# zhangkao/IIP_UAVSal_Saliency

Hardware: AMD Instinct MI355X
Metric: saliency frames/sec at 360x640 (higher is better)
Workload: dtype f32; 1 GPU; 360x640 batch=1 clip(s)/GPU seq=8, UAVSal.forward_clips, prec=f32, launch loop; requests_in_flight=1, clips_per_gpu=1, seq_len=8, height=360, width=640, precision=f32, persistent_state=False, parallelism=single GPU, fused_dw=10

## Files before the change

iip_uavsal_saliency_amd/_lib.py:

```python
from __future__ import annotations

import collections
import ctypes as C
import os

PKG = os.path.dirname(os.path.abspath(__file__))
LIB_PATH = os.environ.get("UAVSAL_HIP_LIB") or os.path.join(PKG, "libuavsal_hip.so")

PREC = {"f32": 0, "bf16x3": 1, "bf16": 2, "f16x3": 3}
ACT_NONE, ACT_RELU6, ACT_SIGMOID = 0, 1, 2
EPI_AFFINE, EPI_TWA, EPI_LSTM = 0, 1, 2
SK_TICKET_BASE = 4096

_ERR = {-1: "UAVSAL_EINVAL (null pointer / non-positive size)",
        -2: "UAVSAL_EALIGN (channel count / ld / pointer not 16-byte aligned)",
        -3: "UAVSAL_ESHAPE (shape not supported by the kernel)",
        -4: "UAVSAL_ESTATE (plan used in the wrong state)",
        -5: "UAVSAL_EDEVICE (a kernel reported a device-side error; the run's outputs are invalid)"}
ERR_STREAMK = 1
DW_KERNEL = {1: "dw3x3_kernel<1, 4, 4>", 2: "dw3x3_kernel<1, 2, 2>", 3: "dw3x3_kernel<2, 2, 2>", 4: "dw3x3_dilated_kernel",
             16: "dw3x3_map_lds_kernel<16, 256>", 32: "dw3x3_map_lds_kernel<32, 256>",
             528: "dw3x3_map_lds_kernel<16, 512>", 544: "dw3x3_map_lds_kernel<32, 512>",
             2048: "dw3x3_rowclass_kernel<256>"}

_f = C.c_void_p


class ConvDesc(C.Structure):
    _fields_ = [("a", _f), ("lda", C.c_int32), ("a_img_stride", C.c_int64),
                ("w", _f), ("scale", _f), ("bias", _f),
                ("out", _f), ("ldc", C.c_int32), ("o_img_stride", C.c_int64),
                ("res", _f), ("ldr", C.c_int32), ("r_img_stride", C.c_int64),
                ("aux", _f), ("ldx", C.c_int32), ("x_img_stride", C.c_int64),
                ("n_img", C.c_int32), ("H", C.c_int32), ("W", C.c_int32),
                ("Cin", C.c_int32), ("Cout", C.c_int32), ("taps", C.c_int32),
                ("prec", C.c_int32), ("act", C.c_int32), ("epi", C.c_int32), ("tile", C.c_int32),
                ("out2", _f), ("ld2", C.c_int32),
                ("dw_w9c", _f), ("dw_scale", _f), ("dw_bias", _f),
                ("dw_stride", C.c_int32), ("dw_Hin", C.c_int32), ("dw_Win", C.c_int32),
                ("sk_ws", _f), ("sk_ws_bytes", C.c_int64),
                ("a_split", _f), ("ldas", C.c_int32),
                ("out_split", _f), ("ldos", C.c_int32),
                ("err", _f), ("sk_spin_limit", C.c_int32), ("sk_debug_drop", C.c_int32),
                ("w_group_stride", C.c_int64), ("n_group", C.c_int32), ("a_group_off", C.c_int32)]


ROUTE_PRESPLIT, ROUTE_DWPROJ, ROUTE_STREAMK, ROUTE_K32, ROUTE_F32_DMA, ROUTE_STAGED = 1, 2, 3, 4, 5, 6
REDUCE_NONE, REDUCE_LAUNCH, REDUCE_IN_LAUNCH = 0, 1, 2


class ConvRoute(C.Structure):
    _fields_ = [("family", C.c_int32), ("tile", C.c_int32), ("dwproj", C.c_int32), ("streamk", C.c_int32),
                ("ksplit", C.c_int32), ("reduce", C.c_int32)]


Route = collections.namedtuple("Route", [f for f, _ in ConvRoute._fields_])


def conv_route(lib, d: ConvDesc) -> Route:
    r = ConvRoute()
    check(lib.uavsal_conv_route_of(C.byref(d), C.byref(r)), "uavsal_conv_route_of")
    return Route(*(int(getattr(r, f)) for f in Route._fields))


class DwDesc(C.Structure):
    _fields_ = [("inp", _f), ("ldi", C.c_int32), ("w9c", _f), ("scale", _f), ("bias", _f),
                ("out", _f), ("ldo", C.c_int32),
                ("n_img", C.c_int32), ("H", C.c_int32), ("W", C.c_int32), ("C", C.c_int32),
                ("stride", C.c_int32), ("dilation", C.c_int32), ("act", C.c_int32),
                ("out_split", _f), ("ldos", C.c_int32), ("dil_group_c", C.c_int32), ("dil_groups", C.c_int32 * 4)]


class DwDotDesc(C.Structure):
    _fields_ = [("inp", _f), ("ldi", C.c_int32), ("w9c", _f), ("scale", _f), ("bias", _f),
                ("w2", _f), ("scale2", _f), ("bias2", _f), ("out", _f), ("ldo", C.c_int32),
                ("n_img", C.c_int32), ("H", C.c_int32), ("W", C.c_int32), ("C", C.c_int32), ("act", C.c_int32)]


class StemDesc(C.Structure):
    _fields_ = [("inp", _f), ("in_u8", _f), ("w", _f), ("scale", _f), ("bias", _f),
                ("out", _f), ("ldo", C.c_int32),
                ("n_img", C.c_int32), ("H", C.c_int32), ("W", C.c_int32),
                ("mean", C.c_float * 3), ("stdv", C.c_float * 3)]


class BilinearDesc(C.Structure):
    _fields_ = [("inp", _f), ("ldi", C.c_int32), ("Hi", C.c_int32), ("Wi", C.c_int32),
                ("out", _f), ("ldo", C.c_int32), ("Ho", C.c_int32), ("Wo", C.c_int32),
                ("n_out", C.c_int32), ("C", C.c_int32), ("src_mod", C.c_int32), ("src_div", C.c_int32),
                ("out_split", _f), ("ldos", C.c_int32)]


class TdiffDesc(C.Structure):
    _fields_ = [("inp", _f), ("ldi", C.c_int32), ("out", _f), ("ldo", C.c_int32),
                ("n_img", C.c_int32), ("HW", C.c_int32), ("C", C.c_int32), ("seq_len", C.c_int32)]


class TsumDesc(C.Structure):
    _fields_ = [("inp", _f), ("ldi", C.c_int32), ("out", _f), ("ldo", C.c_int32),
                ("n_groups", C.c_int32), ("T", C.c_int32), ("HW", C.c_int32), ("C", C.c_int32)]


class LayoutDesc(C.Structure):
    _fields_ = [("inp", _f), ("out", _f), ("n_img", C.c_int32), ("C", C.c_int32), ("HW", C.c_int32),
                ("ld", C.c_int32), ("to_nhwc", C.c_int32), ("Cpad", C.c_int32)]


class PostDesc(C.Structure):
    _fields_ = [("inp", _f), ("out", _f), ("scratch", _f), ("n_img", C.c_int32), ("h", C.c_int32),
                ("w", C.c_int32), ("H", C.c_int32), ("W", C.c_int32)]


class GuardDesc(C.Structure):
    _fields_ = [("err", _f), ("host_err", _f), ("buf", _f * 3), ("n", C.c_int64 * 3)]


class CopyDesc(C.Structure):
    _fields_ = [("inp", _f), ("out", _f), ("in_pitch", C.c_int64), ("out_pitch", C.c_int64),
                ("row_floats", C.c_int64), ("rows", C.c_int32)]


class FillDesc(C.Structure):
    _fields_ = [("out", _f), ("n", C.c_int64), ("bits", C.c_uint32)]


class FusedIrDesc(C.Structure):
    _fields_ = [("inp", _f), ("ldi", C.c_int32), ("w1", _f), ("scale1", _f), ("bias1", _f),
                ("wd", _f), ("scale_d", _f), ("bias_d", _f), ("w2", _f), ("scale2", _f), ("bias2", _f),
                ("res", _f), ("ldr", C.c_int32), ("out", _f), ("ldo", C.c_int32),
                ("n_img", C.c_int32), ("H", C.c_int32), ("W", C.c_int32), ("Cin", C.c_int32),
                ("hidden", C.c_int32), ("Cout", C.c_int32), ("stride", C.c_int32), ("tile", C.c_int32)]


class WinoDesc(C.Structure):
    _fields_ = [("inp", _f), ("ldi", C.c_int32), ("in_img_stride", C.c_int64),
                ("out", _f), ("ldo", C.c_int32), ("out_img_stride", C.c_int64),
                ("n_img", C.c_int32), ("H", C.c_int32), ("W", C.c_int32), ("C", C.c_int32),
                ("Mp", C.c_int64), ("R", C.c_int32),
                ("scale", _f), ("bias", _f), ("act", C.c_int32), ("epi", C.c_int32),
                ("res", _f), ("ldr", C.c_int32), ("res_img_stride", C.c_int64),
                ("aux", _f), ("ldx", C.c_int32), ("aux_img_stride", C.c_int64),
                ("hprev", _f), ("ldh", C.c_int32), ("h_img_stride", C.c_int64),
                ("n_seg", C.c_int32), ("seg_in", _f * 3), ("seg_ld", C.c_int32 * 3), ("seg_c", C.c_int32 * 3),
                ("seg_H", C.c_int32 * 3), ("seg_W", C.c_int32 * 3)]


SCORE_NSTAT, SCORE_REPS, SCORE_RUN, SCORE_NKEY = 16, 100, 4096, 7


class ScoreDesc(C.Structure):
    _fields_ = [("sal", _f), ("fix_loc", _f), ("fix_map", _f), ("jitter", _f),
                ("sal_u8", C.c_int32), ("loc_u8", C.c_int32), ("n_frames", C.c_int32), ("n_pix", C.c_int32),
                ("stats", _f), ("fix_off", _f), ("run_off", _f), ("total_fix", C.c_int64), ("total_runs", C.c_int32),
                ("nan_rows", C.c_int32), ("samp", _f * 2), ("samp_off", _f * 2), ("n_samp", C.c_int64 * 2),
                ("ws", _f), ("ws_bytes", C.c_int64),
                ("out", _f), ("n_keys", C.c_int32), ("keys", C.c_int32 * SCORE_NKEY)]


LETTERBOX_HWC, LETTERBOX_CHW = 0, 1


class LetterboxDesc(C.Structure):
    _fields_ = [("src", _f), ("dst", _f), ("row_pitch", C.c_int64), ("plane_pitch", C.c_int64), ("img_pitch", C.c_int64),
                ("n_img", C.c_int32), ("h0", C.c_int32), ("w0", C.c_int32), ("R", C.c_int32), ("C", C.c_int32),
                ("layout", C.c_int32), ("swap_rb", C.c_int32)]


class OverlayDesc(C.Structure):
    _fields_ = [("frames", _f), ("row_pitch", C.c_int64), ("plane_pitch", C.c_int64), ("img_pitch", C.c_int64),
                ("map", _f), ("map_img_pitch", C.c_int64), ("fix", _f), ("lut", _f),
                ("out", _f), ("ws", _f), ("ws_bytes", C.c_int64),
                ("n_img", C.c_int32), ("layout", C.c_int32), ("h0", C.c_int32), ("w0", C.c_int32),
                ("map_h", C.c_int32), ("map_w", C.c_int32), ("fix_h", C.c_int32), ("fix_w", C.c_int32),
                ("mid_h", C.c_int32), ("mid_w", C.c_int32), ("out_h", C.c_int32), ("out_w", C.c_int32)]


class GazeDesc(C.Structure):
    _fields_ = [("fix_map", _f), ("map_row_pitch", C.c_int64), ("map_col_pitch", C.c_int64), ("map_img_pitch", C.c_int64),
                ("fix_loc", _f), ("loc_row_pitch", C.c_int64), ("loc_col_pitch", C.c_int64), ("loc_img_pitch", C.c_int64),
                ("out", _f), ("flags", _f),
                ("n_img", C.c_int32), ("h0", C.c_int32), ("w0", C.c_int32), ("h", C.c_int32), ("w", C.c_int32)]


LOSS_NSTAT = 16
LOSS_FU_WEIGHTS, LOSS_KL_WEIGHTS = (10.0, -2.0, -1.0), (10.0, 0.0, 0.0)


class LossDesc(C.Structure):
    _fields_ = [("pred", _f), ("truth", _f), ("stats", _f), ("out", _f), ("grad_out", _f), ("grad", _f),
                ("n_img", C.c_int32), ("n_pix", C.c_int32),
                ("w_kl", C.c_double), ("w_cc", C.c_double), ("w_nss", C.c_double)]


PRIOR_MIN_SLAB = 32
PRIOR_MAX_FRAMES = (2 ** 31 - 1) // 255


class PriorAccDesc(C.Structure):
    _fields_ = [("frames", _f), ("row_pitch", C.c_int64), ("col_pitch", C.c_int64), ("img_pitch", C.c_int64),
                ("acc", _f), ("acc_row_pitch", C.c_int64), ("acc_col_pitch", C.c_int64),
                ("n_img", C.c_int32), ("h0", C.c_int32), ("w0", C.c_int32)]


class PriorFinishDesc(C.Structure):
    _fields_ = [("acc", _f), ("acc_row_pitch", C.c_int64), ("acc_col_pitch", C.c_int64),
                ("ws", _f), ("out", _f), ("image", _f),
                ("n_frames", C.c_int32), ("h0", C.c_int32), ("w0", C.c_int32), ("h", C.c_int32), ("w", C.c_int32)]


PRIOR_DESC_TYPES = [PriorAccDesc, PriorFinishDesc]

WGRAD_CHAIN = 1024


class TwaGateDesc(C.Structure):
    _fields_ = [("g", _f), ("ldg", C.c_int32), ("carry", _f), ("z", _f), ("x", _f), ("ldx", C.c_int32),
                ("hprev", _f), ("ldh", C.c_int32), ("dz", _f), ("carry_out", _f), ("dx", _f),
                ("n_pix", C.c_int64), ("C", C.c_int32)]


class TwaWgradDesc(C.Structure):
    _fields_ = [("dz", _f), ("x", _f), ("ldx", C.c_int32), ("h", _f), ("ldh", C.c_int32), ("h0", _f), ("ldh0", C.c_int32),
                ("ws", _f), ("ws_bytes", C.c_int64), ("out", _f),
                ("T", C.c_int32), ("H", C.c_int32), ("W", C.c_int32), ("C", C.c_int32), ("accumulate", C.c_int32)]


class DecBwdDesc(C.Structure):
    _fields_ = [("gy", _f), ("gy_img_pitch", C.c_int64), ("gy_row_pitch", C.c_int64), ("gy_col_pitch", C.c_int64),
                ("y", _f), ("e", _f), ("d", _f), ("s1", _f), ("wd9", _f), ("s2", _f), ("w3", _f), ("s3", _f), ("ge", _f),
                ("n_img", C.c_int32), ("H", C.c_int32), ("W", C.c_int32), ("C", C.c_int32)]


TRAIN_DESC_TYPES = [TwaGateDesc, TwaWgradDesc, DecBwdDesc]

class PixGemmDesc(C.Structure):
    _fields_ = [("a", _f), ("lda", C.c_int32), ("b", _f), ("ldb", C.c_int32), ("row_scale", _f),
                ("w", _f), ("ldw", C.c_int32), ("rowdot", C.c_void_p), ("ws", _f), ("ws_bytes", C.c_int64),
                ("out", _f), ("ldo", C.c_int32), ("K", C.c_int64), ("M", C.c_int32), ("N", C.c_int32), ("accumulate", C.c_int32)]


class DecSumsDesc(C.Structure):
    _fields_ = [("gy", _f), ("gy_img_pitch", C.c_int64), ("gy_row_pitch", C.c_int64), ("gy_col_pitch", C.c_int64),
                ("y", _f), ("e", _f), ("d", _f), ("ga", _f), ("w3", _f), ("s3", _f),
                ("ws", C.c_void_p), ("ws_bytes", C.c_int64),
                ("n_img", C.c_int32), ("H", C.c_int32), ("W", C.c_int32), ("C", C.c_int32)]


class DecFinishDesc(C.Structure):
    _fields_ = [("ws", C.c_void_p), ("ws_bytes", C.c_int64), ("rowdot", C.c_void_p)] + [(n, _f) for n in (
        "wd", "w3", "s2", "s3", "r1", "mu1", "r2", "mu2", "r3", "mu3",
        "g_gamma1", "g_beta1", "g_wd", "g_gamma2", "g_beta2", "g_w3", "g_gamma3", "g_beta3")] + [
        ("C", C.c_int32), ("slabs", C.c_int32), ("accumulate", C.c_int32)]


DEC_NSUM = 12
TRAIN_DECODER_DESC_TYPES = [PixGemmDesc, DecSumsDesc, DecFinishDesc]


class IrBwdDesc(C.Structure):
    _fields_ = [("gd", _f), ("d", _f), ("e", _f), ("wd9", _f), ("s2", _f), ("ga", _f),
                ("n_img", C.c_int32), ("H", C.c_int32), ("W", C.c_int32), ("C", C.c_int32)]


class IrSumsDesc(C.Structure):
    _fields_ = [("gd", _f), ("d", _f), ("e", _f), ("ga", _f), ("go", _f), ("ldgo", C.c_int32),
                ("ws", C.c_void_p), ("ws_bytes", C.c_int64),
                ("n_img", C.c_int32), ("H", C.c_int32), ("W", C.c_int32), ("Ch", C.c_int32), ("Co", C.c_int32)]


class IrFinishDesc(C.Structure):
    _fields_ = [("ws", C.c_void_p), ("ws_bytes", C.c_int64), ("rowdot1", C.c_void_p), ("rowdot3", C.c_void_p)] + [(n, _f) for n in (
        "wd", "s2", "r1", "mu1", "r2", "mu2", "r3", "mu3",
        "g_gamma1", "g_beta1", "g_wd", "g_gamma2", "g_beta2", "g_gamma3", "g_beta3")] + [
        ("Ch", C.c_int32), ("Co", C.c_int32), ("slabs", C.c_int32), ("accumulate", C.c_int32)]


IR_NSUM = 11
BLOCK_DESC_TYPES = [IrBwdDesc, IrSumsDesc, IrFinishDesc]


class IrBwdS2Desc(C.Structure):
    _fields_ = [("gd", _f), ("d", _f), ("e", _f), ("wd9", _f), ("s2", _f), ("ga", _f),
                ("n_img", C.c_int32), ("H", C.c_int32), ("W", C.c_int32), ("C", C.c_int32)]


class BilinearBwdDesc(C.Structure):
    _fields_ = [("gout", _f), ("ldo", C.c_int32), ("Ho", C.c_int32), ("Wo", C.c_int32),
                ("gin", _f), ("Hi", C.c_int32), ("Wi", C.c_int32),
                ("n_out", C.c_int32), ("n_src", C.c_int32), ("C", C.c_int32), ("src_mod", C.c_int32), ("src_div", C.c_int32)]


class TsumBwdDesc(C.Structure):
    _fields_ = [("a", _f), ("lda", C.c_int32), ("g", _f), ("ldg", C.c_int32), ("out", _f), ("ldo", C.c_int32),
                ("n_groups", C.c_int32), ("T", C.c_int32), ("HW", C.c_int32), ("C", C.c_int32)]


CTX_DESC_TYPES = [IrBwdS2Desc, BilinearBwdDesc, TsumBwdDesc]


class IrSumsS2Desc(C.Structure):
    _fields_ = IrSumsDesc._fields_


MP_DESC_TYPES = [IrSumsS2Desc]


class IrNarrowDesc(C.Structure):
    _fields_ = [("x", _f), ("e", _f), ("d", _f), ("gd", _f), ("ga", _f), ("go", _f), ("ldgo", C.c_int32),
                ("ws", C.c_void_p), ("ws_bytes", C.c_int64),
                ("n_img", C.c_int32), ("H", C.c_int32), ("W", C.c_int32), ("Cin", C.c_int32), ("Ch", C.c_int32), ("Co", C.c_int32)]


class IrNarrowFinishDesc(C.Structure):
    _fields_ = [("ws", C.c_void_p), ("ws_bytes", C.c_int64)] + [(n, _f) for n in (
        "w1", "wd", "w3", "s1", "s2", "s3", "r1", "mu1", "r2", "mu2", "r3", "mu3",
        "g_w1", "g_gamma1", "g_beta1", "g_wd", "g_gamma2", "g_beta2", "g_w3", "g_gamma3", "g_beta3")] + [
        ("Cin", C.c_int32), ("Ch", C.c_int32), ("Co", C.c_int32), ("slabs", C.c_int32), ("accumulate", C.c_int32)]


class FrameSumDesc(C.Structure):
    _fields_ = [("a", _f), ("lda", C.c_int32), ("out", _f), ("ldo", C.c_int32),
                ("N", C.c_int32), ("HW", C.c_int32), ("C", C.c_int32)]


NARROW_CHUNK = 32
NETS_DESC_TYPES = [IrNarrowDesc, IrNarrowFinishDesc, FrameSumDesc]

REPACK_MAX_SRC = 4
REPACK_CONV, REPACK_WINO, REPACK_FOLD, REPACK_DW, REPACK_COPY = range(5)
REPACK_LAYOUT = {"f32": 0, "f32k32": 0, "f16x3": 1, "f16x3i": 2, "f16x3j": 3, "bf16": 4, "bf16x3": 5}
REPACK_SCALE, REPACK_BIAS, REPACK_RSTD, REPACK_MEAN = range(4)


class RepackEntry(C.Structure):
    _fields_ = [("kind", C.c_int32), ("layout", C.c_int32), ("dst", _f), ("units", C.c_int64),
                ("src", _f * REPACK_MAX_SRC), ("beta", _f * REPACK_MAX_SRC), ("mean", _f * REPACK_MAX_SRC),
                ("var", _f * REPACK_MAX_SRC), ("eps", C.c_double * REPACK_MAX_SRC), ("rows", C.c_int32 * REPACK_MAX_SRC),
                ("n_src", C.c_int32), ("N", C.c_int32), ("C", C.c_int32), ("taps", C.c_int32), ("Npad", C.c_int32),
                ("Kpad", C.c_int32), ("kt", C.c_int32), ("flip", C.c_int32), ("gi", C.c_int32), ("P", C.c_int32),
                ("sN", C.c_int64), ("sC", C.c_int64), ("off", C.c_int64),
                ("sg", _f), ("sv", _f), ("seps", C.c_double), ("pad", C.c_float), ("reserved", C.c_int32),
                ("G", C.c_double * 18)]


DESC_TYPES = [ConvDesc, DwDesc, StemDesc, BilinearDesc, TdiffDesc, TsumDesc, LayoutDesc, PostDesc, GuardDesc, CopyDesc,
              FusedIrDesc, WinoDesc, DwDotDesc, FillDesc, ScoreDesc, LetterboxDesc, OverlayDesc, GazeDesc, LossDesc, ConvRoute]

SYMBOLS = [
    ("uavsal_conv_gemm", C.c_int, [C.POINTER(ConvDesc), C.c_void_p]),
    ("uavsal_conv_route_of", C.c_int, [C.POINTER(ConvDesc), C.POINTER(ConvRoute)]),
    ("uavsal_conv_tile", C.c_int, [C.POINTER(ConvDesc)]),
    ("uavsal_conv_uses_split", C.c_int, [C.POINTER(ConvDesc)]),
    ("uavsal_conv_dwproj", C.c_int, [C.POINTER(ConvDesc)]),
    ("uavsal_streamk_workspace_bytes", C.c_longlong, []),
    ("uavsal_conv_streamk_grid", C.c_int, [C.POINTER(ConvDesc)]),
    ("uavsal_dw3x3", C.c_int, [C.POINTER(DwDesc), C.c_void_p]),
    ("uavsal_dw3x3_dot", C.c_int, [C.POINTER(DwDotDesc), C.c_void_p]),
    ("uavsal_dw_variant", C.c_int, [C.POINTER(DwDesc)]),
    ("uavsal_stem_conv", C.c_int, [C.POINTER(StemDesc), C.c_void_p]),
    ("uavsal_bilinear_ac", C.c_int, [C.POINTER(BilinearDesc), C.c_void_p]),
    ("uavsal_tdiff", C.c_int, [C.POINTER(TdiffDesc), C.c_void_p]),
    ("uavsal_tsum", C.c_int, [C.POINTER(TsumDesc), C.c_void_p]),
    ("uavsal_layout", C.c_int, [C.POINTER(LayoutDesc), C.c_void_p]),
    ("uavsal_postprocess", C.c_int, [C.POINTER(PostDesc), C.c_void_p]),
    ("uavsal_letterbox_u8", C.c_int, [C.POINTER(LetterboxDesc), C.c_void_p]),
    ("uavsal_overlay_workspace_bytes", C.c_int64, [C.POINTER(OverlayDesc)]),
    ("uavsal_overlay_u8", C.c_int, [C.POINTER(OverlayDesc), C.c_void_p]),
    ("uavsal_gaze_prepare", C.c_int, [C.POINTER(GazeDesc), C.c_void_p]),
    ("uavsal_loss_fu", C.c_int, [C.POINTER(LossDesc), C.c_void_p]),
    ("uavsal_loss_fu_grad", C.c_int, [C.POINTER(LossDesc), C.c_void_p]),
    ("uavsal_prior_accumulate", C.c_int, [C.POINTER(PriorAccDesc), C.c_void_p]),
    ("uavsal_prior_finish", C.c_int, [C.POINTER(PriorFinishDesc), C.c_void_p]),
    ("uavsal_prior_slab_frames", C.c_int, [C.c_int64, C.c_int32]),
    ("uavsal_prior_sizeof_desc", C.c_int, [C.c_int]),
    ("uavsal_twa_gate_bwd", C.c_int, [C.POINTER(TwaGateDesc), C.c_void_p]),
    ("uavsal_twa_wgrad_workspace_bytes", C.c_int64, [C.POINTER(TwaWgradDesc)]),
    ("uavsal_twa_wgrad_shares", C.c_int, [C.POINTER(TwaWgradDesc)]),
    ("uavsal_twa_wgrad", C.c_int, [C.POINTER(TwaWgradDesc), C.c_void_p]),
    ("uavsal_dec_bwd", C.c_int, [C.POINTER(DecBwdDesc), C.c_void_p]),
    ("uavsal_train_sizeof_desc", C.c_int, [C.c_int]),
    ("uavsal_pix_gemm_workspace_bytes", C.c_int64, [C.POINTER(PixGemmDesc)]),
    ("uavsal_pix_gemm_shares", C.c_int, [C.POINTER(PixGemmDesc)]),
    ("uavsal_pix_gemm", C.c_int, [C.POINTER(PixGemmDesc), C.c_void_p]),
    ("uavsal_dec_sums_workspace_bytes", C.c_int64, [C.POINTER(DecSumsDesc)]),
    ("uavsal_dec_sums_slabs", C.c_int, [C.POINTER(DecSumsDesc)]),
    ("uavsal_dec_sums_slab_rows", C.c_int, [C.POINTER(DecSumsDesc)]),
    ("uavsal_dec_sums", C.c_int, [C.POINTER(DecSumsDesc), C.c_void_p]),
    ("uavsal_dec_finish", C.c_int, [C.POINTER(DecFinishDesc), C.c_void_p]),
    ("uavsal_train_decoder_sizeof_desc", C.c_int, [C.c_int]),
    ("uavsal_ir_bwd", C.c_int, [C.POINTER(IrBwdDesc), C.c_void_p]),
    ("uavsal_ir_sums_workspace_bytes", C.c_int64, [C.POINTER(IrSumsDesc)]),
    ("uavsal_ir_sums_slabs", C.c_int, [C.POINTER(IrSumsDesc)]),
    ("uavsal_ir_sums_slab_rows", C.c_int, [C.POINTER(IrSumsDesc)]),
    ("uavsal_ir_sums", C.c_int, [C.POINTER(IrSumsDesc), C.c_void_p]),
    ("uavsal_ir_finish", C.c_int, [C.POINTER(IrFinishDesc), C.c_void_p]),
    ("uavsal_block_sizeof_desc", C.c_int, [C.c_int]),
    ("uavsal_ir_bwd_s2", C.c_int, [C.POINTER(IrBwdS2Desc), C.c_void_p]),
    ("uavsal_bilinear_ac_bwd", C.c_int, [C.POINTER(BilinearBwdDesc), C.c_void_p]),
    ("uavsal_tsum_bwd", C.c_int, [C.POINTER(TsumBwdDesc), C.c_void_p]),
    ("uavsal_ctx_sizeof_desc", C.c_int, [C.c_int]),
    ("uavsal_ir_sums_s2_workspace_bytes", C.c_int64, [C.POINTER(IrSumsS2Desc)]),
    ("uavsal_ir_sums_s2_slabs", C.c_int, [C.POINTER(IrSumsS2Desc)]),
    ("uavsal_ir_sums_s2_slab_rows", C.c_int, [C.POINTER(IrSumsS2Desc)]),
    ("uavsal_ir_sums_s2", C.c_int, [C.POINTER(IrSumsS2Desc), C.c_void_p]),
    ("uavsal_mp_sizeof_desc", C.c_int, [C.c_int]),
    ("uavsal_ir_narrow_workspace_bytes", C.c_int64, [C.POINTER(IrNarrowDesc)]),
    ("uavsal_ir_narrow_slabs", C.c_int, [C.POINTER(IrNarrowDesc)]),
    ("uavsal_ir_narrow_slab_rows", C.c_int, [C.POINTER(IrNarrowDesc)]),
    ("uavsal_ir_narrow_grads", C.c_int, [C.POINTER(IrNarrowDesc), C.c_void_p]),
    ("uavsal_ir_narrow_finish", C.c_int, [C.POINTER(IrNarrowFinishDesc), C.c_void_p]),
    ("uavsal_frame_sum", C.c_int, [C.POINTER(FrameSumDesc), C.c_void_p]),
    ("uavsal_nets_sizeof_desc", C.c_int, [C.c_int]),
    ("uavsal_repack", C.c_int, [C.c_void_p, C.c_int, C.c_int, C.c_void_p]),
    ("uavsal_repack_sizeof_desc", C.c_int, []),
    ("uavsal_guard", C.c_int, [C.POINTER(GuardDesc), C.c_void_p]),
    ("uavsal_copy_rows", C.c_int, [C.POINTER(CopyDesc), C.c_void_p]),
    ("uavsal_fill", C.c_int, [C.POINTER(FillDesc), C.c_void_p]),
    ("uavsal_plan_add_fill", C.c_int, [C.c_void_p, C.POINTER(FillDesc)]),
    ("uavsal_fused_ir", C.c_int, [C.POINTER(FusedIrDesc), C.c_void_p]),
    ("uavsal_fused_ir_supported", C.c_int, [C.POINTER(FusedIrDesc)]),
    ("uavsal_plan_add_fused_ir", C.c_int, [C.c_void_p, C.POINTER(FusedIrDesc)]),
    ("uavsal_wino_input", C.c_int, [C.POINTER(WinoDesc), C.c_void_p]),
    ("uavsal_wino_output", C.c_int, [C.POINTER(WinoDesc), C.c_void_p]),
    ("uavsal_plan_add_wino_input", C.c_int, [C.c_void_p, C.POINTER(WinoDesc)]),
    ("uavsal_plan_add_wino_output", C.c_int, [C.c_void_p, C.POINTER(WinoDesc)]),
    ("uavsal_plan_add_copy", C.c_int, [C.c_void_p, C.POINTER(CopyDesc)]),
    ("uavsal_plan_create", C.c_void_p, []),
    ("uavsal_plan_destroy", None, [C.c_void_p]),
    ("uavsal_plan_add_conv", C.c_int, [C.c_void_p, C.POINTER(ConvDesc)]),
    ("uavsal_plan_add_dw", C.c_int, [C.c_void_p, C.POINTER(DwDesc)]),
    ("uavsal_plan_add_dw_dot", C.c_int, [C.c_void_p, C.POINTER(DwDotDesc)]),
    ("uavsal_plan_add_stem", C.c_int, [C.c_void_p, C.POINTER(StemDesc)]),
    ("uavsal_plan_add_bilinear", C.c_int, [C.c_void_p, C.POINTER(BilinearDesc)]),
    ("uavsal_plan_add_tdiff", C.c_int, [C.c_void_p, C.POINTER(TdiffDesc)]),
    ("uavsal_plan_add_tsum", C.c_int, [C.c_void_p, C.POINTER(TsumDesc)]),
    ("uavsal_plan_add_layout", C.c_int, [C.c_void_p, C.POINTER(LayoutDesc)]),
    ("uavsal_plan_error_word", C.c_void_p, [C.c_void_p]),
    ("uavsal_plan_add_guard", C.c_int, [C.c_void_p, _f, C.c_int64, _f, C.c_int64, _f, C.c_int64]),
    ("uavsal_plan_status", C.c_int, [C.c_void_p, C.c_int]),
    ("uavsal_plan_patch_ptr", C.c_int, [C.c_void_p, C.c_int, C.c_int, C.c_void_p]),
    ("uavsal_plan_set_lane", C.c_int, [C.c_void_p, C.c_int]),
    ("uavsal_plan_add_fork", C.c_int, [C.c_void_p, C.c_int]),
    ("uavsal_plan_add_join", C.c_int, [C.c_void_p, C.c_int]),
    ("uavsal_plan_enable_lanes", C.c_int, [C.c_void_p, C.c_int]),
    ("uavsal_plan_size", C.c_int, [C.c_void_p]),
    ("uavsal_plan_run", C.c_int, [C.c_void_p, C.c_int, C.c_int, C.c_void_p]),
    ("uavsal_plan_group_mark", C.c_int, [C.c_void_p, C.c_int, C.c_int, C.c_int]),
    ("uavsal_plan_group_enable", C.c_int, [C.c_void_p, C.c_int, C.c_int]),
    ("uavsal_plan_group_launches", C.c_int, [C.c_void_p, C.c_int]),
    ("uavsal_plan_last_launches", C.c_int, [C.c_void_p]),
    ("uavsal_plan_frame_repeat", C.c_int, [C.c_void_p, C.c_int, C.c_int, C.c_int, C.c_int, C.c_int]),
    ("uavsal_plan_frame_repeat_workgroups", C.c_int, [C.c_void_p, C.c_int]),
    ("uavsal_plan_graph_build", C.c_int, [C.c_void_p, C.c_void_p]),
    ("uavsal_plan_graph_launch", C.c_int, [C.c_void_p, C.c_void_p]),
    ("uavsal_plan_time", C.c_int, [C.c_void_p, C.c_int, C.c_int, C.c_int, C.c_void_p, C.POINTER(C.c_float)]),
    ("uavsal_score_workspace_bytes", C.c_int64, [C.POINTER(ScoreDesc)]),
    ("uavsal_score_stats", C.c_int, [C.POINTER(ScoreDesc), C.c_void_p]),
    ("uavsal_score_run", C.c_int, [C.POINTER(ScoreDesc), C.c_void_p]),
    ("uavsal_abi_version", C.c_int, []),
    ("uavsal_sizeof_desc", C.c_int, [C.c_int]),
    ("uavsal_build_info", C.c_char_p, []),
]

_lib = None


def load():
    global _lib
    if _lib is not None:
        return _lib
    if not os.path.exists(LIB_PATH):
        raise RuntimeError(
            "libuavsal_hip.so is not built (%s). Run `python -m iip_uavsal_saliency_amd.build` "
            "(needs hipcc). There is no CPU fallback for the UAVSal HIP path." % LIB_PATH)
    lib = C.CDLL(LIB_PATH)
    for name, res, args in SYMBOLS:
        fn = getattr(lib, name)
        fn.restype = res
        fn.argtypes = args
    if lib.uavsal_abi_version() != 20:
        raise RuntimeError("libuavsal_hip.so ABI version mismatch")
    for i, t in enumerate(DESC_TYPES):
        if lib.uavsal_sizeof_desc(i) != C.sizeof(t):
            raise RuntimeError("descriptor %s: ctypes size %d != C size %d" % (
                t.__name__, C.sizeof(t), lib.uavsal_sizeof_desc(i)))
    for sizeof, types in ((lib.uavsal_prior_sizeof_desc, PRIOR_DESC_TYPES), (lib.uavsal_train_sizeof_desc, TRAIN_DESC_TYPES),
                          (lib.uavsal_train_decoder_sizeof_desc, TRAIN_DECODER_DESC_TYPES),
                          (lib.uavsal_block_sizeof_desc, BLOCK_DESC_TYPES), (lib.uavsal_ctx_sizeof_desc, CTX_DESC_TYPES),
                          (lib.uavsal_mp_sizeof_desc, MP_DESC_TYPES), (lib.uavsal_nets_sizeof_desc, NETS_DESC_TYPES)):
        for i, t in enumerate(types):
            if sizeof(i) != C.sizeof(t):
                raise RuntimeError("descriptor %s: ctypes size %d != C size %d" % (t.__name__, C.sizeof(t), sizeof(i)))
    if lib.uavsal_repack_sizeof_desc() != C.sizeof(RepackEntry):
        raise RuntimeError("descriptor RepackEntry: ctypes size %d != C size %d" % (C.sizeof(RepackEntry), lib.uavsal_repack_sizeof_desc()))
    _lib = lib
    return lib


def check(code: int, what: str = "uavsal call"):
    if code == 0:
        return
    if code == -5:
        raise RuntimeError("%s: %s" % (what, _ERR[-5]))
    if code < 0:
        raise RuntimeError("%s rejected its arguments: %s" % (what, _ERR.get(code, str(code))))
    raise RuntimeError("%s failed with hipError_t %d" % (what, code))
```

iip_uavsal_saliency_amd/csrc/plan.hip:

```cpp
#include <vector>
#include <new>
#include "common.h"

namespace {
enum OpKind { OP_CONV = 0, OP_DW, OP_STEM, OP_BILINEAR, OP_TDIFF, OP_TSUM, OP_LAYOUT, OP_GUARD, OP_COPY, OP_FUSED_IR, OP_FORK, OP_JOIN,
              OP_WINO_IN, OP_WINO_OUT, OP_DW_DOT, OP_FILL };
constexpr int MAX_LANES = 8;
constexpr int MAX_GROUPS = 32;

struct Op {
    int kind;
    int lane;
    int group;
    union {
        uavsal_conv_desc conv;
        uavsal_dw_desc dw;
        uavsal_stem_desc stem;
        uavsal_bilinear_desc bil;
        uavsal_tdiff_desc td;
        uavsal_tsum_desc ts;
        uavsal_layout_desc lay;
        uavsal_guard_desc guard;
        uavsal_copy_desc copy;
        uavsal_fused_ir_desc fir;
        uavsal_wino_desc wino;
        uavsal_dw_dot_desc dwdot;
        uavsal_fill_desc fill;
    } u;
};

int run_op(const Op& op, uavsal_stream_t s) {
    switch (op.kind) {
        case OP_CONV: return uavsal_conv_gemm(&op.u.conv, s);
        case OP_DW: return uavsal_dw3x3(&op.u.dw, s);
        case OP_STEM: return uavsal_stem_conv(&op.u.stem, s);
        case OP_BILINEAR: return uavsal_bilinear_ac(&op.u.bil, s);
        case OP_TDIFF: return uavsal_tdiff(&op.u.td, s);
        case OP_TSUM: return uavsal_tsum(&op.u.ts, s);
        case OP_LAYOUT: return uavsal_layout(&op.u.lay, s);
        case OP_GUARD: return uavsal_guard(&op.u.guard, s);
        case OP_COPY: return uavsal_copy_rows(&op.u.copy, s);
        case OP_FUSED_IR: return uavsal_fused_ir(&op.u.fir, s);
        case OP_WINO_IN: return uavsal_wino_input(&op.u.wino, s);
        case OP_WINO_OUT: return uavsal_wino_output(&op.u.wino, s);
        case OP_DW_DOT: return uavsal_dw3x3_dot(&op.u.dwdot, s);
        case OP_FILL: return uavsal_fill(&op.u.fill, s);
    }
    return UAVSAL_EINVAL;
}
}

struct uavsal_plan {
    std::vector<Op> ops;
    hipGraph_t graph = nullptr;
    hipGraphExec_t exec = nullptr;
    int cur_lane = 0;
    bool lanes_on = true;
    hipStream_t side[MAX_LANES] = {};
    std::vector<hipEvent_t> events;
    int32_t* err_dev = nullptr;
    int32_t* err_host = nullptr;
    int32_t* err_host_dev = nullptr;
    hipEvent_t done = nullptr;
    bool ran = false;
    uint32_t groups_off = 0;
    int last_launches = 0;
    int graph_launches = 0;
    int fr_pw = -1, fr_dw = -1, fr_mod = 0, fr_div = 0;
    bool fr_on = false;
    int fr_wg[2] = {0, 0};
};

extern "C" uavsal_plan* uavsal_plan_create(void) { return new (std::nothrow) uavsal_plan(); }

static bool ensure_error_words(uavsal_plan* p) {
    if (p->err_dev && p->err_host && p->done) return true;
    bool ok = hipMalloc((void**)&p->err_dev, 64) == hipSuccess && hipMemset(p->err_dev, 0, 64) == hipSuccess &&
              hipHostMalloc((void**)&p->err_host, 64, hipHostMallocMapped) == hipSuccess;
    if (ok) {
        p->err_host[0] = 0;
        ok = hipHostGetDevicePointer((void**)&p->err_host_dev, p->err_host, 0) == hipSuccess &&
             hipEventCreateWithFlags(&p->done, hipEventDisableTiming) == hipSuccess;
    }
    if (!ok) (void)hipGetLastError();
    return ok;
}

extern "C" int32_t* uavsal_plan_error_word(uavsal_plan* p) { return (p && ensure_error_words(p)) ? p->err_dev : nullptr; }

extern "C" int uavsal_plan_add_guard(uavsal_plan* p, float* b0, int64_t n0, float* b1, int64_t n1, float* b2, int64_t n2) {
    if (!p) return UAVSAL_EINVAL;
    if (p->exec) return UAVSAL_ESTATE;
    if (!ensure_error_words(p)) return UAVSAL_ESTATE;
    Op op; op.kind = OP_GUARD; op.lane = 0; op.group = -1;
    op.u.guard.err = p->err_dev; op.u.guard.host_err = p->err_host_dev;
    op.u.guard.buf[0] = b0; op.u.guard.n[0] = n0;
    op.u.guard.buf[1] = b1; op.u.guard.n[1] = n1;
    op.u.guard.buf[2] = b2; op.u.guard.n[2] = n2;
    for (int b = 0; b < 3; ++b)
        if ((op.u.guard.buf[b] == nullptr) != (op.u.guard.n[b] == 0) || op.u.guard.n[b] < 0) return UAVSAL_EINVAL;
    p->ops.push_back(op);
    return (int)p->ops.size() - 1;
}

extern "C" int uavsal_plan_status(uavsal_plan* p, int wait) {
    if (!p) return UAVSAL_EINVAL;
    if (!p->ran) return 0;
    if (wait) {
        const hipError_t e = hipEventSynchronize(p->done);
        if (e != hipSuccess) return (int)e;
    } else {
        const hipError_t e = hipEventQuery(p->done);
        if (e == hipErrorNotReady) { (void)hipGetLastError(); return 0; }
        if (e != hipSuccess) return (int)e;
    }
    const int32_t code = *(volatile int32_t*)p->err_host;
    if (code == 0) return 0;
    p->err_host[0] = 0;
    const hipError_t e = hipMemset(p->err_dev, 0, 64);
    if (e != hipSuccess) return (int)e;
    return UAVSAL_EDEVICE;
}

extern "C" void uavsal_plan_destroy(uavsal_plan* p) {
    if (!p) return;
    if (p->exec) hipGraphExecDestroy(p->exec);
    if (p->graph) hipGraphDestroy(p->graph);
    for (hipEvent_t e : p->events) if (e) hipEventDestroy(e);
    for (int i = 1; i < MAX_LANES; ++i) if (p->side[i]) hipStreamDestroy(p->side[i]);
    if (p->done) hipEventDestroy(p->done);
    if (p->err_host) hipHostFree(p->err_host);
    if (p->err_dev) hipFree(p->err_dev);
    delete p;
}

extern "C" int uavsal_plan_set_lane(uavsal_plan* p, int lane) {
    if (!p || lane < 0 || lane >= MAX_LANES) return UAVSAL_EINVAL;
    p->cur_lane = lane;
    return 0;
}

extern "C" int uavsal_plan_enable_lanes(uavsal_plan* p, int on) {
    if (!p) return UAVSAL_EINVAL;
    if (p->exec) return UAVSAL_ESTATE;
    p->lanes_on = on != 0;
    return 0;
}

static int add_sync(uavsal_plan* p, int kind, int lane) {
    if (!p || lane < 1 || lane >= MAX_LANES) return UAVSAL_EINVAL;
    if (p->exec) return UAVSAL_ESTATE;
    Op op; op.kind = kind; op.lane = lane; op.group = -1;
    p->ops.push_back(op);
    return (int)p->ops.size() - 1;
}
extern "C" int uavsal_plan_add_fork(uavsal_plan* p, int lane) { return add_sync(p, OP_FORK, lane); }
extern "C" int uavsal_plan_add_join(uavsal_plan* p, int lane) { return add_sync(p, OP_JOIN, lane); }

#define UAVSAL_ADD(fn, KIND, field, T)                                   \
    extern "C" int fn(uavsal_plan* p, const T* d) {                      \
        if (!p || !d) return UAVSAL_EINVAL;                              \
        if (p->exec) return UAVSAL_ESTATE;                               \
        Op op; op.kind = KIND; op.lane = p->cur_lane; op.group = -1; op.u.field = *d; \
        p->ops.push_back(op);                                            \
        return (int)p->ops.size() - 1;                                   \
    }
UAVSAL_ADD(uavsal_plan_add_conv, OP_CONV, conv, uavsal_conv_desc)
UAVSAL_ADD(uavsal_plan_add_dw, OP_DW, dw, uavsal_dw_desc)
UAVSAL_ADD(uavsal_plan_add_stem, OP_STEM, stem, uavsal_stem_desc)
UAVSAL_ADD(uavsal_plan_add_bilinear, OP_BILINEAR, bil, uavsal_bilinear_desc)
UAVSAL_ADD(uavsal_plan_add_tdiff, OP_TDIFF, td, uavsal_tdiff_desc)
UAVSAL_ADD(uavsal_plan_add_tsum, OP_TSUM, ts, uavsal_tsum_desc)
UAVSAL_ADD(uavsal_plan_add_layout, OP_LAYOUT, lay, uavsal_layout_desc)
UAVSAL_ADD(uavsal_plan_add_copy, OP_COPY, copy, uavsal_copy_desc)
UAVSAL_ADD(uavsal_plan_add_fused_ir, OP_FUSED_IR, fir, uavsal_fused_ir_desc)
UAVSAL_ADD(uavsal_plan_add_wino_input, OP_WINO_IN, wino, uavsal_wino_desc)
UAVSAL_ADD(uavsal_plan_add_wino_output, OP_WINO_OUT, wino, uavsal_wino_desc)
UAVSAL_ADD(uavsal_plan_add_dw_dot, OP_DW_DOT, dwdot, uavsal_dw_dot_desc)
UAVSAL_ADD(uavsal_plan_add_fill, OP_FILL, fill, uavsal_fill_desc)

extern "C" int uavsal_plan_patch_ptr(uavsal_plan* p, int op, int slot, void* ptr) {
    if (!p || op < 0 || op >= (int)p->ops.size() || !ptr) return UAVSAL_EINVAL;
    if (p->exec) return UAVSAL_ESTATE;
    Op& o = p->ops[op];
    switch (o.kind) {
        case OP_CONV:
            if (!uavsal_aligned16(ptr)) return UAVSAL_EALIGN;
            if (slot == 0) o.u.conv.a = (const float*)ptr;
            else if (slot == 1) o.u.conv.out = (float*)ptr;
            else return UAVSAL_EINVAL;
            return 0;
        case OP_DW_DOT:
            if (slot == 0) { if (!uavsal_aligned16(ptr)) return UAVSAL_EALIGN; o.u.dwdot.in = (const float*)ptr; }
            else if (slot == 1) o.u.dwdot.out = (float*)ptr;
            else return UAVSAL_EINVAL;
            return 0;
        case OP_STEM:
            if (slot == 0) { o.u.stem.in = (const float*)ptr; o.u.stem.in_u8 = nullptr; }
            else if (slot == 1) { o.u.stem.in_u8 = (const uint8_t*)ptr; o.u.stem.in = nullptr; }
            else return UAVSAL_EINVAL;
            return 0;
        case OP_LAYOUT:
            if (slot == 0) o.u.lay.in = (const float*)ptr;
            else if (slot == 1) o.u.lay.out = (float*)ptr;
            else return UAVSAL_EINVAL;
            return 0;
        case OP_GUARD:
            if (slot < 0 || slot > 2 || !o.u.guard.buf[slot]) return UAVSAL_EINVAL;
            o.u.guard.buf[slot] = (float*)ptr;
            return 0;
    }
    return UAVSAL_ESHAPE;
}

extern "C" int uavsal_plan_size(const uavsal_plan* p) { return p ? (int)p->ops.size() : UAVSAL_EINVAL; }

extern "C" int uavsal_plan_group_mark(uavsal_plan* p, int group, int first, int last) {
    if (!p || group < 0 || group >= MAX_GROUPS || first < 0 || last > (int)p->ops.size() || first >= last) return UAVSAL_EINVAL;
    if (p->exec) return UAVSAL_ESTATE;
    for (int i = first; i < last; ++i)
        if (p->ops[i].group >= 0 && p->ops[i].group != group) return UAVSAL_EINVAL;
    for (int i = first; i < last; ++i) p->ops[i].group = group;
    return 0;
}

extern "C" int uavsal_plan_group_enable(uavsal_plan* p, int group, int on) {
    if (!p || group < 0 || group >= MAX_GROUPS) return UAVSAL_EINVAL;
    const uint32_t bit = 1u << group;
    if (((p->groups_off & bit) == 0) == (on != 0)) return 0;
    if (p->exec) return UAVSAL_ESTATE;
    if (on) p->groups_off &= ~bit; else p->groups_off |= bit;
    return 0;
}

extern "C" int uavsal_plan_group_launches(const uavsal_plan* p, int group) {
    if (!p || group < 0 || group >= MAX_GROUPS) return UAVSAL_EINVAL;
    int n = 0;
    for (const Op& op : p->ops) n += op.group == group && op.kind != OP_FORK && op.kind != OP_JOIN;
    return n;
}

extern "C" int uavsal_plan_last_launches(const uavsal_plan* p) { return p ? p->last_launches : UAVSAL_EINVAL; }

static int run_range(uavsal_plan* p, int first, int last, uavsal_stream_t stream, bool masked, int* launched, bool repeat = false) {
    const int n = (int)p->ops.size();
    if (last < 0 || last > n) last = n;
    if (first < 0 || first > last) return UAVSAL_EINVAL;
    bool fr = repeat && p->fr_on && p->fr_pw >= 0 && first == 0 && last > p->fr_dw;
    if (fr) {
        const Op& a = p->ops[p->fr_pw];
        const Op& b = p->ops[p->fr_dw];
        const uint32_t goff = masked ? p->groups_off : 0u;
        hipStreamCaptureStatus cs = hipStreamCaptureStatusNone;
        if (hipStreamIsCapturing((hipStream_t)stream, &cs) != hipSuccess) { (void)hipGetLastError(); cs = hipStreamCaptureStatusActive; }
        fr = cs == hipStreamCaptureStatusNone && !(a.group >= 0 && ((goff >> a.group) & 1u)) && !(b.group >= 0 && ((goff >> b.group) & 1u)) &&
             uavsal_conv_repeat_pair(&a.u.conv, &b.u.conv, p->fr_mod, p->fr_div) == 1;
    }
    const bool lanes = p->lanes_on && first == 0 && last == n;
    const uint32_t off = masked ? p->groups_off : 0u;
    hipStream_t main_s = (hipStream_t)stream;
    if (p->events.size() < p->ops.size()) p->events.resize(p->ops.size(), nullptr);
    for (int i = first; i < last; ++i) {
        const Op& op = p->ops[i];
        if (op.group >= 0 && ((off >> op.group) & 1u)) continue;
        if (op.kind == OP_FORK || op.kind == OP_JOIN) {
            if (!lanes) continue;
            if (!p->side[op.lane] &&
                hipStreamCreateWithFlags(&p->side[op.lane], hipStreamNonBlocking) != hipSuccess) return (int)hipGetLastError();
            if (!p->events[i] &&
                hipEventCreateWithFlags(&p->events[i], hipEventDisableTiming) != hipSuccess) return (int)hipGetLastError();
            hipStream_t from = op.kind == OP_FORK ? main_s : p->side[op.lane];
            hipStream_t to = op.kind == OP_FORK ? p->side[op.lane] : main_s;
            hipError_t e = hipEventRecord(p->events[i], from);
            if (e == hipSuccess) e = hipStreamWaitEvent(to, p->events[i], 0);
            if (e != hipSuccess) return (int)e;
            continue;
        }
        uavsal_stream_t s = (lanes && op.lane > 0) ? (uavsal_stream_t)p->side[op.lane] : stream;
        if (lanes && op.lane > 0 && !p->side[op.lane]) return UAVSAL_ESTATE;
        int e;
        if (repeat && (i == p->fr_pw || i == p->fr_dw))
            e = uavsal_conv_gemm_mapped(&op.u.conv, s, fr ? p->fr_mod : 0, fr ? p->fr_div : 0, &p->fr_wg[i == p->fr_dw]);
        else
            e = run_op(op, s);
        if (e) return e;
        ++*launched;
    }
    if (last == n) {
        hipStreamCaptureStatus cs = hipStreamCaptureStatusNone;
        if (hipStreamIsCapturing(main_s, &cs) != hipSuccess) { (void)hipGetLastError(); cs = hipStreamCaptureStatusNone; }
        if (cs == hipStreamCaptureStatusNone && p->done) {
            const hipError_t e = hipEventRecord(p->done, main_s);
            if (e != hipSuccess) return (int)e;
            p->ran = true;
        }
    }
    return 0;
}

extern "C" int uavsal_plan_run(uavsal_plan* p, int first, int last, uavsal_stream_t stream) {
    if (!p) return UAVSAL_EINVAL;
    if (first == 0) p->last_launches = 0;
    return run_range(p, first, last, stream, true, &p->last_launches, true);
}

extern "C" int uavsal_plan_frame_repeat(uavsal_plan* p, int op_pw, int op_dwpl, int src_mod, int src_div, int on) {
    const int n = p ? (int)p->ops.size() : 0;
    if (!p || op_pw < 0 || op_dwpl <= op_pw || op_dwpl >= n || src_mod <= 0 || src_div <= 0) return UAVSAL_EINVAL;
    if (p->ops[op_pw].kind != OP_CONV || p->ops[op_dwpl].kind != OP_CONV) return UAVSAL_EINVAL;
    p->fr_pw = op_pw; p->fr_dw = op_dwpl; p->fr_mod = src_mod; p->fr_div = src_div;
    p->fr_on = on != 0 && !p->exec &&
               uavsal_conv_repeat_pair(&p->ops[op_pw].u.conv, &p->ops[op_dwpl].u.conv, src_mod, src_div) == 1;
    return p->fr_on ? 1 : 0;
}

extern "C" int uavsal_plan_frame_repeat_workgroups(const uavsal_plan* p, int which) {
    return p && (which == 0 || which == 1) ? p->fr_wg[which] : UAVSAL_EINVAL;
}

extern "C" int uavsal_plan_graph_build(uavsal_plan* p, uavsal_stream_t stream) {
    if (!p) return UAVSAL_EINVAL;
    if (p->exec) return 0;
    p->fr_on = false;
    hipStream_t s = (hipStream_t)stream;
    hipError_t e = hipStreamBeginCapture(s, hipStreamCaptureModeThreadLocal);
    if (e != hipSuccess) return (int)e;
    const int r = uavsal_plan_run(p, 0, -1, stream);
    hipGraph_t g = nullptr;
    e = hipStreamEndCapture(s, &g);
    if (r) { if (g) hipGraphDestroy(g); return r; }
    if (e != hipSuccess) return (int)e;
    hipGraphExec_t ex = nullptr;
    e = hipGraphInstantiate(&ex, g, nullptr, nullptr, 0);
    if (e != hipSuccess) { hipGraphDestroy(g); return (int)e; }
    p->graph = g; p->exec = ex;
    p->graph_launches = p->last_launches;
    return 0;
}

extern "C" int uavsal_plan_graph_launch(uavsal_plan* p, uavsal_stream_t stream) {
    if (!p) return UAVSAL_EINVAL;
    if (!p->exec) return UAVSAL_ESTATE;
    hipError_t e = hipGraphLaunch(p->exec, (hipStream_t)stream);
    if (e == hipSuccess && p->done) {
        e = hipEventRecord(p->done, (hipStream_t)stream);
        if (e == hipSuccess) p->ran = true;
    }
    if (e == hipSuccess) p->last_launches = p->graph_launches;
    return e == hipSuccess ? 0 : (int)e;
}

extern "C" int uavsal_plan_time(uavsal_plan* p, int first, int last, int iters, uavsal_stream_t stream, float* ms) {
    if (!p || !ms || iters <= 0) return UAVSAL_EINVAL;
    hipStream_t s = (hipStream_t)stream;
    hipEvent_t e0, e1;
    if (hipEventCreate(&e0) != hipSuccess) return (int)hipGetLastError();
    if (hipEventCreate(&e1) != hipSuccess) { hipEventDestroy(e0); return (int)hipGetLastError(); }
    int r = 0, launched = 0;
    hipEventRecord(e0, s);
    for (int i = 0; i < iters && !r; ++i) r = run_range(p, first, last, stream, false, &launched);
    hipEventRecord(e1, s);
    hipError_t e = hipEventSynchronize(e1);
    float t = 0.f;
    if (e == hipSuccess) e = hipEventElapsedTime(&t, e0, e1);
    hipEventDestroy(e0); hipEventDestroy(e1);
    if (r) return r;
    if (e != hipSuccess) return (int)e;
    *ms = t / iters;
    return 0;
}

extern "C" int uavsal_abi_version(void) { return UAVSAL_ABI_VERSION; }

extern "C" int uavsal_sizeof_desc(int which) {
    switch (which) {
        case 0: return (int)sizeof(uavsal_conv_desc);
        case 1: return (int)sizeof(uavsal_dw_desc);
        case 2: return (int)sizeof(uavsal_stem_desc);
        case 3: return (int)sizeof(uavsal_bilinear_desc);
        case 4: return (int)sizeof(uavsal_tdiff_desc);
        case 5: return (int)sizeof(uavsal_tsum_desc);
        case 6: return (int)sizeof(uavsal_layout_desc);
        case 7: return (int)sizeof(uavsal_post_desc);
        case 8: return (int)sizeof(uavsal_guard_desc);
        case 9: return (int)sizeof(uavsal_copy_desc);
        case 10: return (int)sizeof(uavsal_fused_ir_desc);
        case 11: return (int)sizeof(uavsal_wino_desc);
        case 12: return (int)sizeof(uavsal_dw_dot_desc);
        case 13: return (int)sizeof(uavsal_fill_desc);
        case 14: return (int)sizeof(uavsal_score_desc);
        case 15: return (int)sizeof(uavsal_letterbox_desc);
        case 16: return (int)sizeof(uavsal_overlay_desc);
        case 17: return (int)sizeof(uavsal_gaze_desc);
        case 18: return (int)sizeof(uavsal_loss_desc);
        case 19: return (int)sizeof(uavsal_conv_route);
    }
    return UAVSAL_EINVAL;
}

extern "C" const char* uavsal_build_info(void) {
#define UAVSAL_STR2(x) #x
#define UAVSAL_STR(x) UAVSAL_STR2(x)
    return "libuavsal_hip gfx950 abi " UAVSAL_STR(UAVSAL_ABI_VERSION) " (" __DATE__ " " __TIME__ ")";
}
```

iip_uavsal_saliency_amd/csrc/winograd.hip:

```cpp
#include "common.h"

namespace {

struct WinoK {
    const float* in; float* out;
    const float* scale; const float* bias; const float* res; const float* aux; const float* hprev;
    long long in_is, out_is, res_is, aux_is, h_is;
    long long Mp;
    int ldi, ldo, ldr, ldx, ldh;
    int n_img, H, W, C4, ty, tx, act, epi;
    long long total;
    int nseg;
    const float* sin[3];
    int sld[3], sq1[3], sH[3], sW[3];
    float ssy[3], ssx[3];
};

template <int R> struct WinoT;
template <> struct WinoT<2> {
    static constexpr int P = 4;
    __device__ static __forceinline__ void bt(const f32x4 (&d)[4], f32x4 (&t)[4]) {
        t[0] = d[0] - d[2]; t[1] = d[1] + d[2]; t[2] = d[2] - d[1]; t[3] = d[1] - d[3];
    }
    __device__ static __forceinline__ void at(const f32x4 (&m)[4], f32x4 (&y)[2]) {
        y[0] = m[0] + m[1] + m[2]; y[1] = m[1] - m[2] - m[3];
    }
};
template <> struct WinoT<4> {
    static constexpr int P = 6;
    __device__ static __forceinline__ void bt(const f32x4 (&d)[6], f32x4 (&t)[6]) {
        t[0] = 4.f * d[0] - 5.f * d[2] + d[4];
        t[1] = (d[3] + d[4]) - 4.f * (d[1] + d[2]);
        t[2] = 4.f * (d[1] - d[2]) + (d[4] - d[3]);
        t[3] = 2.f * (d[3] - d[1]) + (d[4] - d[2]);
        t[4] = 2.f * (d[1] - d[3]) + (d[4] - d[2]);
        t[5] = 4.f * d[1] - 5.f * d[3] + d[5];
    }
    __device__ static __forceinline__ void at(const f32x4 (&m)[6], f32x4 (&y)[4]) {
        const f32x4 s12 = m[1] + m[2], d12 = m[1] - m[2], s34 = m[3] + m[4], d34 = m[3] - m[4];
        y[0] = m[0] + s12 + s34;
        y[1] = d12 + 2.f * d34;
        y[2] = s12 + 4.f * s34;
        y[3] = d12 + 8.f * d34 + m[5];
    }
};

template <int R, bool SEG>
__global__ __launch_bounds__(256) void wino_input_kernel(const WinoK p) {
    constexpr int P = WinoT<R>::P;
    const long long idx = (long long)blockIdx.x * 256 + threadIdx.x;
    if (idx >= p.total) return;
    const int c4 = (int)(idx % p.C4);
    const long long tile = idx / p.C4;
    const int tpi = p.ty * p.tx;
    const int n = (int)(tile / tpi);
    const int r = (int)(tile - (long long)n * tpi);
    const int tyi = r / p.tx, txi = r - tyi * p.tx;
    const int y0 = R * tyi - 1, x0 = R * txi - 1;
    const float* base = p.in + (size_t)n * p.in_is * p.ldi + c4 * 4;
    int ldi = p.ldi, sW = p.W, sH = p.H;
    bool resize = false;
    float sy = 0.f, sx = 0.f;
    if (SEG) {
        const int s = c4 < p.sq1[0] ? 0 : (c4 < p.sq1[1] ? 1 : 2);
        const int q0 = s == 0 ? 0 : (s == 1 ? p.sq1[0] : p.sq1[1]);
        ldi = s == 0 ? p.sld[0] : (s == 1 ? p.sld[1] : p.sld[2]);
        sH = s == 0 ? p.sH[0] : (s == 1 ? p.sH[1] : p.sH[2]);
        sW = s == 0 ? p.sW[0] : (s == 1 ? p.sW[1] : p.sW[2]);
        sy = s == 0 ? p.ssy[0] : (s == 1 ? p.ssy[1] : p.ssy[2]);
        sx = s == 0 ? p.ssx[0] : (s == 1 ? p.ssx[1] : p.ssx[2]);
        const float* b0 = s == 0 ? p.sin[0] : (s == 1 ? p.sin[1] : p.sin[2]);
        base = b0 + (size_t)n * sH * sW * ldi + (c4 - q0) * 4;
        resize = sH != p.H || sW != p.W;
    }
    int ry0[P], ry1[P];
    float rly[P];
    if (SEG && resize) {
#pragma unroll
        for (int i = 0; i < P; ++i) {
            const int y = y0 + i;
            const float fy = sy * (float)y;
            const int a = (int)fy;
            ry0[i] = a; ry1[i] = a + (a < sH - 1 ? 1 : 0); rly[i] = fy - (float)a;
        }
    }
    f32x4 t[P][P];
#pragma unroll
    for (int j = 0; j < P; ++j) {
        const int x = x0 + j;
        f32x4 col[P], tc[P];
        int cx0 = 0, cx1 = 0;
        float lx = 0.f;
        if (SEG && resize) {
            const float fx = sx * (float)x;
            cx0 = (int)fx; cx1 = cx0 + (cx0 < sW - 1 ? 1 : 0); lx = fx - (float)cx0;
        }
#pragma unroll
        for (int i = 0; i < P; ++i) {
            const int y = y0 + i;
            const bool ok = y >= 0 && y < p.H && x >= 0 && x < p.W;
            if (SEG && resize) {
                col[i] = (f32x4){0.f, 0.f, 0.f, 0.f};
                if (ok) {
                    const float ly = rly[i], hy = 1.f - ly, hx = 1.f - lx;
                    const f32x4 v00 = *reinterpret_cast<const f32x4*>(base + ((size_t)ry0[i] * sW + cx0) * ldi);
                    const f32x4 v01 = *reinterpret_cast<const f32x4*>(base + ((size_t)ry0[i] * sW + cx1) * ldi);
                    const f32x4 v10 = *reinterpret_cast<const f32x4*>(base + ((size_t)ry1[i] * sW + cx0) * ldi);
                    const f32x4 v11 = *reinterpret_cast<const f32x4*>(base + ((size_t)ry1[i] * sW + cx1) * ldi);
                    col[i] = hy * (hx * v00 + lx * v01) + ly * (hx * v10 + lx * v11);
                }
            } else {
                col[i] = ok ? *reinterpret_cast<const f32x4*>(base + ((size_t)y * p.W + x) * ldi) : (f32x4){0.f, 0.f, 0.f, 0.f};
            }
        }
        WinoT<R>::bt(col, tc);
#pragma unroll
        for (int i = 0; i < P; ++i) t[i][j] = tc[i];
    }
    float* o = p.out + (size_t)tile * p.ldo + c4 * 4;
    const size_t plane = (size_t)p.Mp * p.ldo;
#pragma unroll
    for (int i = 0; i < P; ++i) {
        f32x4 v[P];
        WinoT<R>::bt(t[i], v);
#pragma unroll
        for (int j = 0; j < P; ++j) *reinterpret_cast<f32x4*>(o + (size_t)(P * i + j) * plane) = v[j];
    }
}

__device__ __forceinline__ f32x4 sigmoid4(f32x4 z) {
    f32x4 g;
    g.x = 1.f / (1.f + expf(-z.x)); g.y = 1.f / (1.f + expf(-z.y));
    g.z = 1.f / (1.f + expf(-z.z)); g.w = 1.f / (1.f + expf(-z.w));
    return g;
}

template <int R>
__global__ __launch_bounds__(256) void wino_output_kernel(const WinoK p) {
    constexpr int P = WinoT<R>::P;
    const long long idx = (long long)blockIdx.x * 256 + threadIdx.x;
    if (idx >= p.total) return;
    const int c4 = (int)(idx % p.C4);
    const long long tile = idx / p.C4;
    const int tpi = p.ty * p.tx;
    const int n = (int)(tile / tpi);
    const int r = (int)(tile - (long long)n * tpi);
    const int tyi = r / p.tx, txi = r - tyi * p.tx;
    const float* mi = p.in + (size_t)tile * p.ldi + c4 * 4;
    const size_t plane = (size_t)p.Mp * p.ldi;
    f32x4 s[R][P];
#pragma unroll
    for (int j = 0; j < P; ++j) {
        f32x4 col[P], sc_[R];
#pragma unroll
        for (int i = 0; i < P; ++i) col[i] = *reinterpret_cast<const f32x4*>(mi + (size_t)(P * i + j) * plane);
        WinoT<R>::at(col, sc_);
#pragma unroll
        for (int a = 0; a < R; ++a) s[a][j] = sc_[a];
    }
    f32x4 y[R][R];
#pragma unroll
    for (int a = 0; a < R; ++a) WinoT<R>::at(s[a], y[a]);
    f32x4 sc = {1.f, 1.f, 1.f, 1.f}, bi = {0.f, 0.f, 0.f, 0.f};
    if (p.scale) {
        sc = *reinterpret_cast<const f32x4*>(p.scale + c4 * 4);
        bi = *reinterpret_cast<const f32x4*>(p.bias + c4 * 4);
    }
    const float lo = p.act == UAVSAL_ACT_RELU6 ? 0.f : -3.0e38f, hi = p.act == UAVSAL_ACT_RELU6 ? 6.f : 3.0e38f;
#pragma unroll
    for (int a = 0; a < R; ++a)
#pragma unroll
        for (int b = 0; b < R; ++b) {
            const int yy = R * tyi + a, xx = R * txi + b;
            if (yy >= p.H || xx >= p.W) continue;
            const size_t pix = (size_t)yy * p.W + xx;
            f32x4 v = y[a][b];
            if (p.epi == UAVSAL_EPI_TWA) {
                const f32x4 z = v + *reinterpret_cast<const f32x4*>(p.aux + ((size_t)n * p.aux_is + pix) * p.ldx + c4 * 4);
                const f32x4 xt = *reinterpret_cast<const f32x4*>(p.res + ((size_t)n * p.res_is + pix) * p.ldr + c4 * 4);
                const f32x4 hp = *reinterpret_cast<const f32x4*>(p.hprev + ((size_t)n * p.h_is + pix) * p.ldh + c4 * 4);
                const f32x4 g = sigmoid4(z);
                v = g * xt + (1.f - g) * hp;
            } else {
                v.x = __builtin_amdgcn_fmed3f(fmaf(v.x, sc.x, bi.x), lo, hi); v.y = __builtin_amdgcn_fmed3f(fmaf(v.y, sc.y, bi.y), lo, hi);
                v.z = __builtin_amdgcn_fmed3f(fmaf(v.z, sc.z, bi.z), lo, hi); v.w = __builtin_amdgcn_fmed3f(fmaf(v.w, sc.w, bi.w), lo, hi);
                if (p.res) v += *reinterpret_cast<const f32x4*>(p.res + ((size_t)n * p.res_is + pix) * p.ldr + c4 * 4);
            }
            *reinterpret_cast<f32x4*>(p.out + ((size_t)n * p.out_is + pix) * p.ldo + c4 * 4) = v;
        }
}

int fill(const uavsal_wino_desc* d, WinoK& k, bool input) {
    if (!d || !d->out) return UAVSAL_EINVAL;
    const bool seg = input && d->n_seg > 0;
    if (!seg && !d->in) return UAVSAL_EINVAL;
    if (d->n_seg < 0 || d->n_seg > 3 || (!input && d->n_seg)) return UAVSAL_EINVAL;
    if (d->n_img <= 0 || d->H <= 0 || d->W <= 0 || d->C <= 0) return UAVSAL_EINVAL;
    if ((d->C & 3) || (d->ldo & 3) || d->ldo < d->C) return UAVSAL_EALIGN;
    if (!seg && ((d->ldi & 3) || d->ldi < d->C || !uavsal_aligned16(d->in))) return UAVSAL_EALIGN;
    if (!uavsal_aligned16(d->out)) return UAVSAL_EALIGN;
    k.nseg = 0;
    for (int s = 0; s < 3; ++s) { k.sin[s] = nullptr; k.sld[s] = 0; k.sq1[s] = 0x7fffffff; k.sH[s] = d->H; k.sW[s] = d->W; k.ssy[s] = k.ssx[s] = 0.f; }
    if (seg) {
        int c = 0;
        for (int s = 0; s < d->n_seg; ++s) {
            if (!d->seg_in[s] || d->seg_c[s] <= 0 || d->seg_H[s] <= 0 || d->seg_W[s] <= 0) return UAVSAL_EINVAL;
            if ((d->seg_c[s] & 3) || (d->seg_ld[s] & 3) || d->seg_ld[s] < d->seg_c[s] || !uavsal_aligned16(d->seg_in[s])) return UAVSAL_EALIGN;
            c += d->seg_c[s];
            k.sin[s] = d->seg_in[s]; k.sld[s] = d->seg_ld[s]; k.sq1[s] = c / 4; k.sH[s] = d->seg_H[s]; k.sW[s] = d->seg_W[s];
            k.ssy[s] = d->H > 1 ? (float)(d->seg_H[s] - 1) / (float)(d->H - 1) : 0.f;
            k.ssx[s] = d->W > 1 ? (float)(d->seg_W[s] - 1) / (float)(d->W - 1) : 0.f;
        }
        if (c != d->C) return UAVSAL_ESHAPE;
        k.sq1[d->n_seg - 1] = 0x7fffffff;
        k.nseg = d->n_seg;
    }
    if (d->R != 2 && d->R != 4) return UAVSAL_ESHAPE;
    k.ty = (d->H + d->R - 1) / d->R; k.tx = (d->W + d->R - 1) / d->R;
    const long long tiles = (long long)d->n_img * k.ty * k.tx;
    if ((d->Mp & 127) || d->Mp < tiles) return UAVSAL_ESHAPE;
    k.in = d->in; k.out = d->out; k.ldi = d->ldi; k.ldo = d->ldo; k.Mp = d->Mp;
    k.n_img = d->n_img; k.H = d->H; k.W = d->W; k.C4 = d->C / 4;
    const long long hw = (long long)d->H * d->W;
    k.in_is = d->in_img_stride > 0 ? d->in_img_stride : hw;
    k.out_is = d->out_img_stride > 0 ? d->out_img_stride : hw;
    k.scale = k.bias = k.res = k.aux = k.hprev = nullptr;
    k.res_is = k.aux_is = k.h_is = hw; k.ldr = k.ldx = k.ldh = 0; k.act = UAVSAL_ACT_NONE; k.epi = UAVSAL_EPI_AFFINE;
    if (!input) {
        if ((d->scale == nullptr) != (d->bias == nullptr)) return UAVSAL_EINVAL;
        if (d->act != UAVSAL_ACT_NONE && d->act != UAVSAL_ACT_RELU6) return UAVSAL_ESHAPE;
        if (d->epi != UAVSAL_EPI_AFFINE && d->epi != UAVSAL_EPI_TWA) return UAVSAL_ESHAPE;
        k.scale = d->scale; k.bias = d->bias; k.act = d->act; k.epi = d->epi;
        if (d->res) {
            if ((d->ldr & 3) || d->ldr < d->C || !uavsal_aligned16(d->res)) return UAVSAL_EALIGN;
            k.res = d->res; k.ldr = d->ldr; k.res_is = d->res_img_stride > 0 ? d->res_img_stride : hw;
        }
        if (d->epi == UAVSAL_EPI_TWA) {
            if (!d->res || !d->aux || !d->hprev) return UAVSAL_EINVAL;
            if ((d->ldx & 3) || (d->ldh & 3) || d->ldx < d->C || d->ldh < d->C || !uavsal_aligned16(d->aux) || !uavsal_aligned16(d->hprev))
                return UAVSAL_EALIGN;
            k.aux = d->aux; k.ldx = d->ldx; k.aux_is = d->aux_img_stride > 0 ? d->aux_img_stride : hw;
            k.hprev = d->hprev; k.ldh = d->ldh; k.h_is = d->h_img_stride > 0 ? d->h_img_stride : hw;
        }
        if (d->scale && (!uavsal_aligned16(d->scale) || !uavsal_aligned16(d->bias))) return UAVSAL_EALIGN;
    }
    k.total = tiles * k.C4;
    if ((k.total + 255) / 256 > 0x7fffffffLL) return UAVSAL_ESHAPE;
    return 0;
}

}

extern "C" int uavsal_wino_input(const uavsal_wino_desc* d, uavsal_stream_t stream) {
    WinoK k;
    const int e = fill(d, k, true);
    if (e) return e;
    const dim3 grid((unsigned)((k.total + 255) / 256));
    if (k.nseg) {
        if (d->R == 4) hipLaunchKernelGGL((wino_input_kernel<4, true>), grid, dim3(256), 0, (hipStream_t)stream, k);
        else hipLaunchKernelGGL((wino_input_kernel<2, true>), grid, dim3(256), 0, (hipStream_t)stream, k);
    } else if (d->R == 4) hipLaunchKernelGGL((wino_input_kernel<4, false>), grid, dim3(256), 0, (hipStream_t)stream, k);
    else hipLaunchKernelGGL((wino_input_kernel<2, false>), grid, dim3(256), 0, (hipStream_t)stream, k);
    return uavsal_launch_status();
}

extern "C" int uavsal_wino_output(const uavsal_wino_desc* d, uavsal_stream_t stream) {
    WinoK k;
    const int e = fill(d, k, false);
    if (e) return e;
    if (d->R == 4) hipLaunchKernelGGL(wino_output_kernel<4>, dim3((unsigned)((k.total + 255) / 256)), dim3(256), 0, (hipStream_t)stream, k);
    else hipLaunchKernelGGL(wino_output_kernel<2>, dim3((unsigned)((k.total + 255) / 256)), dim3(256), 0, (hipStream_t)stream, k);
    return uavsal_launch_status();
}
```

iip_uavsal_saliency_amd/engine.py:

```python
from __future__ import annotations

import contextlib
import ctypes as C
from typing import Dict, Optional

import torch

from . import _lib as L
from .arena import ARENA_ALIGN, Arena, _ArenaRef, arena_conflict, plan_arena
from .views import OpView, V, _down, read_view
from .recorder import PRIOR_GROUP, Recorder
from .topology import record_forward
from .weights import WeightCache


class PriorCache:

    def __init__(self, lib, plan, ops):
        self.lib, self.plan, self.ops = lib, plan, sorted(ops)
        self.marked = self.off = False
        self.rec = self.new = None
        self.group_launches = 0

    def mark(self):
        if self.marked:
            return
        self.marked = True
        ops = self.ops
        i = 0
        while i < len(ops):
            j = i
            while j + 1 < len(ops) and ops[j + 1] == ops[j] + 1:
                j += 1
            L.check(self.lib.uavsal_plan_group_mark(self.plan, PRIOR_GROUP, ops[i], ops[j] + 1), "plan_group_mark")
            i = j + 1
        self.group_launches = int(self.lib.uavsal_plan_group_launches(self.plan, PRIOR_GROUP)) if ops else 0

    def gate(self, sig, check) -> bool:
        self.mark()
        self.new = None
        if not self.ops:
            return False
        skip = False
        rec = self.rec
        if sig is not None and rec is not None and len(rec["sig"]) == len(sig) and all(
                a[0] is b[0] and a[1:] == b[1:] for a, b in zip(rec["sig"], sig)):
            if not rec["confirmed"]:
                check()
            skip = self.rec is not None
        if not skip:
            self.rec = None
            self.new = None if sig is None else dict(sig=sig, bound={})
        if skip != self.off:
            L.check(self.lib.uavsal_plan_group_enable(self.plan, PRIOR_GROUP, 0 if skip else 1), "plan_group_enable")
            self.off = skip
        return skip

    def note(self, bound):
        if self.new is not None:
            self.new["bound"].update(bound)

    def compare_frames(self, src_idx):
        if self.new is None:
            return
        ts = [t for t in self.new["bound"].values() if t.shape[0] > 1]
        if not ts:
            self.new["same"] = True
            return
        ok = None
        for t in ts:
            e = (t == t.index_select(0, src_idx)).all()
            ok = e if ok is None else ok & e
        word = torch.zeros(1, dtype=torch.bool).pin_memory()
        word.copy_(ok.reshape(1), non_blocking=True)
        ev = torch.cuda.Event()
        ev.record()
        self.new["same"] = (ev, word)

    def frames_repeat(self) -> bool:
        s = self.rec.get("same") if self.rec is not None else None
        if isinstance(s, tuple):
            ev, word = s
            if not ev.query():
                return False
            s = self.rec["same"] = bool(word[0])
        return s is True

    def bound(self):
        return self.rec["bound"]

    @contextlib.contextmanager
    def launches(self):
        try:
            yield
        except Exception:
            self.rec = self.new = None
            raise
        if self.new is not None:
            self.rec = dict(self.new, confirmed=False)
            self.new = None

    def confirm(self):
        if self.rec is not None:
            self.rec["confirmed"] = True

    def drop(self):
        self.rec = None


class Engine:
    def __init__(self, model, device, n_seq, seq_len, H, W, ctx_T, ctx_mode="tile",
                 precision="f32", taps=False, in_dtype=torch.float32, use_graph=False, fuse_dw=None,
                 use_lanes=True, stream_k=True, sync_errors=True, persistent=False,
                 wcache=None, static_priors=False, plan_only=False):
        if precision not in L.PREC:
            raise ValueError("precision must be one of %s" % list(L.PREC))
        self.lib = L.load()
        self.device = torch.device(device)
        self.plan_only = bool(plan_only)
        if self.device.type != "cuda" and not self.plan_only:
            raise RuntimeError("Engine needs a cuda (ROCm) device; there is no CPU fallback")
        self.model, self.n_seq, self.seq_len = model, n_seq, seq_len
        self.N = n_seq * seq_len
        self.H, self.W = H, W
        self.ctx_T, self.ctx_mode = ctx_T, ctx_mode
        self.prec_name, self.prec = precision, L.PREC[precision]
        self.keep_taps = taps
        self.in_dtype = in_dtype
        self.static_priors = bool(static_priors)
        self.use_graph = use_graph
        self.stream_k = bool(stream_k)
        self.sync_errors = bool(sync_errors)
        self._first_run_verified = False
        self._sk_debug = tuple(getattr(model, "_sk_debug", (0, 0)))
        self.fuse_dw = fuse_dw if fuse_dw is None else bool(fuse_dw)
        if self.N % ctx_T:
            raise RuntimeError("frame count %d is not a multiple of time_dims %d" % (self.N, ctx_T))
        self.h = _down(_down(_down(H)))
        self.w = _down(_down(_down(W)))
        self.weights = WeightCache(self.device, wcache if wcache is not None else {})
        self.lstm = getattr(model, "rnn_type", "twa") == "lstm"
        self.persistent = bool(persistent)
        presplit = getattr(model, "presplit", None)
        self.prec_overrides = dict(getattr(model, "prec_overrides", None) or {})
        for v in self.prec_overrides.values():
            if v not in L.PREC:
                raise ValueError("prec_overrides: unknown precision %r" % (v,))
        self.split_mode = (precision == "f16x3" and not self.prec_overrides
                           and (bool(presplit) if presplit is not None else n_seq >= 4))
        self.winograd = (precision == "f32" or bool(getattr(model, "prec_overrides", None))) and bool(getattr(model, "winograd", True))
        self.winograd_r = int(getattr(model, "winograd_r", None) or 4)
        self.winograd_step_r = int(getattr(model, "winograd_step_r", None)
                                   or (2 if getattr(model, "winograd_r", None) == 2 else 0))
        self.fuse_blocks = bool(getattr(model, "fuse_blocks", True))
        self.use_priors = tuple(bool(getattr(model, a, 1)) for a in ("use_gauss_prior", "use_ob_prior", "use_context_prior"))
        self.inplace = not use_graph
        self._bound_t: Dict[str, torch.Tensor] = {}
        self.priors = None
        self.use_arena = bool(getattr(model, "arena", True))
        self.arena_debug = bool(getattr(model, "arena_debug", False))
        self.rec = Recorder(torch, self.lib, self.device, self.weights, precision, self.prec_overrides, self.split_mode, self.stream_k,
                            self._sk_debug, self.fuse_dw, self.fuse_blocks, self.use_arena, self.arena_debug)
        if self.plan_only:
            self._size()
            return
        with torch.cuda.device(self.device):
            self._init_on_device(use_lanes)

    plan = property(lambda self: self.rec.plan)
    ops_meta = property(lambda self: self.rec.ops_meta)
    op_args = property(lambda self: self.rec.op_args)
    _op_idx = property(lambda self: self.rec.op_idx)
    named = property(lambda self: self.rec.named)
    stage_ranges = property(lambda self: self.rec.stage_ranges)
    arena = property(lambda self: self.rec.arena)
    _scratch = property(lambda self: self.rec.scratch)
    _sk_ws = property(lambda self: self.rec.sk_ws)
    x_in = property(lambda self: self.rec.callers["x"])
    cb0_in = property(lambda self: self.rec.callers["cb0"])
    cb1_in = property(lambda self: self.rec.callers["cb1"])
    state_in = property(lambda self: self.rec.callers["state_in"])
    state_out = property(lambda self: self.rec.callers["state_out"])
    cstate_in = property(lambda self: self.rec.callers["cstate_in"])
    cstate_out = property(lambda self: self.rec.callers["cstate_out"])
    zero_state = property(lambda self: self.rec.callers["zero_state"])
    out = property(lambda self: self.rec.callers["out"])
    logits = property(lambda self: self.rec.callers.get("logits"))
    _prior_rec = property(lambda self: self.priors.rec)
    prior_group_launches = property(lambda self: self.priors.group_launches if self.priors else 0)
    _arena = property(lambda self: self.arena.buf)
    arena_stats = property(lambda self: self.arena.stats)
    TAP_NAMES = ("c3", "c4", "c5", "sfnet", "st0", "st1", "fust_in_cb", "prefuse", "rnn")
    TAPS_ON_REQUEST = ("fu320", "cb192")

    def _size(self):
        self.rec.begin(dry=True)
        record_forward(self.rec, self)
        self.rec.place(self.TAP_NAMES + self.TAPS_ON_REQUEST if self.keep_taps else ())

    def arena_layout(self):
        return self.arena.layout()

    def _init_on_device(self, use_lanes, resume=False):
        if not resume:
            self._size()
        N, h, w = self.N, self.h, self.w
        f32, state = torch.float32, (self.n_seq, 256, h, w)
        stage = "shape" if self.inplace else "empty"
        np_ = 1 if self.static_priors else N
        callers = {"x": ((N, 3, self.H, self.W), self.in_dtype, stage), "cb0": ((np_, 8, h, w), f32, stage),
                   "cb1": ((np_, 20, h, w), f32, stage), "state_in": (state, f32, "zeros"),
                   "zero_state": (state, f32, "zeros"),
                   "state_out": (state, f32, "empty"), "cstate_in": (state, f32, "zeros"), "cstate_out": (state, f32, "empty"),
                   "out": ((N, h * w), f32, "empty")}
        if self.keep_taps:
            callers["logits"] = ((N, h * w), f32, "empty")
        rec = self.rec
        rec.allocate(callers)
        rec.begin(dry=False)
        record_forward(rec, self)
        rec.end()
        if self.persistent:
            self.h_view, self.c_view = (rec.named[k].t.view(self.n_seq, h, w, 256).permute(0, 3, 1, 2) if k in rec.named else None
                                        for k in ("h0", "c0"))
        self.priors = PriorCache(self.lib, rec.plan, rec.prior_ops)
        pw, dwpl = rec.op_idx.get("fucb.pw"), rec.op_idx.get("fucb.dwpl")
        self._fr = None
        if pw is not None and dwpl is not None and rec.ops_meta[pw]["kind"] == "conv1" and rec.ops_meta[dwpl]["kind"] == "conv1":
            self._fr = (pw, dwpl) + ((N // self.ctx_T, 1) if self.ctx_mode == "tile" else (N, self.ctx_T))
        self._fr_idx = None
        self.repeat_armed = False
        self.use_lanes = bool(use_lanes)
        L.check(self.lib.uavsal_plan_enable_lanes(self.plan, 1 if self.use_lanes else 0), "plan_enable_lanes")
        self._graph_ready = False

    def __del__(self):
        try:
            if getattr(self, "plan", None) and not getattr(self, "plan_only", False):
                self.lib.uavsal_plan_destroy(self.plan)
                self.rec.plan = None
        except Exception:
            pass

    def bound(self, name) -> torch.Tensor:
        return self._bound_t[name] if self.inplace else self.rec.callers[name]

    def _stream(self):
        return C.c_void_p(torch.cuda.current_stream(self.device).cuda_stream)

    def _prior_sig(self, srcs):
        sig = []
        for t, on in zip(srcs, self.use_priors[:2]):
            if not on:
                continue
            try:
                base = t._base if t._base is not None else t
                sig.append((base, t.data_ptr(), tuple(t.shape), tuple(t.stride()), t._version))
            except RuntimeError:
                return None
        return sig

    def drop_prior_record(self):
        self.priors.drop()

    def _prior_gate(self, srcs) -> bool:
        sig = self._prior_sig(srcs) if (self.inplace and bool(getattr(self.model, "cache_priors", True))) else None
        return self.priors.gate(sig, lambda: self.check(wait=True))

    def _arm_repeat(self, skip):
        self.repeat_armed = False
        if self._fr is None or not self.inplace:
            return
        pw, dwpl, mod, div = self._fr
        if not skip:
            if self._fr_idx is None:
                self._fr_idx = torch.tensor([(f // div * div) % mod for f in range(self.N)], dtype=torch.int64, device=self.device)
            self.priors.compare_frames(self._fr_idx)
        on = (skip and bool(getattr(self.model, "dedupe_priors", True)) and bool(getattr(self.model, "cache_priors", True))
              and self.priors.frames_repeat())
        r = self.lib.uavsal_plan_frame_repeat(self.plan, pw, dwpl, mod, div, 1 if on else 0)
        if r < 0:
            L.check(r, "plan_frame_repeat")
        self.repeat_armed = r == 1

    def _disarm_repeat(self):
        if self.repeat_armed:
            pw, dwpl, mod, div = self._fr
            self.lib.uavsal_plan_frame_repeat(self.plan, pw, dwpl, mod, div, 0)

    def repeat_workgroups(self):
        return tuple(int(self.lib.uavsal_plan_frame_repeat_workgroups(self.plan, i)) for i in (0, 1))

    def last_launches(self) -> int:
        return int(self.lib.uavsal_plan_last_launches(self.plan))

    def launch(self):
        self.priors.mark()
        if self.use_graph:
            cur = torch.cuda.current_stream(self.device)
            if not self._graph_ready:
                self._gstream = torch.cuda.Stream(self.device)
                self._gstream.wait_stream(cur)
                gs = C.c_void_p(self._gstream.cuda_stream)
                L.check(self.lib.uavsal_plan_run(self.plan, 0, -1, gs), "plan_run (warm-up)")
                self._gstream.synchronize()
                L.check(self.lib.uavsal_plan_graph_build(self.plan, gs), "plan_graph_build")
                self._graph_ready = True
            self._gstream.wait_stream(cur)
            L.check(self.lib.uavsal_plan_graph_launch(self.plan, C.c_void_p(self._gstream.cuda_stream)),
                    "plan_graph_launch")
            cur.wait_stream(self._gstream)
        else:
            if self.inplace and not self._bound_t:
                raise RuntimeError("launch-loop plan was never bound to the caller's tensors (Engine.run does that)")
            L.check(self.lib.uavsal_plan_run(self.plan, 0, -1, self._stream()), "plan_run")

    def _is_resident(self, t, view) -> bool:
        return (t is not None and view is not None and t.data_ptr() == view.data_ptr()
                and t.numel() == view.numel() and t.reshape(view.shape).stride() == view.stride())

    def _stage_state_persistent(self, state, cstate):
        pairs = [(state, self.h_view, self.state_in, "h0")]
        if self.c_view is not None:
            pairs.append((cstate, self.c_view, self.cstate_in, "c0"))
        for t, view, stage, name in pairs:
            if self._is_resident(t, view):
                continue
            buf = self.named[name]
            if t is None:
                buf.t.zero_()
                continue
            stage.copy_(t.reshape(stage.shape))
            d = L.LayoutDesc()
            d.inp, d.out, d.n_img, d.C, d.HW, d.ld, d.to_nhwc, d.Cpad = (
                stage.data_ptr(), buf.ptr, self.n_seq, 256, self.h * self.w, 256, 1, 0)
            L.check(self.lib.uavsal_layout(C.byref(d), self._stream()), "uavsal_layout(state)")

    def _bind_in_place(self, x, cb0, cb1, state, cstate, lstm, skip_priors=False):
        dev, callers = self.device, self.rec.callers
        bound = {"x": x.reshape(callers["x"].shape).contiguous()}
        if not skip_priors:
            for name, t, on in (("cb0", cb0, self.use_priors[0]), ("cb1", cb1, self.use_priors[1])):
                if not on:
                    continue
                if self.static_priors:
                    t = t[:1]
                bound[name] = t.reshape(callers[name].shape).contiguous()
            self.priors.note({k: bound[k] for k in ("cb0", "cb1") if k in bound})
        out = bound["out"] = torch.empty((self.N, self.h * self.w), dtype=torch.float32, device=dev)
        st = None
        if self.persistent:
            self._stage_state_persistent(state, cstate)
        else:
            shape = callers["state_in"].shape
            for nm, t in [("state", state)] + ([("cstate", cstate)] if lstm else []):
                bound[nm + "_in"] = callers["zero_state"] if t is None else t.reshape(shape).contiguous()
                bound[nm + "_out"] = torch.empty(shape, dtype=torch.float32, device=dev)
            st = (bound["state_out"], bound["cstate_out"]) if lstm else bound["state_out"]
        for name, op, slot, off in self.rec.binds:
            if name in bound:
                L.check(self.lib.uavsal_plan_patch_ptr(self.plan, op, slot, bound[name].data_ptr() + off), "plan_patch_ptr(%s)" % name)
        if skip_priors:
            bound.update(self.priors.bound())
        self._bound_t = bound
        return out, st

    def stage_inputs(self, x, cb0, cb1, state, cstate=None):
        self.x_in.copy_(x.reshape(self.x_in.shape))
        for t, stage, on in ((cb0, self.cb0_in, self.use_priors[0]), (cb1, self.cb1_in, self.use_priors[1])):
            if on:
                stage.copy_((t[:1] if self.static_priors else t).reshape(stage.shape))
        if self.persistent:
            return self._stage_state_persistent(state, cstate)
        if state is None:
            self.state_in.zero_()
        else:
            self.state_in.copy_(state.reshape(self.state_in.shape))
        if cstate is None:
            self.cstate_in.zero_()
        else:
            self.cstate_in.copy_(cstate.reshape(self.cstate_in.shape))

    def run(self, x, cb0, cb1, state=None, taps: Optional[dict] = None, cstate=None, prior_src=None):
        if x.dtype != self.in_dtype:
            raise RuntimeError("engine built for %s frames, got %s" % (self.in_dtype, x.dtype))
        lstm = self.lstm
        with torch.cuda.device(self.device):
            self.check(wait=False)
            skip = self._prior_gate(prior_src if prior_src is not None else (cb0, cb1))
            if self.inplace:
                out, st = self._bind_in_place(x, cb0, cb1, state, cstate, lstm, skip)
            else:
                self.stage_inputs(x, cb0, cb1, state, cstate)
            self._arm_repeat(skip)
            with self.priors.launches():
                try:
                    self.launch()
                finally:
                    self._disarm_repeat()
            if self.sync_errors:
                self.check(wait=True)
            if not self._first_run_verified and self.split_mode:
                self._first_run_verified = True
                self.check(wait=True)
                res = out if self.inplace else self.out
                if bool(torch.isnan(res).any().item()) and not bool(torch.isnan(x.float()).any().item()):
                    raise RuntimeError("the first run of this plan produced NaN maps from finite frames: a split shadow "
                                       "was read that no producer wrote (Recorder.no_shadow is missing a buffer)")
            if not self.inplace:
                out = self.out.clone()
                if self.persistent:
                    st = None
                else:
                    st = self.state_out.clone()
                    if lstm:
                        st = (st, self.cstate_out.clone())
            if self.persistent:
                st = (self.h_view, self.c_view) if lstm else self.h_view
            if taps is not None:
                if not self.keep_taps:
                    raise RuntimeError("engine was built without taps")
                for k in self.TAPS_ON_REQUEST:
                    if k in taps:
                        if k not in self.named:
                            raise RuntimeError("this plan has no buffer %r to tap (a model without priors)" % k)
                        taps[k] = self.tap(k, channels_last=True)
                for k in self.TAP_NAMES:
                    if k in self.named:
                        taps[k] = self.tap(k)
                taps["logits"] = self.logits.clone().view(self.N, 1, self.h, self.w)
        return out, st

    def state_split(self) -> int:
        for i, m in enumerate(self.ops_meta):
            if m.get("name", "").startswith(("twa.step0", "lstm.step0")):
                return i
        raise RuntimeError("plan has no recurrence step")

    def run_streamed(self, x, cb0, cb1, prev: Optional["Engine"] = None, prev_done: Optional[torch.cuda.Event] = None, reset=False):
        if not (self.persistent and self.inplace):
            raise RuntimeError("run_streamed needs the resident-state launch-loop plan (model.persistent_state = True, no graph)")
        lstm = self.lstm
        with torch.cuda.device(self.device):
            self.check(wait=False)
            skip = self._prior_gate((cb0, cb1))
            out, _ = self._bind_in_place(x, cb0, cb1, self.h_view, self.c_view, lstm, skip)
            split = self.state_split()
            self._arm_repeat(skip)
            with self.priors.launches():
                try:
                    L.check(self.lib.uavsal_plan_run(self.plan, 0, split, self._stream()), "plan_run(head)")
                finally:
                    self._disarm_repeat()
                cur = torch.cuda.current_stream(self.device)
                if prev_done is not None:
                    cur.wait_event(prev_done)
                for name in ("h0", "c0") if lstm else ("h0",):
                    mine = self.named[name].t
                    if reset:
                        mine.zero_()
                    elif prev is not None and prev is not self:
                        mine.copy_(prev.named[name].t)
                L.check(self.lib.uavsal_plan_run(self.plan, split, -1, self._stream()), "plan_run(tail)")
        return out

    def check(self, wait=True):
        code = self.lib.uavsal_plan_status(self.plan, 1 if wait else 0)
        if code == 0:
            if wait:
                self.priors.confirm()
            return
        self.priors.drop()
        if code == -5:
            torch.cuda.synchronize(self.device)
            for ws in self._sk_ws.values():
                ws[:65536].zero_()
            raise RuntimeError("UAVSal HIP path: a stream-K hand-off timed out on the device "
                               "(UAVSAL_ERR_STREAMK); the maps and state of that call are invalid (NaN-filled)")
        L.check(code, "uavsal_plan_status")

    def streamk_clean(self) -> bool:
        torch.cuda.synchronize(self.device)
        return all(int(ws[:65536].view(torch.int32).abs().sum().item()) == 0 for ws in self._sk_ws.values())

    def tap(self, name, channels_last=False) -> torch.Tensor:
        v = self.named[name]
        base = v.t.tensor() if isinstance(v.t, _ArenaRef) else v.t
        t = base.view(v.n, v.h, v.w, v.ld) if base.numel() == v.n * v.h * v.w * v.ld else None
        if t is None:
            raise RuntimeError("tap %s is not a dense buffer" % name)
        t = t[..., v.coff:v.coff + v.c]
        return t.contiguous().permute(0, 3, 1, 2) if channels_last else t.permute(0, 3, 1, 2).contiguous()

    def run_ops(self, first, last):
        if last > first:
            L.check(self.lib.uavsal_plan_run(self.plan, first, last, self._stream()), "plan_run")

    def time_ops(self, first, last, iters=10) -> float:
        ms = C.c_float(0.0)
        L.check(self.lib.uavsal_plan_time(self.plan, first, last, iters, self._stream(), C.byref(ms)), "plan_time")
        return float(ms.value)
```

iip_uavsal_saliency_amd/model.py:

```python
from __future__ import annotations

import os
from collections import OrderedDict
from typing import Dict, List, Optional, Sequence, Tuple

import numpy as np
import torch
import torch.nn as nn

from .model_convlstm import ConvLSTM, ConvTWA
from .model_feature import ReMobileNetV2, _no_eager

feature_inplanes = {"mobilenet_v2": [24, 32, 96, 320]}


def init_weights(model, funcname="kaiming_normal", **kwargs):
    fn = {"kaiming_normal": nn.init.kaiming_normal_, "kaiming_uniform": nn.init.kaiming_uniform_,
          "xavier_uniform": nn.init.xavier_uniform_, "xavier_normal": nn.init.xavier_normal_,
          "normal": nn.init.normal_, "uniform": nn.init.uniform_}[funcname]
    for m in model.modules():
        if isinstance(m, nn.Conv2d):
            fn(m.weight, **kwargs)
            if m.bias is not None:
                nn.init.zeros_(m.bias)
        elif isinstance(m, nn.BatchNorm2d):
            nn.init.ones_(m.weight)
            nn.init.zeros_(m.bias)


class BasicConv2d(nn.Sequential):

    def __init__(self, in_planes, out_planes, kernel_size=3, stride=1, dilation=1, groups=1):
        padding = dilation * (kernel_size - 1) // 2
        super().__init__(
            nn.Conv2d(in_planes, out_planes, kernel_size, stride, padding, dilation=dilation, groups=groups, bias=False),
            nn.BatchNorm2d(out_planes), nn.ReLU6(inplace=True))

    def forward(self, x):
        _no_eager("BasicConv2d")


class dwBlock(nn.Module):

    def __init__(self, inp, oup, kernel_size=3, stride=1, expand_ratio=6, dilation=1, res_connect=None):
        super().__init__()
        assert stride in (1, 2) and kernel_size == 3
        hidden = int(round(inp * expand_ratio))
        self.stride, self.dilation, self.expand_ratio = stride, dilation, expand_ratio
        self.cin, self.cout, self.hidden = inp, oup, hidden
        self.use_res_connect = stride == 1 and inp == oup
        if res_connect is not None:
            self.use_res_connect = bool(res_connect) and self.use_res_connect
        layers = []
        if expand_ratio != 1:
            layers.append(BasicConv2d(inp, hidden, kernel_size=1))
        layers += [BasicConv2d(hidden, hidden, kernel_size, stride=stride, dilation=dilation, groups=hidden),
                   nn.Conv2d(hidden, oup, 1, 1, 0, bias=False), nn.BatchNorm2d(oup)]
        self.conv = nn.Sequential(*layers)

    def forward(self, x):
        _no_eager("dwBlock")


class uavsal_srfnet_aspp(nn.Module):

    def __init__(self, cnn_type="mobilenet_v2", planes=(64, 64, 128, 256), last_channel=256):
        super().__init__()
        if cnn_type.lower() != "mobilenet_v2":
            raise NotImplementedError("the HIP path covers the mobilenet_v2 backbone (Demo_Test.py:33)")
        planes = list(planes)
        if last_channel == 128:
            planes = [32, 32, 64, 128]
        inpl = feature_inplanes["mobilenet_v2"]
        self.conv_lv3 = BasicConv2d(inpl[1], planes[1], 1)
        self.conv_lv4 = BasicConv2d(inpl[2], planes[2], 1)
        self.lv5_aspp1 = BasicConv2d(inpl[3], planes[3], 1)
        self.lv5_aspp2 = dwBlock(inpl[3], planes[3], 3, dilation=6)
        self.lv5_aspp3 = dwBlock(inpl[3], planes[3], 3, dilation=12)
        self.lv5_aspp4 = dwBlock(inpl[3], planes[3], 3, dilation=18)
        self.conv_lv5 = BasicConv2d(planes[3] * 4, planes[3], 1)
        self.conv_last = BasicConv2d(planes[1] + planes[2] + planes[3], last_channel, 3)
        init_weights(self, "kaiming_normal", mode="fan_out")
        self.features = ReMobileNetV2(name="mobilenet_v2")

    def forward(self, x):
        _no_eager("uavsal_srfnet_aspp")


class spConv(nn.Module):
    def __init__(self, inplanes, planes=256, kernel_size=3, stride=1, expand_ratio=6, dilation=1, res_connect=False):
        super().__init__()
        self.spconv = dwBlock(inplanes, planes, kernel_size, stride, expand_ratio, dilation, res_connect)
        init_weights(self, "kaiming_normal", mode="fan_out")

    def forward(self, x):
        _no_eager("spConv")


class teConv_sub(nn.Module):
    def __init__(self, inplanes, planes=256, time_dims=8, reduction=8, res_connect=False):
        super().__init__()
        self.time_dims = time_dims
        self.res_connect = res_connect and inplanes == planes
        width = planes // reduction
        self.reduce_conv = BasicConv2d(inplanes, width, 1)
        self.sub_conv = dwBlock(2 * width, width, 3, res_connect=False)
        self.last_conv = BasicConv2d(width, planes, 1)
        init_weights(self, "kaiming_normal", mode="fan_out")

    def forward(self, x):
        _no_eager("teConv_sub")


class STBlock(nn.Module):
    def __init__(self, inplanes, planes=256, time_dims=8, fu_type="sum", res_connect=True, **kwargs):
        super().__init__()
        if fu_type.lower() != "sum":
            raise NotImplementedError("UAVSal builds STBlock with fu_type='sum' (model.py:274)")
        self.res_connect = res_connect and inplanes == planes
        self.time_dims, self.fu_type, self.inplanes, self.planes = time_dims, "sum", inplanes, planes
        self.stconv_sp = spConv(inplanes, planes, res_connect=False)
        self.stconv_te = teConv_sub(inplanes, planes, time_dims, res_connect=False, **kwargs)
        self.stconv_last = BasicConv2d(planes, planes, 1)
        init_weights(self, "kaiming_normal", mode="fan_out")

    def forward(self, x):
        _no_eager("STBlock")


class UAVSal(nn.Module):
    rnn_type = "twa"

    def __init__(self, cnn_type="mobilenet_v2", time_dims=5, num_stblock=2, bias_type=[1, 1, 1],
                 iosize=[360, 640, 45, 80], planes=256, pre_model_path="", precision="f32"):
        super().__init__()
        bias_type = [int(b) for b in bias_type]
        if len(bias_type) != 3 or any(b not in (0, 1) for b in bias_type):
            raise ValueError("bias_type must be three 0/1 flags [gauss, observed, context] (reference model.py:281-284)")
        if planes != 256:
            raise NotImplementedError("planes=256 is the only configuration on the Demo_Test path")
        self.time_dims = time_dims
        self.precision = precision
        self.use_graph = False
        self.fuse_dw = None
        self.use_lanes = True
        self.stream_k = True
        self.presplit = None
        self.fuse_blocks = True
        self.winograd = True
        self.prec_overrides = None
        self.winograd_r = None
        self.sync_errors = None
        self.persistent_state = False
        self.dedupe_priors = True
        self.cache_priors = True
        self.arena = True
        self.arena_debug = False
        self.max_engines = 4
        self.check_weight_versions = True
        self.sfnet = uavsal_srfnet_aspp(cnn_type, last_channel=planes)
        self.num_stblock = num_stblock
        self.st_layer = nn.Sequential(*[
            STBlock(planes, planes, time_dims=time_dims, reduction=planes // 32, res_connect=True)
            for _ in range(num_stblock)])
        self.fust_layer = nn.Sequential(dwBlock(planes, planes, kernel_size=3))
        self.use_gauss_prior, self.use_ob_prior, self.use_context_prior = bias_type
        self.num_cb = int(np.sum(np.array(bias_type) > 0))
        if self.use_gauss_prior:
            self.gauss_cb_layer = nn.Sequential(dwBlock(8, 64, kernel_size=3), dwBlock(64, 64, kernel_size=3))
            init_weights(self.gauss_cb_layer)
        if self.use_ob_prior:
            self.ob_cb_layer = nn.Sequential(dwBlock(20, 64, kernel_size=3), dwBlock(64, 64, kernel_size=3))
            init_weights(self.ob_cb_layer)
        if self.use_context_prior:
            self.cxt_cb_prior = nn.Sequential(dwBlock(planes, 64, kernel_size=3, stride=2),
                                              dwBlock(64, 64, kernel_size=3, stride=2))
            init_weights(self.cxt_cb_prior)
        if self.num_cb:
            self.fucb_layer = nn.Sequential(dwBlock(64 * self.num_cb, planes // 4, kernel_size=3))
            self.fucbst_layer = nn.Sequential(dwBlock(planes + planes // 4, planes, kernel_size=3))
        _, _, shape_r_out, shape_c_out = iosize
        rnn_cls = ConvLSTM if self.rnn_type == "lstm" else ConvTWA
        self.rnn = rnn_cls((shape_r_out, shape_c_out), planes, planes, kernel_size=(3, 3), num_layers=1,
                           batch_first=True, bias=False, return_all_layers=False)
        self.conv_out_st = dwBlock(planes, 1, kernel_size=3)
        init_weights(self.st_layer, "kaiming_normal", mode="fan_out")
        init_weights(self.fust_layer, "kaiming_normal", mode="fan_out")
        init_weights(self.conv_out_st, "kaiming_normal", mode="fan_out")
        self._engines: "OrderedDict[tuple, object]" = OrderedDict()
        self._wshared: Dict[str, dict] = {}
        self._wversion = None
        if pre_model_path and os.path.exists(pre_model_path):
            from .checkpoint import load_reference_state_dict
            self.load_state_dict(load_reference_state_dict(pre_model_path), strict=False)

    def replica(self):
        import copy
        r = copy.copy(self)
        r._wshared, r._wversion = self._wshared, self._wversion
        for k in ("_wtensors", "_wvers"):
            if k in self.__dict__:
                setattr(r, k, self.__dict__[k])
        return r

    _RUNTIME_STATE = ("_engines", "_wshared", "_wversion", "_wtensors", "_wvers", "_stream_replicas", "_stream_streams")

    def __getstate__(self):
        return {k: v for k, v in self.__dict__.items() if k not in self._RUNTIME_STATE}

    def __setstate__(self, state):
        super().__setstate__(state)
        self._engines = OrderedDict()
        self._wshared = {}
        self._wversion = None

    def _drop_engines(self):
        self._engines = OrderedDict()
        self._wshared = {}
        self._wversion = None

    invalidate_engines = _drop_engines

    def refresh_weights(self, *modules, device=False):
        from .weights import WeightCache
        if self._wversion is None or "_wtensors" not in self.__dict__:
            return 0
        mods = {id(s): s for m in modules for s in m.modules()}
        mine = {id(t) for m in modules for t in list(m.parameters()) + list(m.buffers())}
        then = self.__dict__.get("_wvers")
        if then is None or any(t._version != v for t, v in zip(self._wtensors, then) if id(t) not in mine):
            self._drop_engines()
            return 0
        caches = [WeightCache(dev, store) for dev, store in self._wshared.items()]
        if device and any(c.device.type == "cpu" for c in caches):
            raise ValueError("refresh_weights(device=True) needs packed weights on a GPU: this model holds a CPU store")
        for c in caches:
            (c.refresh_device if device else c.refresh)(mods, dry=True)
        n = sum(c.refresh_device(mods) if device else c.refresh(mods) for c in caches)
        for m in [self] + list(self.__dict__.get("_stream_replicas") or []):
            if m._wversion is not None and "_wtensors" in m.__dict__:
                m._wversion = m._weights_version()
                m._wvers = [t._version for t in m._wtensors]
        nets = [getattr(self, a, None) for a in ("gauss_cb_layer", "ob_cb_layer")]
        if any(id(s) in mods for net in nets if net is not None for s in net.modules()):
            self.invalidate_priors()
        return n

    def invalidate_priors(self):
        for m in [self] + list(self.__dict__.get("_stream_replicas") or []):
            for eng in list(m._engines.values()):
                eng.drop_prior_record()

    def _weights_version(self):
        return sum(t._version for t in self._wtensors)

    def check_errors(self):
        for eng in list(self._engines.values()):
            eng.check(wait=True)

    def load_state_dict(self, *args, **kwargs):
        out = super().load_state_dict(*args, **kwargs)
        self._drop_engines()
        return out

    def _apply(self, fn, *args, **kwargs):
        out = super()._apply(fn, *args, **kwargs)
        self._drop_engines()
        return out

    def train(self, mode: bool = True):
        if mode:
            self._drop_engines()
        return super().train(mode)

    @staticmethod
    def frame_invariant(cb, frame_dims=1):
        return all(all(t.shape[d] == 1 or t.stride(d) == 0 for d in range(frame_dims)) for t in cb)

    def _check_weights(self):
        if not self.check_weight_versions:
            return
        if self._wversion is not None and self._weights_version() != self._wversion:
            self._drop_engines()
        if self._wversion is None:
            self._wtensors = [t for k, t in self.state_dict(keep_vars=True).items()
                              if not k.endswith("num_batches_tracked")]
            self._wversion = self._weights_version()
            self._wvers = [t._version for t in self._wtensors]

    def _engine(self, device, n_seq, seq_len, H, W, ctx_mode, taps=False, in_dtype=torch.float32, sync_default=True, static_priors=False):
        from .engine import Engine
        self._check_weights()
        key = (str(device), n_seq, seq_len, H, W, self.time_dims if ctx_mode == "tile" else seq_len,
               ctx_mode, self.precision, bool(taps), in_dtype, bool(self.use_graph), self.rnn_type, self.fuse_dw, bool(self.use_lanes),
               bool(self.stream_k), bool(self.persistent_state), tuple(getattr(self, "_sk_debug", (0, 0))),
               self.presplit, bool(self.fuse_blocks), bool(getattr(self, "winograd", True)), getattr(self, "winograd_r", None),
               tuple(sorted((getattr(self, "prec_overrides", None) or {}).items())), bool(static_priors),
               bool(getattr(self, "arena", True)), bool(getattr(self, "arena_debug", False)))
        eng = self._engines.get(key)
        if eng is None:
            while len(self._engines) >= max(1, int(self.max_engines)):
                _, old = self._engines.popitem(last=False)
                old.check(wait=True)
            eng = Engine(self, device, n_seq=n_seq, seq_len=seq_len, H=H, W=W,
                         ctx_T=key[5], ctx_mode=ctx_mode, precision=self.precision, taps=taps,
                         in_dtype=in_dtype, use_graph=self.use_graph, fuse_dw=self.fuse_dw,
                         use_lanes=self.use_lanes, stream_k=self.stream_k, persistent=self.persistent_state,
                         wcache=self._wshared.setdefault(str(torch.device(device)), {}), static_priors=static_priors)
            self._engines[key] = eng
        else:
            self._engines.move_to_end(key)
        eng.sync_errors = sync_default if self.sync_errors is None else bool(self.sync_errors)
        return eng

    def _check_common(self, x):
        if self.training:
            raise RuntimeError("UAVSal HIP path is inference-only: call model.eval() (Demo_Test.py:55)")
        if not x.is_cuda:
            raise RuntimeError("UAVSal.forward needs tensors on the MI355X (cuda) device; "
                               "there is no CPU fallback in this package")
        if x.dtype != torch.float32 and x.dtype != torch.uint8:
            raise RuntimeError("frames must be float32 (ImageNet-normalised) or uint8 RGB")

    @torch.no_grad()
    def forward(self, x, cb, in_state=None, taps: Optional[dict] = None):
        self._check_common(x)
        if x.dim() != 4 or x.shape[1] != 3:
            raise RuntimeError("x must be [B*T, 3, H, W]")
        n, _, H, W = x.shape
        if n < 2:
            raise RuntimeError("UAVSal.forward needs at least 2 frames per call (reference teConv_sub, model.py:194)")
        if n % self.time_dims:
            raise RuntimeError("shape '[%d, %d, ...]' is invalid for input of %d frames (model.py:357)" % (
                n // self.time_dims, self.time_dims, n))
        cb0, cb1 = self._used_cb(cb)
        static = self.dedupe_priors and n > 1 and self._static(cb0, cb1, 1)
        eng = self._engine(x.device, 1, n, H, W, "tile", taps is not None, x.dtype, static_priors=static)
        h, w = eng.h, eng.w
        self._check_cb(cb0, cb1, n, h, w)
        st, cst = None, None
        if in_state is not None:
            st = in_state[0]
            if self.rnn_type == "lstm":
                st, cst = st
            if tuple(st.shape) != (1, 256, h, w) or (cst is not None and tuple(cst.shape) != (1, 256, h, w)):
                raise RuntimeError("in_state tensors must be [1, 256, %d, %d]" % (h, w))
            if st.dtype != torch.float32 or st.device != x.device:
                raise RuntimeError("in_state must be float32 on the frames' device")
        out, state = eng.run(x, cb0, cb1, st, taps, cstate=cst)
        if self.rnn_type == "lstm":
            return out.view(n, 1, h, w), [state[0].view(1, 256, h, w), state[1].view(1, 256, h, w)]
        return out.view(n, 1, h, w), [state.view(1, 256, h, w)]

    @torch.no_grad()
    def forward_clips(self, x, cb, states=None, taps: Optional[dict] = None):
        self._check_common(x)
        if x.dim() != 5 or x.shape[2] != 3:
            raise RuntimeError("x must be [C, T, 3, H, W]")
        C, T, _, H, W = x.shape
        if T < 2:
            raise RuntimeError("each clip needs at least 2 frames (reference teConv_sub, model.py:194)")
        cb0, cb1 = self._used_cb(cb)
        for t in (cb0, cb1):
            if t is not None and (t.dim() != 5 or tuple(t.shape[:2]) != (C, T)):
                raise RuntimeError("cb tensors must be [C, T, channels, h, w]")
        static = self.dedupe_priors and self._static(cb0, cb1, 2)
        eng = self._engine(x.device, C, T, H, W, "clip", taps is not None, x.dtype, sync_default=False, static_priors=static)
        h, w = eng.h, eng.w
        src = (cb0, cb1)
        cb0 = None if cb0 is None else cb0.reshape(C * T, *cb0.shape[2:])
        cb1 = None if cb1 is None else cb1.reshape(C * T, *cb1.shape[2:])
        self._check_cb(cb0, cb1, C * T, h, w)
        cst = None
        if self.rnn_type == "lstm" and states is not None:
            states, cst = states
        if states is not None and tuple(states.shape) != (C, 256, h, w):
            raise RuntimeError("states must be [C, 256, h, w]")
        out, state = eng.run(x.reshape(C * T, 3, H, W), cb0, cb1, states, taps, cstate=cst, prior_src=src)
        if self.rnn_type == "lstm":
            return out.view(C, T, 1, h, w), (state[0].view(C, 256, h, w), state[1].view(C, 256, h, w))
        return out.view(C, T, 1, h, w), state.view(C, 256, h, w)

    def _used_cb(self, cb):
        need = 2 if self.use_ob_prior else (1 if self.use_gauss_prior else 0)
        if need and (cb is None or len(cb) < need):
            raise RuntimeError("cb must be [gauss priors, observed priors] (Demo_Test.py:14-27)")
        return (cb[0] if self.use_gauss_prior else None), (cb[1] if self.use_ob_prior else None)

    def _static(self, cb0, cb1, frame_dims):
        used = [t for t in (cb0, cb1) if t is not None]
        return bool(used) and all(t.dim() > frame_dims for t in used) and self.frame_invariant(used, frame_dims)

    @staticmethod
    def _check_cb(cb0, cb1, n, h, w):
        for t, c, what in ((cb0, 8, "gauss"), (cb1, 20, "observed")):
            if t is None:
                continue
            if tuple(t.shape) != (n, c, h, w):
                raise RuntimeError("%s priors must be [%d,%d,%d,%d], got %s" % (what, n, c, h, w, tuple(t.shape)))
            if t.dtype != torch.float32:
                raise RuntimeError("cb tensors must be float32")


class UAVSAL_LSTM(UAVSal):
    rnn_type = "lstm"
```

iip_uavsal_saliency_amd/recorder.py:

```python
import ctypes as C
from typing import Dict, List, Optional

import torch

from . import _lib as L
from . import synth
from .arena import Arena, _ArenaRef
from .packing import conv_weight_layout, roundup
from .views import Caller, OpView, V, _Fake

FUSE_DW_MIN_WORK = 1 << 20
FUSE_DW_MAX_WASTE = 1.15


MID_MIN_WGS = 1
MID_MAX_WGS = 288


def _dwproj_patch_waste(h, w):
    return ((h + 7) // 8 * 8) * ((w + 15) // 16 * 16) / float(h * w)


BLOCK_CHUNK_BYTES = 6 << 30

PRIOR_LANE = 1
PRIOR_GROUP = 0


SLOT_CONV_A, SLOT_CONV_OUT = 0, 1
SLOT_STEM_F32, SLOT_STEM_U8 = 0, 1
SLOT_LAYOUT_IN, SLOT_LAYOUT_OUT = 0, 1


class Recorder:
    def __init__(self, alloc, lib, device, weights, precision, prec_overrides, split_mode, stream_k, sk_debug, fuse_dw, fuse_blocks,
                 use_arena, arena_debug):
        self.torch = alloc
        self.lib, self.device, self.weights = lib, device, weights
        self.prec_name, self.prec, self.prec_overrides = precision, L.PREC[precision], prec_overrides
        self.split_mode, self.stream_k, self.sk_debug = split_mode, stream_k, sk_debug
        self.fuse_dw, self.fuse_blocks = fuse_dw, fuse_blocks
        self.use_arena, self.arena_debug = use_arena, arena_debug
        self.arena = Arena()
        self.plan, self.err = None, None
        self.split_want, self.no_shadow = set(), set()
        self.scratch_need: Dict[tuple, int] = {}
        self.arena_floats = 0
        self.scratch: Dict[tuple, torch.Tensor] = {}
        self.sk_ws: Dict[int, torch.Tensor] = {}
        self.callers: Dict[str, torch.Tensor] = {}
        self.keep: List[torch.Tensor] = []

    def begin(self, dry):
        self.dry = dry
        self.lane = 0
        self.arena.begin(dry)
        self.ops_meta: List[dict] = []
        self.op_args: List[dict] = []
        self.op_idx: Dict[str, int] = {}
        self.stage_ranges: Dict[str, tuple] = {}
        self.named: Dict[str, V] = {}
        self.prior_ops: List[int] = []
        self.binds: List[tuple] = []
        if not dry:
            self.plan = C.c_void_p(self.lib.uavsal_plan_create())
            if not self.plan:
                raise RuntimeError("uavsal_plan_create failed")
            self.err = self.lib.uavsal_plan_error_word(self.plan)

    def place(self, keep_names=()):
        self.arena.close(len(self.ops_meta))
        if self.use_arena:
            keep = [self.named[k].t for k in keep_names if k in self.named]
            self.arena_floats = self.arena.place(len(self.ops_meta), [t for t in keep if isinstance(t, _ArenaRef)])

    def allocate(self, callers):
        self.split_want -= self.no_shadow
        if self.use_arena:
            self.arena.buf = self.torch.empty(max(self.arena_floats, 4), dtype=torch.float32, device=self.device)
            if self.arena_debug:
                self.arena.buf.fill_(float("nan"))
        for k, need in self.scratch_need.items():
            alloc = self.torch.zeros if k[0] == "WV" else self.torch.empty
            self.scratch[k] = alloc(max(need, 4), dtype=torch.float16 if k[0] == "Ds" else torch.float32,
                                    device=self.device)
        for name, (shape, dtype, how) in callers.items():
            if how == "shape":
                t = self.torch.zeros(1024, dtype=dtype, device=self.device)[:1].expand(shape)
            else:
                t = (self.torch.zeros if how == "zeros" else self.torch.empty)(shape, dtype=dtype, device=self.device)
            self.callers[name] = t

    def end(self):
        self._flush_poison(final=True)
        self.arena.recording = False

    def caller(self, name, n, h, w, c) -> V:
        return V(Caller(name, self.callers.get(name), named=name != "logits"), n, h, w, c)

    def _bind(self, v, slot):
        if v is not None and isinstance(v.t, Caller):
            self.binds.append((v.t.name, len(self.ops_meta) - 1, slot, 4 * v.coff))

    def pin(self, *vs):
        if self.use_arena and self.dry:
            for t in {id(v.t): v.t for v in vs}.values():
                self.arena.pin(t)

    def buf(self, name, n, h, w, c, pinned=False) -> V:
        sp = None
        numel = n * h * w * c
        if self.use_arena and not pinned:
            t = self.arena.ref(name, numel)
        elif self.dry:
            t = _Fake()
        else:
            t = self.torch.empty(numel, dtype=torch.float32, device=self.device)
            self.keep.append(t)
        if not self.dry and name in self.split_want and c % 32 == 0:
            sp = self.torch.full((2 * numel,), float("nan"), dtype=torch.float16, device=self.device)
            self.keep.append(sp)
        v = V(t, n, h, w, c, sp=sp, key=name)
        if name:
            self.named[name] = v
        return v

    def _flush_poison(self, final=False):
        if not (self.arena_debug and self.use_arena) or self.dry:
            return
        cur = self.lane
        for r, lane in self.arena.due(final):
            if lane != cur:
                L.check(self.lib.uavsal_plan_set_lane(self.plan, lane), "plan_set_lane")
                cur = lane
            self.op_idx["poison:%s" % (r.aid,)] = len(self.ops_meta)
            if lane == PRIOR_LANE:
                self.prior_ops.append(len(self.ops_meta))
            self.ops_meta.append(dict(kind="poison", name="poison:%s" % (r.aid,), flops=0.0, bytes=4.0 * r.numel_, lane=lane))
            self.op_args.append(dict(kind="poison", name="poison:%s" % (r.aid,)))
            d = L.FillDesc()
            d.out, d.n, d.bits = self.arena.buf.data_ptr() + 4 * r.off, r.numel_, 0x7FC00000
            self._add(self.lib.uavsal_plan_add_fill, d, "plan_add_fill")
        if cur != self.lane:
            L.check(self.lib.uavsal_plan_set_lane(self.plan, self.lane), "plan_set_lane")

    def scr_split(self, n, h, w, c) -> V:
        numel = 2 * n * h * w * c
        k = ("Ds", self.lane)
        if self.dry:
            self.scratch_need[k] = max(self.scratch_need.get(k, 0), numel)
            return V(None, n, h, w, c, sp=_Fake(), key=k)
        return V(None, n, h, w, c, sp=self.scratch[k], key=k)

    def _would_split(self, n_img, h, w, cin, cout, taps, act, has_res, ldc=None, ldr=None) -> bool:
        if not self.split_mode:
            return False
        d = L.ConvDesc()
        P_ = 1 << 20
        d.a, d.lda, d.a_img_stride = P_, cin, h * w
        d.a_split, d.ldas = P_, 2 * cin
        d.w, d.out, d.ldc, d.o_img_stride = P_, P_, (cout if ldc is None else ldc), h * w
        if has_res:
            d.res, d.ldr, d.r_img_stride = P_, (cout if ldr is None else ldr), h * w
        d.n_img, d.H, d.W, d.Cin, d.Cout, d.taps = n_img, h, w, cin, cout, taps
        d.prec, d.act, d.epi, d.tile = self.prec, act, L.EPI_AFFINE, 0
        return L.conv_route(self.lib, d).family == L.ROUTE_PRESPLIT

    def scr(self, kind, n, h, w, c) -> V:
        numel = n * h * w * c
        if self.use_arena:
            return V(self.arena.scratch(kind, numel), n, h, w, c)
        key = (kind, self.lane)
        if self.dry:
            self.scratch_need[key] = max(self.scratch_need.get(key, 0), numel)
            return V(_Fake(), n, h, w, c)
        return V(self.scratch[key], n, h, w, c)

    def fork(self, lane):
        self._meta(kind="sync", name="fork%d" % lane, flops=0.0, bytes=0.0, group_lane=lane)
        self.arena.fork(lane)
        if not self.dry:
            r = self.lib.uavsal_plan_add_fork(self.plan, lane)
            if r < 0:
                L.check(r, "plan_add_fork")
            L.check(self.lib.uavsal_plan_set_lane(self.plan, lane), "plan_set_lane")
        self.lane = self.arena.lane = lane

    def main(self):
        if not self.dry:
            L.check(self.lib.uavsal_plan_set_lane(self.plan, 0), "plan_set_lane")
        self.lane = self.arena.lane = 0

    def join(self, lane):
        self._meta(kind="sync", name="join%d" % lane, flops=0.0, bytes=0.0, group_lane=lane)
        self.arena.join(lane)
        if not self.dry:
            r = self.lib.uavsal_plan_add_join(self.plan, lane)
            if r < 0:
                L.check(r, "plan_add_join")

    def prec_for(self, name) -> str:
        best, val = -1, self.prec_name
        for k, v in self.prec_overrides.items():
            if name.startswith(k) and len(k) > best:
                best, val = len(k), v
        return val

    def _tile_of(self, n_img, h, w, cout, epi) -> int:
        d = L.ConvDesc()
        d.n_img, d.H, d.W, d.Cout, d.prec, d.epi, d.tile = n_img, h, w, cout, self.prec, epi, 0
        d.out = 1 << 20
        return L.conv_route(self.lib, d).tile

    def _meta(self, **kw):
        self._flush_poison()
        self.arena.lop += 1
        if kw.pop("group_lane", self.lane) == PRIOR_LANE:
            self.prior_ops.append(len(self.ops_meta))
        self.op_idx[kw.get("name")] = len(self.ops_meta)
        self.ops_meta.append(kw)
        self.op_args.append(dict(kind=kw.get("kind"), name=kw.get("name")))

    def _ov(self, v, img=None):
        return None if v is None else OpView.of(v, img)

    def _add(self, fn, desc, what):
        r = fn(self.plan, C.byref(desc))
        if r < 0:
            L.check(r, what)

    def conv(self, name, a: V, conv, bn, out: V, act, taps=1, res: Optional[V] = None, wslice=None,
             epi=L.EPI_AFFINE, aux: Optional[V] = None, n_img=None, strides=None, cout=None,
             out2: Optional[V] = None, gate_interleave=0, dw=None, n_group=0):
        cin = a.c
        cout = out.c if cout is None else cout
        n_img = a.n if n_img is None else n_img
        hin, win = a.h, a.w
        a_in = a
        if dw is not None:
            a = V(a.t, a.n, (hin - 1) // dw[2] + 1, (win - 1) // dw[2] + 1, a.c, a.ld, a.coff)
        hw = a.h * a.w
        flops = 2.0 * n_img * hw * cin * cout * taps
        byts = 4.0 * n_img * hw * (cin + cout) + 4.0 * cin * cout * taps
        if dw is not None:
            flops += 18.0 * n_img * hw * cin
            byts = 4.0 * n_img * (hin * win * cin + hw * cout) + 4.0 * cin * (cout + 11)
        self._meta(kind="conv%d" % (3 if taps == 9 else 1), name=name, flops=flops, bytes=byts,
                   M=n_img * hw, K=cin * taps, Nc=cout)
        self.arena.touch(a, out, res, aux, out2)
        shadow_out = False
        if self.split_mode:
            aligned = cout % 4 == 0 and out.ld % 4 == 0 and (res is None or res.ld % 4 == 0)
            if epi == L.EPI_AFFINE:
                shadow_out = aligned and act != L.ACT_SIGMOID
            elif epi == L.EPI_TWA:
                shadow_out = aligned and self._tile_of(n_img, a.h, a.w, cout, epi) in (3, 4)
            if self.dry:
                if not shadow_out and out.key is not None:
                    self.no_shadow.add(out.key)
                if (a.key is not None and a.key not in self.no_shadow and dw is None and strides is None
                        and epi == L.EPI_AFFINE and a.ld % 32 == 0 and (a.coff % a.ld) % 32 == 0 and self._would_split(
                            n_img, a.h, a.w, cin, cout, taps, act, res is not None, out.ld, res.ld if res is not None else None)):
                    self.split_want.add(a.key)
        if self.dry:
            return
        d = L.ConvDesc()
        st = strides or {}
        d.a, d.lda, d.a_img_stride = a.ptr, a.ld, st.get("a", hin * win if dw is not None else hw)
        self._bind(a, SLOT_CONV_A)
        self._bind(out, SLOT_CONV_OUT)
        if a.sp is not None and dw is None and strides is None and epi == L.EPI_AFFINE:
            d.a_split, d.ldas = a.sp_ptr, 2 * a.ld
        if out.sp is not None and shadow_out:
            d.out_split, d.ldos = out.sp_ptr, 2 * out.ld
        if dw is not None:
            w9, s_, b_ = self.weights.depthwise(dw[0], dw[1])
            d.dw_w9c, d.dw_scale, d.dw_bias = w9.data_ptr(), s_.data_ptr(), b_.data_ptr()
            d.dw_stride, d.dw_Hin, d.dw_Win = dw[2], hin, win
            self.ops_meta[-1]["fused_dw"] = True
        if bn is not None:
            s, b = self.weights.affine(bn, cout)
            d.scale, d.bias = s.data_ptr(), b.data_ptr()
        else:
            d.scale, d.bias = None, None
        d.out, d.ldc, d.o_img_stride = out.ptr, out.ld, st.get("o", hw)
        if res is not None:
            d.res, d.ldr, d.r_img_stride = res.ptr, res.ld, st.get("r", hw)
        else:
            d.res, d.ldr, d.r_img_stride = None, 0, hw
        if aux is not None:
            d.aux, d.ldx, d.x_img_stride = aux.ptr, aux.ld, st.get("x", hw)
        else:
            d.aux, d.ldx, d.x_img_stride = None, 0, hw
        d.n_img, d.H, d.W = n_img, a.h, a.w
        d.Cin, d.Cout, d.taps = cin, cout, taps
        pn = self.prec_for(name)
        d.prec, d.act, d.epi, d.tile = L.PREC[pn], act, epi, 0
        d.n_group, d.a_group_off = n_group, (cin if n_group else 0)
        if self.lane != 0 and pn == "f32" and epi == L.EPI_AFFINE and dw is None and cin % 32 == 0:
            d.tile = 11
        if out2 is not None:
            d.out2, d.ld2 = out2.ptr, out2.ld
        if self.stream_k:
            ws = self.sk_ws.get(self.lane)
            if ws is None:
                ws = self.sk_ws[self.lane] = self.torch.zeros(int(self.lib.uavsal_streamk_workspace_bytes()),
                                                           dtype=torch.uint8, device=self.device)
            d.sk_ws, d.sk_ws_bytes = ws.data_ptr(), ws.numel()
        d.err = self.err
        d.sk_spin_limit, d.sk_debug_drop = self.sk_debug
        d.w = 1 << 20
        route = L.conv_route(self.lib, d)
        split, dwproj, tile = route.family == L.ROUTE_PRESPLIT, route.dwproj, route.tile
        if a.t is None and not split:
            raise RuntimeError("%s: its input only exists as a split shadow but the GEMM is not eligible" % name)
        ksize = (conv[0] if isinstance(conv, (list, tuple)) else conv).weight.shape[-1]
        d.w = self.weights.conv(conv, wslice, gate_interleave, conv_weight_layout(pn, split, dwproj != 0, tile, ksize)).data_ptr()
        self.ops_meta[-1]["prec"] = pn
        self.ops_meta[-1]["split"] = split
        self.ops_meta[-1]["tile"] = tile
        self.ops_meta[-1]["streamk"] = route.streamk
        self.ops_meta[-1]["dwproj"] = dwproj
        groups = cout // n_group if n_group else 1
        ad = self._ov(V(a_in.t, n_img, hin, win, cin + (groups - 1) * cin, a_in.ld, a_in.coff, a_in.sp, a_in.key),
                      d.a_img_stride)
        if not split:
            ad.sp = None
        od = self._ov(out, d.o_img_stride)
        if not d.out_split:
            od.sp = None
        self.op_args[-1].update(conv=conv, bn=bn, act=act, epi=epi, taps=taps, wslice=wslice, gate_interleave=gate_interleave,
                                n_group=n_group, dw=dw, prec=pn, split_in=split, cin=cin, cout=cout, a=ad, out=od,
                                res=self._ov(res, d.r_img_stride), aux=self._ov(aux, d.x_img_stride),
                                out2=self._ov(out2, d.o_img_stride))
        self._add(self.lib.uavsal_plan_add_conv, d, "plan_add_conv(%s)" % name)

    def conv3_wino(self, name, a: V, conv, bn, out: V, act, wslice=None, n_img=None, strides=None, twa=None, gemm_tile=0, r=2):
        cin, cout = a.c, out.c
        n = a.n if n_img is None else n_img
        hw = a.h * a.w
        tiles = n * ((a.h + r - 1) // r) * ((a.w + r - 1) // r)
        pp = (r + 2) * (r + 2)
        mp = roundup(tiles, 128)
        st = strides or {}
        v = self.scr("WV", pp, mp, 1, cin)
        mm = self.scr("WM", pp, mp, 1, cout)
        self._meta(kind="wino_in", name=name + ".xin", flops=0.0, bytes=4.0 * n * hw * cin + 4.0 * float(pp) * tiles * cin)
        self.op_args[-1].update(triple=name + ".xout")
        self.arena.touch(a, v)
        if not self.dry:
            wi = L.WinoDesc()
            wi.inp, wi.ldi, wi.in_img_stride = a.ptr, a.ld, st.get("a", hw)
            wi.out, wi.ldo = v.ptr, cin
            wi.n_img, wi.H, wi.W, wi.C, wi.Mp, wi.R = n, a.h, a.w, cin, mp, r
            self._add(self.lib.uavsal_plan_add_wino_input, wi, "plan_add_wino_input(%s)" % name)
        self._meta(kind="conv1", name=name, flops=2.0 * pp * tiles * cin * cout,
                   bytes=4.0 * pp * (tiles * (cin + cout) + cin * cout), M=pp * mp, K=cin, Nc=cout,
                   direct_flops=2.0 * n * hw * cin * cout * 9)
        self.arena.touch(v, mm)
        self.op_args[-1].update(triple=name + ".xout")
        if not self.dry:
            d = L.ConvDesc()
            d.a, d.lda, d.a_img_stride = v.ptr, cin, mp
            d.w, d.w_group_stride = self.weights.wino(conv, wslice, r).data_ptr(), roundup(cout, 32) * roundup(cin, 32)
            d.out, d.ldc, d.o_img_stride = mm.ptr, cout, mp
            d.n_img, d.H, d.W, d.Cin, d.Cout, d.taps = pp, mp, 1, cin, cout, 1
            d.prec, d.act, d.epi, d.tile = L.PREC["f32"], L.ACT_NONE, L.EPI_AFFINE, gemm_tile
            d.err = self.err
            m_ = self.ops_meta[-1]
            m_["split"], m_["tile"], m_["streamk"], m_["dwproj"] = False, L.conv_route(self.lib, d).tile, 0, 0
            m_["prec"] = "f32"
            self._add(self.lib.uavsal_plan_add_conv, d, "plan_add_conv(%s)" % name)
        self._meta(kind="wino_out", name=name + ".xout", flops=0.0, bytes=4.0 * (float(pp) * tiles * cout + n * hw * cout))
        self.arena.touch(mm, out, *(twa or ()), *((a,) if twa is not None else ()))
        if out.key is not None and self.dry:
            self.no_shadow.add(out.key)
        if not self.dry:
            wo = L.WinoDesc()
            wo.inp, wo.ldi = mm.ptr, cout
            wo.out, wo.ldo, wo.out_img_stride = out.ptr, out.ld, st.get("o", hw)
            wo.n_img, wo.H, wo.W, wo.C, wo.Mp, wo.R = n, a.h, a.w, cout, mp, r
            if bn is not None:
                s_, b_ = self.weights.affine(bn, cout)
                wo.scale, wo.bias = s_.data_ptr(), b_.data_ptr()
            wo.act, wo.epi = act, L.EPI_AFFINE
            if twa is not None:
                xt, pre = twa
                wo.epi = L.EPI_TWA
                wo.res, wo.ldr, wo.res_img_stride = xt.ptr, xt.ld, st.get("r", hw)
                wo.aux, wo.ldx, wo.aux_img_stride = pre.ptr, pre.ld, st.get("x", hw)
                wo.hprev, wo.ldh, wo.h_img_stride = a.ptr, a.ld, st.get("a", hw)
            ai = st.get("a", hw)
            self.op_args[-1].update(kind="wino", triple_first=name + ".xin", conv=conv, bn=bn, act=act, wslice=wslice, r=r, cin=cin,
                                    cout=cout, a=self._ov(a, ai), segs=None, out=self._ov(out, wo.out_img_stride),
                                    twa=None if twa is None else (self._ov(twa[0], wo.res_img_stride), self._ov(twa[1], wo.aux_img_stride)))
            self._add(self.lib.uavsal_plan_add_wino_output, wo, "plan_add_wino_output(%s)" % name)

    def dw(self, name, a: V, conv, bn, out: V, stride, dilation):
        c = a.c
        ho, wo = (a.h - 1) // stride + 1, (a.w - 1) // stride + 1
        byts = 4.0 * a.n * c * (a.h * a.w + ho * wo) + 4.0 * 9 * c + 4.0 * 2 * c
        self._meta(kind="dw", name=name, flops=2.0 * 9 * a.n * ho * wo * c, bytes=byts, stride=stride,
                   dil=dilation if not isinstance(dilation, (list, tuple)) else tuple(dilation), patches44=a.n * ((ho + 3) // 4) * ((wo + 3) // 4) * (c // 4))
        self.arena.touch(a, out)
        if self.dry:
            return
        grouped = isinstance(conv, (list, tuple))
        w9, s, b = self.weights.depthwise(conv, bn)
        d = L.DwDesc()
        if grouped:
            d.dil_group_c = c // len(conv)
            for gi, dl in enumerate(dilation):
                d.dil_groups[gi] = dl
            dilation = dilation[0]
        d.inp, d.ldi = a.ptr, a.ld
        d.w9c, d.scale, d.bias = w9.data_ptr(), s.data_ptr(), b.data_ptr()
        if out.t is None:
            d.out, d.ldo = None, out.ld
            d.out_split, d.ldos = out.sp_ptr, 2 * out.ld
            self.ops_meta[-1]["split_out"] = True
        else:
            d.out, d.ldo = out.ptr, out.ld
        d.n_img, d.H, d.W, d.C = a.n, a.h, a.w, c
        d.stride, d.dilation, d.act = stride, dilation, L.ACT_RELU6
        self.ops_meta[-1]["kernel"] = L.DW_KERNEL.get(int(self.lib.uavsal_dw_variant(C.byref(d))), "dw3x3")
        self.op_args[-1].update(conv=conv, bn=bn, stride=stride, dilation=(tuple(d.dil_groups[:len(conv)]) if grouped else dilation),
                                a=self._ov(a), out=self._ov(out))
        self._add(self.lib.uavsal_plan_add_dw, d, "plan_add_dw(%s)" % name)

    def dw_dot(self, name, a: V, dwc, dwbn, pl, plbn, out: V, act):
        c = a.c
        self._meta(kind="dw_dot", name=name, flops=2.0 * 10 * a.n * a.h * a.w * c, bytes=4.0 * a.n * a.h * a.w * (c + 1) + 4.0 * 12 * c,
                   stride=1, dil=1, kernel="dw3x3_dot_kernel<4, 4>")
        self.arena.touch(a, out)
        if self.dry:
            return
        w9, s, b, w2, s2, b2 = self.weights.dw_dot(dwc, dwbn, pl, plbn)
        d = L.DwDotDesc()
        d.inp, d.ldi = a.ptr, a.ld
        d.w9c, d.scale, d.bias, d.w2, d.scale2, d.bias2 = (t.data_ptr() for t in (w9, s, b, w2, s2, b2))
        d.out, d.ldo = out.ptr, out.ld
        self._bind(out, SLOT_CONV_OUT)
        d.n_img, d.H, d.W, d.C, d.act = a.n, a.h, a.w, c, act
        self.op_args[-1].update(dw=(dwc, dwbn), conv=pl, bn=plbn, act=act, a=self._ov(a), out=self._ov(out))
        self._add(self.lib.uavsal_plan_add_dw_dot, d, "plan_add_dw_dot(%s)" % name)

    def bilinear(self, name, a: V, out: V, src_mod=None, src_div=1):
        self._meta(kind="bilinear", name=name, flops=0.0, bytes=4.0 * out.n * out.h * out.w * out.c * 2)
        self.arena.touch(a, out)
        if self.dry:
            return
        d = L.BilinearDesc()
        d.inp, d.ldi, d.Hi, d.Wi = a.ptr, a.ld, a.h, a.w
        d.out, d.ldo, d.Ho, d.Wo = out.ptr, out.ld, out.h, out.w
        d.n_out, d.C = out.n, a.c
        if out.sp is not None:
            d.out_split, d.ldos = out.sp_ptr, 2 * out.ld
        d.src_mod, d.src_div = (out.n if src_mod is None else src_mod), src_div
        self.op_args[-1].update(a=self._ov(a), out=self._ov(out), src_mod=d.src_mod, src_div=src_div)
        self._add(self.lib.uavsal_plan_add_bilinear, d, "plan_add_bilinear(%s)" % name)

    def layout(self, name, src: V, dst: V, to_nhwc, cpad=0):
        nhwc, nchw = (dst, src) if to_nhwc else (src, dst)
        n, c, hw = nhwc.n, nhwc.c, nhwc.h * nhwc.w
        self._meta(kind="layout", name=name, flops=0.0, bytes=8.0 * n * c * hw)
        self.arena.touch(src, dst)
        if self.dry:
            return
        d = L.LayoutDesc()
        d.inp, d.out, d.n_img, d.C, d.HW, d.ld, d.to_nhwc, d.Cpad = src.ptr, dst.ptr, n, c, hw, nhwc.ld, to_nhwc, cpad
        self._bind(src, SLOT_LAYOUT_IN)
        self._bind(dst, SLOT_LAYOUT_OUT)
        ov = self._ov(nhwc)
        cv = OpView(nchw.t.name, nchw.coff, n, nhwc.h, nhwc.w, c, c, hw, nchw=True)
        self.op_args[-1].update(to_nhwc=to_nhwc, cpad=cpad, a=cv if to_nhwc else ov, out=ov if to_nhwc else cv)
        self._add(self.lib.uavsal_plan_add_layout, d, "plan_add_layout(%s)" % name)

    def stem(self, name, x: V, conv0, bn0, out: V, u8):
        self._meta(kind="stem", name=name, flops=2.0 * 27 * 32 * out.n * out.h * out.w,
                   bytes=(1.0 if u8 else 4.0) * x.n * 3 * x.h * x.w + 4.0 * out.n * out.h * out.w * 32)
        self.arena.touch(out)
        if self.dry:
            return
        ws, ss, bs = self.weights.stem(conv0, bn0)
        d = L.StemDesc()
        d.inp, d.in_u8 = (None, x.ptr) if u8 else (x.ptr, None)
        self._bind(x, SLOT_STEM_U8 if u8 else SLOT_STEM_F32)
        d.w, d.scale, d.bias = ws.data_ptr(), ss.data_ptr(), bs.data_ptr()
        d.out, d.ldo = out.ptr, 32
        d.n_img, d.H, d.W = x.n, x.h, x.w
        for i in range(3):
            d.mean[i], d.stdv[i] = synth.IMAGENET_MEAN[i], synth.IMAGENET_STD[i]
        self.op_args[-1].update(conv=conv0, bn=bn0, u8=u8, mean=tuple(synth.IMAGENET_MEAN), stdv=tuple(synth.IMAGENET_STD),
                                a=OpView(x.t.name, 0, x.n, x.h, x.w, 3, 3, 0, nchw=True), out=self._ov(out))
        self._add(self.lib.uavsal_plan_add_stem, d, "plan_add_stem")

    def tdiff(self, name, a: V, out: V, seq_len):
        self._meta(kind="tdiff", name=name, flops=0.0, bytes=4.0 * a.n * a.h * a.w * (a.c + out.c))
        self.arena.touch(a, out)
        if self.dry:
            return
        d = L.TdiffDesc()
        d.inp, d.ldi, d.out, d.ldo = a.ptr, a.ld, out.ptr, out.ld
        d.n_img, d.HW, d.C, d.seq_len = a.n, a.h * a.w, a.c, seq_len
        self.op_args[-1].update(a=self._ov(a), out=self._ov(out), seq_len=seq_len)
        self._add(self.lib.uavsal_plan_add_tdiff, d, "plan_add_tdiff")

    def tsum(self, name, a: V, out: V, T):
        self._meta(kind="tsum", name=name, flops=0.0, bytes=4.0 * (a.n + out.n) * a.h * a.w * out.c)
        self.arena.touch(a, out)
        if self.dry:
            return
        d = L.TsumDesc()
        d.inp, d.ldi, d.out, d.ldo = a.ptr, a.ld, out.ptr, out.ld
        d.n_groups, d.T, d.HW, d.C = out.n, T, a.h * a.w, out.c
        self.op_args[-1].update(a=self._ov(a), out=self._ov(out), T=T)
        self._add(self.lib.uavsal_plan_add_tsum, d, "plan_add_tsum")

    def copy(self, name, hist: V, keep: V, seq_len):
        hw, n = hist.h * hist.w, keep.n
        self._meta(kind="copy", name=name, flops=0.0, bytes=8.0 * n * hist.c * hw)
        self.arena.touch(hist, keep)
        if self.dry:
            return
        d = L.CopyDesc()
        d.inp, d.out = hist.frames(seq_len - 1, 1).ptr, keep.ptr
        d.in_pitch, d.out_pitch, d.row_floats, d.rows = seq_len * hw * hist.c, hw * hist.c, hw * hist.c, n
        self.op_args[-1].update(a=self._ov(hist.frames(seq_len - 1, n), seq_len * hw), out=self._ov(keep))
        self._add(self.lib.uavsal_plan_add_copy, d, "plan_add_copy")

    def guard(self, *bufs):
        self._meta(kind="guard", name="guard", flops=0.0, bytes=0.0)
        self.arena.touch(*bufs)
        if self.dry:
            return
        args = []
        for slot, v in enumerate((bufs + (None, None))[:3]):
            args += [None, 0] if v is None else [v.ptr, v.n * v.h * v.w * v.c]
            self._bind(v, slot)
        r = self.lib.uavsal_plan_add_guard(self.plan, *args)
        if r < 0:
            L.check(r, "plan_add_guard")

    def fused_block(self, name, x: V, blk, out: V) -> bool:
        if not self.fuse_blocks or getattr(blk, "dilation", 1) != 1:
            return False
        d = L.FusedIrDesc()
        d.Cin, d.hidden, d.Cout, d.stride = x.c, blk.hidden, out.c, blk.stride
        d.w1 = (1 << 20) if blk.expand_ratio != 1 else None
        kind = int(self.lib.uavsal_fused_ir_supported(C.byref(d)))
        if not kind:
            return False
        natural = kind == 2
        if natural:
            wgs = x.n * ((x.h + 3) // 4) * ((x.w + 7) // 8)
            if not (MID_MIN_WGS <= wgs <= MID_MAX_WGS):
                return False
        ho, wo = (x.h - 1) // blk.stride + 1, (x.w - 1) // blk.stride + 1
        self._meta(kind="fused_ir", name=name, kernel="%s<%d, %d, %d%s>" % ("fused_mid_kernel" if natural else "fused_ir_kernel", x.c, blk.hidden, out.c,
                                                                    "" if natural else ", %d" % blk.stride),
                   flops=2.0 * x.n * ((x.h * x.w * x.c * blk.hidden if blk.expand_ratio != 1 else 0)
                                      + ho * wo * blk.hidden * (9 + out.c)),
                   bytes=4.0 * x.n * (x.h * x.w * x.c + ho * wo * out.c * (2 if blk.use_res_connect else 1)),
                   unfused_bytes=4.0 * x.n * (x.h * x.w * (x.c + (2 * blk.hidden if blk.expand_ratio != 1 else 0))
                                              + ho * wo * (2 * blk.hidden + out.c)),
                   **({"flops_executed": 2.0 * wgs * blk.hidden * (64 * x.c + 32 * out.c)} if natural else {}))
        self.arena.touch(x, out)
        if out.key is not None:
            self.no_shadow.add(out.key)
        if self.dry:
            return True
        ws = self.weights.fused_block(blk, natural)
        d.inp, d.ldi = x.ptr, x.ld
        if "w1" in ws:
            d.w1, d.scale1, d.bias1 = ws["w1"].data_ptr(), ws["s1"].data_ptr(), ws["b1"].data_ptr()
        d.wd, d.scale_d, d.bias_d = ws["wd"].data_ptr(), ws["sd"].data_ptr(), ws["bd"].data_ptr()
        d.w2, d.scale2, d.bias2 = ws["w2"].data_ptr(), ws["s2"].data_ptr(), ws["b2"].data_ptr()
        if blk.use_res_connect:
            d.res, d.ldr = x.ptr, x.ld
        d.out, d.ldo = out.ptr, out.ld
        d.n_img, d.H, d.W = x.n, x.h, x.w
        self.op_args[-1].update(blk=blk, a=self._ov(x), out=self._ov(out), res=self._ov(x) if blk.use_res_connect else None)
        self._add(self.lib.uavsal_plan_add_fused_ir, d, "plan_add_fused_ir(%s)" % name)
        return True

    def ir_block(self, name, x: V, blk, out: V, final_act=L.ACT_NONE, expanded: Optional[V] = None):
        if expanded is None and final_act == L.ACT_NONE and self.fused_block(name, x, blk, out):
            return
        if (expanded is None and blk.expand_ratio != 1 and x.n > 1 and self.use_arena and out.c > 1
                and 4 * x.n * x.h * x.w * blk.hidden > BLOCK_CHUNK_BYTES):
            per = 4 * x.h * x.w * blk.hidden
            step = max(1, BLOCK_CHUNK_BYTES // per)
            nchunk = (x.n + step - 1) // step
            step = (x.n + nchunk - 1) // nchunk
            for ci, f0 in enumerate(range(0, x.n, step)):
                cnt = min(step, x.n - f0)
                self._ir_block_one("%s#%d" % (name, ci) if nchunk > 1 else name, x.frames(f0, cnt), blk, out.frames(f0, cnt), final_act)
            return
        self._ir_block_one(name, x, blk, out, final_act, expanded)

    def _ir_block_one(self, name, x: V, blk, out: V, final_act=L.ACT_NONE, expanded: Optional[V] = None):
        seq = blk.conv
        stride, dil = blk.stride, getattr(blk, "dilation", 1)
        if blk.expand_ratio != 1:
            if expanded is not None:
                e = expanded
            else:
                e = self.scr("E", x.n, x.h, x.w, blk.hidden)
                self.conv(name + ".pw", x, seq[0][0], seq[0][1], e, L.ACT_RELU6)
            dwc, dwbn, pl, plbn = seq[1][0], seq[1][1], seq[2], seq[3]
        else:
            e = x
            dwc, dwbn, pl, plbn = seq[0][0], seq[0][1], seq[1], seq[2]
        ho, wo = (x.h - 1) // stride + 1, (x.w - 1) // stride + 1
        if (out.c == 1 and stride == 1 and dil == 1 and blk.expand_ratio != 1 and not blk.use_res_connect
                and blk.hidden % 256 == 0 and blk.hidden <= 2048 and self.fuse_dw is not False):
            self.dw_dot(name + ".dwpl", e, dwc, dwbn, pl, plbn, out, final_act)
            return
        if dil == 1 and blk.expand_ratio != 1 and (self.fuse_dw or (
                self.fuse_dw is None and self.prec_for(name + ".dwpl") in ("f32", "f16x3") and stride == 1 and blk.hidden % 16 == 0
                and x.n * x.h * x.w * blk.hidden >= FUSE_DW_MIN_WORK and _dwproj_patch_waste(x.h, x.w) <= FUSE_DW_MAX_WASTE)):
            self.conv(name + ".dwpl", e, pl, plbn, out, final_act, res=x if blk.use_res_connect else None,
                      dw=(dwc, dwbn, stride))
            return
        res = x if blk.use_res_connect else None
        if dil == 1 and self._would_split(x.n, ho, wo, blk.hidden, out.c, 1, final_act, res is not None, out.ld,
                                          res.ld if res is not None else None):
            dd = self.scr_split(x.n, ho, wo, blk.hidden)
        else:
            dd = self.scr("D", x.n, ho, wo, blk.hidden)
        self.dw(name + ".dw", e, dwc, dwbn, dd, stride, dil)
        self.conv(name + ".pl", dd, pl, plbn, out, final_act, res=res)

    def mark(self, stage, start):
        self.stage_ranges[stage] = (start, len(self.ops_meta))
```

include/uavsal_hip.h:

```cpp
#ifndef UAVSAL_HIP_H
#define UAVSAL_HIP_H

#include <stdint.h>

#ifdef __cplusplus
extern "C" {
#endif

#define UAVSAL_ABI_VERSION 20

#define UAVSAL_EINVAL   (-1)
#define UAVSAL_EALIGN   (-2)
#define UAVSAL_ESHAPE   (-3)
#define UAVSAL_ESTATE   (-4)
#define UAVSAL_EDEVICE  (-5)

#define UAVSAL_ERR_STREAMK  1

#define UAVSAL_PREC_F32     0
#define UAVSAL_PREC_BF16X3  1
#define UAVSAL_PREC_BF16    2
#define UAVSAL_PREC_F16X3   3

#define UAVSAL_ACT_NONE     0
#define UAVSAL_ACT_RELU6    1
#define UAVSAL_ACT_SIGMOID  2

#define UAVSAL_EPI_AFFINE   0
#define UAVSAL_EPI_TWA      1
#define UAVSAL_EPI_LSTM     2

typedef void* uavsal_stream_t;

typedef struct uavsal_conv_desc {
    const float* a;      int32_t lda;  int64_t a_img_stride;
    const void*  w;
    const float* scale;  const float* bias;
    float*       out;    int32_t ldc;  int64_t o_img_stride;
    const float* res;    int32_t ldr;  int64_t r_img_stride;
    const float* aux;    int32_t ldx;  int64_t x_img_stride;
    int32_t n_img, H, W;
    int32_t Cin, Cout, taps;
    int32_t prec, act, epi;
    int32_t tile;
    float*       out2;   int32_t ld2;
    const float* dw_w9c; const float* dw_scale; const float* dw_bias;
    int32_t dw_stride, dw_Hin, dw_Win;
    void* sk_ws; int64_t sk_ws_bytes;
    const void* a_split;  int32_t ldas;
    void* out_split;      int32_t ldos;
    int32_t* err;
    int32_t sk_spin_limit;
    int32_t sk_debug_drop;
    int64_t w_group_stride;
    int32_t n_group, a_group_off;
} uavsal_conv_desc;

int uavsal_conv_gemm(const uavsal_conv_desc* d, uavsal_stream_t stream);
long long uavsal_streamk_workspace_bytes(void);

enum { UAVSAL_ROUTE_PRESPLIT = 1, UAVSAL_ROUTE_DWPROJ, UAVSAL_ROUTE_STREAMK, UAVSAL_ROUTE_K32, UAVSAL_ROUTE_F32_DMA,
       UAVSAL_ROUTE_STAGED };
enum { UAVSAL_REDUCE_NONE = 0, UAVSAL_REDUCE_LAUNCH, UAVSAL_REDUCE_IN_LAUNCH };
typedef struct uavsal_conv_route {
    int32_t family;
    int32_t tile;
    int32_t dwproj;
    int32_t streamk;
    int32_t ksplit;
    int32_t reduce;
} uavsal_conv_route;
int uavsal_conv_route_of(const uavsal_conv_desc* d, uavsal_conv_route* r);
int uavsal_conv_tile(const uavsal_conv_desc* d);
int uavsal_conv_uses_split(const uavsal_conv_desc* d);
int uavsal_conv_dwproj(const uavsal_conv_desc* d);
int uavsal_conv_streamk_grid(const uavsal_conv_desc* d);

typedef struct uavsal_dw_desc {
    const float* in;   int32_t ldi;
    const float* w9c;  const float* scale;  const float* bias;
    float*       out;  int32_t ldo;
    int32_t n_img, H, W, C, stride, dilation, act;
    void* out_split;  int32_t ldos;
    int32_t dil_group_c;  int32_t dil_groups[4];
} uavsal_dw_desc;

int uavsal_dw3x3(const uavsal_dw_desc* d, uavsal_stream_t stream);
int uavsal_dw_variant(const uavsal_dw_desc* d);

typedef struct uavsal_dw_dot_desc {
    const float* in;   int32_t ldi;
    const float* w9c;  const float* scale;  const float* bias;
    const float* w2;   const float* scale2; const float* bias2;
    float*       out;  int32_t ldo;
    int32_t n_img, H, W, C, act;
} uavsal_dw_dot_desc;

int uavsal_dw3x3_dot(const uavsal_dw_dot_desc* d, uavsal_stream_t stream);

typedef struct uavsal_fused_ir_desc {
    const float* in;   int32_t ldi;
    const float* w1;   const float* scale1;  const float* bias1;
    const float* wd;   const float* scale_d; const float* bias_d;
    const float* w2;   const float* scale2;  const float* bias2;
    const float* res;  int32_t ldr;
    float*       out;  int32_t ldo;
    int32_t n_img, H, W, Cin, hidden, Cout, stride;
    int32_t tile;
} uavsal_fused_ir_desc;

int uavsal_fused_ir(const uavsal_fused_ir_desc* d, uavsal_stream_t stream);
int uavsal_fused_ir_supported(const uavsal_fused_ir_desc* d);

typedef struct uavsal_stem_desc {
    const float*   in;
    const uint8_t* in_u8;
    const float* w;  const float* scale;  const float* bias;
    float* out;  int32_t ldo;
    int32_t n_img, H, W;
    float mean[3], stdv[3];
} uavsal_stem_desc;

int uavsal_stem_conv(const uavsal_stem_desc* d, uavsal_stream_t stream);

typedef struct uavsal_bilinear_desc {
    const float* in;  int32_t ldi;  int32_t Hi, Wi;
    float* out;       int32_t ldo;  int32_t Ho, Wo;
    int32_t n_out, C, src_mod, src_div;
    void* out_split;  int32_t ldos;
} uavsal_bilinear_desc;

int uavsal_bilinear_ac(const uavsal_bilinear_desc* d, uavsal_stream_t stream);

typedef struct uavsal_tdiff_desc {
    const float* in;  int32_t ldi;
    float* out;       int32_t ldo;
    int32_t n_img, HW, C, seq_len;
} uavsal_tdiff_desc;

int uavsal_tdiff(const uavsal_tdiff_desc* d, uavsal_stream_t stream);

typedef struct uavsal_wino_desc {
    const float* in;   int32_t ldi;  int64_t in_img_stride;
    float* out;        int32_t ldo;  int64_t out_img_stride;
    int32_t n_img, H, W, C;
    int64_t Mp;
    int32_t R;
    const float* scale; const float* bias;
    int32_t act, epi;
    const float* res;   int32_t ldr;  int64_t res_img_stride;
    const float* aux;   int32_t ldx;  int64_t aux_img_stride;
    const float* hprev; int32_t ldh;  int64_t h_img_stride;
    int32_t n_seg;
    const float* seg_in[3];  int32_t seg_ld[3], seg_c[3], seg_H[3], seg_W[3];
} uavsal_wino_desc;

int uavsal_wino_input(const uavsal_wino_desc* d, uavsal_stream_t stream);
int uavsal_wino_output(const uavsal_wino_desc* d, uavsal_stream_t stream);

typedef struct uavsal_tsum_desc {
    const float* in;  int32_t ldi;
    float* out;       int32_t ldo;
    int32_t n_groups, T, HW, C;
} uavsal_tsum_desc;

int uavsal_tsum(const uavsal_tsum_desc* d, uavsal_stream_t stream);

typedef struct uavsal_layout_desc {
    const float* in;  float* out;
    int32_t n_img, C, HW, ld, to_nhwc, Cpad;
} uavsal_layout_desc;

int uavsal_layout(const uavsal_layout_desc* d, uavsal_stream_t stream);

typedef struct uavsal_post_desc {
    const float* in;  uint8_t* out;  void* scratch;
    int32_t n_img, h, w, H, W;
} uavsal_post_desc;

int uavsal_postprocess(const uavsal_post_desc* d, uavsal_stream_t stream);

#define UAVSAL_LETTERBOX_HWC 0
#define UAVSAL_LETTERBOX_CHW 1

typedef struct uavsal_letterbox_desc {
    const uint8_t* src;  uint8_t* dst;
    int64_t row_pitch, plane_pitch, img_pitch;
    int32_t n_img, h0, w0, R, C;
    int32_t layout, swap_rb;
} uavsal_letterbox_desc;

int uavsal_letterbox_u8(const uavsal_letterbox_desc* d, uavsal_stream_t stream);

typedef struct uavsal_overlay_desc {
    const uint8_t* frames;  int64_t row_pitch, plane_pitch, img_pitch;
    const uint8_t* map;  int64_t map_img_pitch;
    const uint8_t* fix;  const uint8_t* lut;
    uint8_t* out;  void* ws;  int64_t ws_bytes;
    int32_t n_img, layout, h0, w0, map_h, map_w, fix_h, fix_w;
    int32_t mid_h, mid_w, out_h, out_w;
} uavsal_overlay_desc;

int64_t uavsal_overlay_workspace_bytes(const uavsal_overlay_desc* d);
int uavsal_overlay_u8(const uavsal_overlay_desc* d, uavsal_stream_t stream);

typedef struct uavsal_copy_desc {
    const float* in;  float* out;
    int64_t in_pitch, out_pitch, row_floats;  int32_t rows;
} uavsal_copy_desc;

int uavsal_copy_rows(const uavsal_copy_desc* d, uavsal_stream_t stream);

typedef struct uavsal_fill_desc {
    uint32_t* out;  int64_t n;  uint32_t bits;
} uavsal_fill_desc;

int uavsal_fill(const uavsal_fill_desc* d, uavsal_stream_t stream);

typedef struct uavsal_guard_desc {
    const int32_t* err;  int32_t* host_err;
    float* buf[3];  int64_t n[3];
} uavsal_guard_desc;

int uavsal_guard(const uavsal_guard_desc* d, uavsal_stream_t stream);

#define UAVSAL_SCORE_NSTAT 16
#define UAVSAL_SCORE_REPS  100
#define UAVSAL_SCORE_RUN   4096
#define UAVSAL_SCORE_NKEY  7

typedef struct uavsal_score_desc {
    const void* sal;  const void* fix_loc;  const float* fix_map;
    const float* jitter;
    int32_t sal_u8, loc_u8, n_frames, n_pix;
    double* stats;
    const int64_t* fix_off;  const int64_t* run_off;  int64_t total_fix;  int32_t total_runs;
    int32_t nan_rows;
    const int32_t* samp[2];  const int64_t* samp_off[2];  int64_t n_samp[2];
    void* ws;  int64_t ws_bytes;
    float* out;  int32_t n_keys;  int32_t keys[UAVSAL_SCORE_NKEY];
} uavsal_score_desc;

int64_t uavsal_score_workspace_bytes(const uavsal_score_desc* d);
int uavsal_score_stats(const uavsal_score_desc* d, uavsal_stream_t stream);
int uavsal_score_run(const uavsal_score_desc* d, uavsal_stream_t stream);

typedef struct uavsal_gaze_desc {
    const uint8_t* fix_map;  int64_t map_row_pitch, map_col_pitch, map_img_pitch;
    const uint8_t* fix_loc;  int64_t loc_row_pitch, loc_col_pitch, loc_img_pitch;
    float* out;  uint8_t* flags;
    int32_t n_img, h0, w0, h, w;
} uavsal_gaze_desc;

int uavsal_gaze_prepare(const uavsal_gaze_desc* d, uavsal_stream_t stream);

#define UAVSAL_LOSS_NSTAT 16

typedef struct uavsal_loss_desc {
    const float* pred;  const float* truth;
    double* stats;
    float* out;
    const float* grad_out;  float* grad;
    int32_t n_img, n_pix;
    double w_kl, w_cc, w_nss;
} uavsal_loss_desc;

int uavsal_loss_fu(const uavsal_loss_desc* d, uavsal_stream_t stream);
int uavsal_loss_fu_grad(const uavsal_loss_desc* d, uavsal_stream_t stream);

#define UAVSAL_PRIOR_MIN_SLAB 32

typedef struct uavsal_prior_acc_desc {
    const uint8_t* frames;  int64_t row_pitch, col_pitch, img_pitch;
    int32_t* acc;  int64_t acc_row_pitch, acc_col_pitch;
    int32_t n_img, h0, w0;
} uavsal_prior_acc_desc;

typedef struct uavsal_prior_finish_desc {
    const int32_t* acc;  int64_t acc_row_pitch, acc_col_pitch;
    int32_t* ws;
    uint8_t* out;
    uint8_t* image;
    int32_t n_frames, h0, w0, h, w;
} uavsal_prior_finish_desc;

int uavsal_prior_accumulate(const uavsal_prior_acc_desc* d, uavsal_stream_t stream);
int uavsal_prior_finish(const uavsal_prior_finish_desc* d, uavsal_stream_t stream);
int uavsal_prior_slab_frames(int64_t plane_pixels, int32_t n_img);
int uavsal_prior_sizeof_desc(int which);

#define UAVSAL_WGRAD_CHAIN 1024

typedef struct uavsal_twa_gate_desc {
    const float* g;      int32_t ldg;
    const float* carry;
    const float* z;
    const float* x;      int32_t ldx;
    const float* hprev;  int32_t ldh;
    float* dz;  float* carry_out;  float* dx;
    int64_t n_pix;  int32_t C;
} uavsal_twa_gate_desc;

typedef struct uavsal_twa_wgrad_desc {
    const float* dz;
    const float* x;      int32_t ldx;
    const float* h;      int32_t ldh;
    const float* h0;     int32_t ldh0;
    float* ws;  int64_t ws_bytes;
    float* out;
    int32_t T, H, W, C, accumulate;
} uavsal_twa_wgrad_desc;

typedef struct uavsal_dec_bwd_desc {
    const float* gy;  int64_t gy_img_pitch, gy_row_pitch, gy_col_pitch;
    const float* y;
    const float* e;  const float* d;
    const float* s1;  const float* wd9;  const float* s2;  const float* w3;  const float* s3;
    float* ge;
    int32_t n_img, H, W, C;
} uavsal_dec_bwd_desc;

int uavsal_twa_gate_bwd(const uavsal_twa_gate_desc* d, uavsal_stream_t stream);
int64_t uavsal_twa_wgrad_workspace_bytes(const uavsal_twa_wgrad_desc* d);
int uavsal_twa_wgrad_shares(const uavsal_twa_wgrad_desc* d);
int uavsal_twa_wgrad(const uavsal_twa_wgrad_desc* d, uavsal_stream_t stream);
int uavsal_dec_bwd(const uavsal_dec_bwd_desc* d, uavsal_stream_t stream);
int uavsal_train_sizeof_desc(int which);

#define UAVSAL_DEC_NSUM 12

typedef struct uavsal_pix_gemm_desc {
    const float* a;  int32_t lda;
    const float* b;  int32_t ldb;
    const float* row_scale;
    const float* w;  int32_t ldw;
    double* rowdot;
    float* ws;  int64_t ws_bytes;
    float* out;  int32_t ldo;
    int64_t K;  int32_t M, N, accumulate;
} uavsal_pix_gemm_desc;

typedef struct uavsal_dec_sums_desc {
    const float* gy;  int64_t gy_img_pitch, gy_row_pitch, gy_col_pitch;
    const float* y;
    const float* e;  const float* d;  const float* ga;
    const float* w3;  const float* s3;
    double* ws;  int64_t ws_bytes;
    int32_t n_img, H, W, C;
} uavsal_dec_sums_desc;

typedef struct uavsal_dec_finish_desc {
    const double* ws;  int64_t ws_bytes;  const double* rowdot;
    const float* wd;  const float* w3;  const float* s2;  const float* s3;
    const float* r1;  const float* mu1;  const float* r2;  const float* mu2;  const float* r3;  const float* mu3;
    float* g_gamma1;  float* g_beta1;  float* g_wd;  float* g_gamma2;  float* g_beta2;
    float* g_w3;  float* g_gamma3;  float* g_beta3;
    int32_t C, slabs, accumulate;
} uavsal_dec_finish_desc;

int64_t uavsal_pix_gemm_workspace_bytes(const uavsal_pix_gemm_desc* d);
int uavsal_pix_gemm_shares(const uavsal_pix_gemm_desc* d);
int uavsal_pix_gemm(const uavsal_pix_gemm_desc* d, uavsal_stream_t stream);
int64_t uavsal_dec_sums_workspace_bytes(const uavsal_dec_sums_desc* d);
int uavsal_dec_sums_slabs(const uavsal_dec_sums_desc* d);
int uavsal_dec_sums_slab_rows(const uavsal_dec_sums_desc* d);
int uavsal_dec_sums(const uavsal_dec_sums_desc* d, uavsal_stream_t stream);
int uavsal_dec_finish(const uavsal_dec_finish_desc* d, uavsal_stream_t stream);
int uavsal_train_decoder_sizeof_desc(int which);

#define UAVSAL_IR_NSUM 11

typedef struct uavsal_ir_bwd_desc {
    const float* gd;  const float* d;  const float* e;
    const float* wd9;  const float* s2;
    float* ga;
    int32_t n_img, H, W, C;
} uavsal_ir_bwd_desc;

typedef struct uavsal_ir_sums_desc {
    const float* gd;  const float* d;  const float* e;  const float* ga;
    const float* go;  int32_t ldgo;
    double* ws;  int64_t ws_bytes;
    int32_t n_img, H, W, Ch, Co;
} uavsal_ir_sums_desc;

typedef struct uavsal_ir_finish_desc {
    const double* ws;  int64_t ws_bytes;  const double* rowdot1;  const double* rowdot3;
    const float* wd;  const float* s2;
    const float* r1;  const float* mu1;  const float* r2;  const float* mu2;  const float* r3;  const float* mu3;
    float* g_gamma1;  float* g_beta1;  float* g_wd;  float* g_gamma2;  float* g_beta2;  float* g_gamma3;  float* g_beta3;
    int32_t Ch, Co, slabs, accumulate;
} uavsal_ir_finish_desc;

int uavsal_ir_bwd(const uavsal_ir_bwd_desc* d, uavsal_stream_t stream);
int64_t uavsal_ir_sums_workspace_bytes(const uavsal_ir_sums_desc* d);
int uavsal_ir_sums_slabs(const uavsal_ir_sums_desc* d);
int uavsal_ir_sums_slab_rows(const uavsal_ir_sums_desc* d);
int uavsal_ir_sums(const uavsal_ir_sums_desc* d, uavsal_stream_t stream);
int uavsal_ir_finish(const uavsal_ir_finish_desc* d, uavsal_stream_t stream);
int uavsal_block_sizeof_desc(int which);

typedef struct uavsal_ir_bwd_s2_desc {
    const float* gd;  const float* d;
    const float* e;
    const float* wd9;  const float* s2;
    float* ga;
    int32_t n_img, H, W, C;
} uavsal_ir_bwd_s2_desc;

typedef struct uavsal_bilinear_bwd_desc {
    const float* gout;  int32_t ldo;  int32_t Ho, Wo;
    float* gin;         int32_t Hi, Wi;
    int32_t n_out, n_src, C, src_mod, src_div;
} uavsal_bilinear_bwd_desc;

typedef struct uavsal_tsum_bwd_desc {
    const float* a;  int32_t lda;
    const float* g;  int32_t ldg;
    float* out;      int32_t ldo;
    int32_t n_groups, T, HW, C;
} uavsal_tsum_bwd_desc;

int uavsal_ir_bwd_s2(const uavsal_ir_bwd_s2_desc* d, uavsal_stream_t stream);
int uavsal_bilinear_ac_bwd(const uavsal_bilinear_bwd_desc* d, uavsal_stream_t stream);
int uavsal_tsum_bwd(const uavsal_tsum_bwd_desc* d, uavsal_stream_t stream);
int uavsal_ctx_sizeof_desc(int which);

typedef struct uavsal_ir_sums_s2_desc {
    const float* gd;  const float* d;
    const float* e;  const float* ga;
    const float* go;  int32_t ldgo;
    double* ws;  int64_t ws_bytes;
    int32_t n_img, H, W, Ch, Co;
} uavsal_ir_sums_s2_desc;

int64_t uavsal_ir_sums_s2_workspace_bytes(const uavsal_ir_sums_s2_desc* d);
int uavsal_ir_sums_s2_slabs(const uavsal_ir_sums_s2_desc* d);
int uavsal_ir_sums_s2_slab_rows(const uavsal_ir_sums_s2_desc* d);
int uavsal_ir_sums_s2(const uavsal_ir_sums_s2_desc* d, uavsal_stream_t stream);
int uavsal_mp_sizeof_desc(int which);

#define UAVSAL_NARROW_CHUNK 32

typedef struct uavsal_ir_narrow_desc {
    const float* x;
    const float* e;  const float* d;  const float* gd;  const float* ga;
    const float* go;  int32_t ldgo;
    double* ws;  int64_t ws_bytes;
    int32_t n_img, H, W, Cin, Ch, Co;
} uavsal_ir_narrow_desc;

typedef struct uavsal_ir_narrow_finish_desc {
    const double* ws;  int64_t ws_bytes;
    const float* w1;  const float* wd;  const float* w3;
    const float* s1;  const float* s2;  const float* s3;
    const float* r1;  const float* mu1;  const float* r2;  const float* mu2;  const float* r3;  const float* mu3;
    float* g_w1;  float* g_gamma1;  float* g_beta1;  float* g_wd;  float* g_gamma2;  float* g_beta2;
    float* g_w3;  float* g_gamma3;  float* g_beta3;
    int32_t Cin, Ch, Co, slabs, accumulate;
} uavsal_ir_narrow_finish_desc;

typedef struct uavsal_frame_sum_desc {
    const float* a;  int32_t lda;
    float* out;      int32_t ldo;
    int32_t N, HW, C;
} uavsal_frame_sum_desc;

int64_t uavsal_ir_narrow_workspace_bytes(const uavsal_ir_narrow_desc* d);
int uavsal_ir_narrow_slabs(const uavsal_ir_narrow_desc* d);
int uavsal_ir_narrow_slab_rows(const uavsal_ir_narrow_desc* d);
int uavsal_ir_narrow_grads(const uavsal_ir_narrow_desc* d, uavsal_stream_t stream);
int uavsal_ir_narrow_finish(const uavsal_ir_narrow_finish_desc* d, uavsal_stream_t stream);
int uavsal_frame_sum(const uavsal_frame_sum_desc* d, uavsal_stream_t stream);
int uavsal_nets_sizeof_desc(int which);

#define UAVSAL_REPACK_MAX_SRC 4
#define UAVSAL_REPACK_MAX_BLOCKS (1 << 24)
enum { UAVSAL_REPACK_CONV = 0, UAVSAL_REPACK_WINO = 1, UAVSAL_REPACK_FOLD = 2, UAVSAL_REPACK_DW = 3, UAVSAL_REPACK_COPY = 4 };
enum { UAVSAL_REPACK_F32 = 0, UAVSAL_REPACK_F16X3 = 1, UAVSAL_REPACK_F16X3I = 2, UAVSAL_REPACK_F16X3J = 3, UAVSAL_REPACK_BF16 = 4,
       UAVSAL_REPACK_BF16X3 = 5 };
enum { UAVSAL_REPACK_SCALE = 0, UAVSAL_REPACK_BIAS = 1, UAVSAL_REPACK_RSTD = 2, UAVSAL_REPACK_MEAN = 3 };

typedef struct uavsal_repack_entry {
    int32_t kind, layout;
    void* dst;
    int64_t units;
    const float* src[UAVSAL_REPACK_MAX_SRC];
    const float* beta[UAVSAL_REPACK_MAX_SRC];
    const float* mean[UAVSAL_REPACK_MAX_SRC];
    const float* var[UAVSAL_REPACK_MAX_SRC];
    double eps[UAVSAL_REPACK_MAX_SRC];
    int32_t rows[UAVSAL_REPACK_MAX_SRC];
    int32_t n_src;
    int32_t N, C, taps, Npad, Kpad, kt, flip, gi;
    int32_t P;
    int64_t sN, sC, off;
    const float* sg;  const float* sv;  double seps;
    float pad;  int32_t reserved;
    double G[18];
} uavsal_repack_entry;

int uavsal_repack(const void* table, int n_entries, int n_blocks, uavsal_stream_t stream);
int uavsal_repack_sizeof_desc(void);

typedef struct uavsal_plan uavsal_plan;

uavsal_plan* uavsal_plan_create(void);
void uavsal_plan_destroy(uavsal_plan* p);
int uavsal_plan_add_conv(uavsal_plan* p, const uavsal_conv_desc* d);
int uavsal_plan_add_dw(uavsal_plan* p, const uavsal_dw_desc* d);
int uavsal_plan_add_dw_dot(uavsal_plan* p, const uavsal_dw_dot_desc* d);
int uavsal_plan_add_stem(uavsal_plan* p, const uavsal_stem_desc* d);
int uavsal_plan_add_bilinear(uavsal_plan* p, const uavsal_bilinear_desc* d);
int uavsal_plan_add_tdiff(uavsal_plan* p, const uavsal_tdiff_desc* d);
int uavsal_plan_add_wino_input(uavsal_plan* p, const uavsal_wino_desc* d);
int uavsal_plan_add_wino_output(uavsal_plan* p, const uavsal_wino_desc* d);
int uavsal_plan_add_tsum(uavsal_plan* p, const uavsal_tsum_desc* d);
int uavsal_plan_add_layout(uavsal_plan* p, const uavsal_layout_desc* d);
int uavsal_plan_add_copy(uavsal_plan* p, const uavsal_copy_desc* d);
int uavsal_plan_add_fused_ir(uavsal_plan* p, const uavsal_fused_ir_desc* d);
int uavsal_plan_add_fill(uavsal_plan* p, const uavsal_fill_desc* d);
int32_t* uavsal_plan_error_word(uavsal_plan* p);
int uavsal_plan_add_guard(uavsal_plan* p, float* b0, int64_t n0, float* b1, int64_t n1, float* b2, int64_t n2);
int uavsal_plan_status(uavsal_plan* p, int wait);
int uavsal_plan_patch_ptr(uavsal_plan* p, int op, int slot, void* ptr);
int uavsal_plan_set_lane(uavsal_plan* p, int lane);
int uavsal_plan_add_fork(uavsal_plan* p, int lane);
int uavsal_plan_add_join(uavsal_plan* p, int lane);
int uavsal_plan_enable_lanes(uavsal_plan* p, int on);
int uavsal_plan_size(const uavsal_plan* p);
int uavsal_plan_run(uavsal_plan* p, int first, int last, uavsal_stream_t stream);
int uavsal_plan_group_mark(uavsal_plan* p, int group, int first, int last);
int uavsal_plan_group_enable(uavsal_plan* p, int group, int on);
int uavsal_plan_group_launches(const uavsal_plan* p, int group);
int uavsal_plan_last_launches(const uavsal_plan* p);
int uavsal_plan_frame_repeat(uavsal_plan* p, int op_pw, int op_dwpl, int src_mod, int src_div, int on);
int uavsal_plan_frame_repeat_workgroups(const uavsal_plan* p, int which);
int uavsal_plan_graph_build(uavsal_plan* p, uavsal_stream_t stream);
int uavsal_plan_graph_launch(uavsal_plan* p, uavsal_stream_t stream);

int uavsal_plan_time(uavsal_plan* p, int first, int last, int iters, uavsal_stream_t stream, float* ms);

int uavsal_abi_version(void);
int uavsal_sizeof_desc(int which);
const char* uavsal_build_info(void);

#ifdef __cplusplus
}
#endif
#endif
```

Measured before the change: 1971 frames/s.

## Fuse Winograd output/input seams in TWA recurrence and skip zero-state step

```diff
diff --git a/iip_uavsal_saliency_amd/_lib.py b/iip_uavsal_saliency_amd/_lib.py
--- a/iip_uavsal_saliency_amd/_lib.py
+++ b/iip_uavsal_saliency_amd/_lib.py
@@ -422,6 +422,10 @@
     ("uavsal_plan_add_fused_ir", C.c_int, [C.c_void_p, C.POINTER(FusedIrDesc)]),
     ("uavsal_wino_input", C.c_int, [C.POINTER(WinoDesc), C.c_void_p]),
     ("uavsal_wino_output", C.c_int, [C.POINTER(WinoDesc), C.c_void_p]),
+    ("uavsal_wino_output_zero_h", C.c_int, [C.POINTER(WinoDesc), C.c_void_p]),
+    ("uavsal_wino_seam", C.c_int, [C.POINTER(WinoDesc), C.POINTER(WinoDesc), C.c_void_p]),
+    ("uavsal_wino_seam_zero_h", C.c_int, [C.POINTER(WinoDesc), C.POINTER(WinoDesc), C.c_void_p]),
+    ("uavsal_wino_seam_check", C.c_int, [C.POINTER(WinoDesc), C.POINTER(WinoDesc)]),
     ("uavsal_plan_add_wino_input", C.c_int, [C.c_void_p, C.POINTER(WinoDesc)]),
     ("uavsal_plan_add_wino_output", C.c_int, [C.c_void_p, C.POINTER(WinoDesc)]),
     ("uavsal_plan_add_copy", C.c_int, [C.c_void_p, C.POINTER(CopyDesc)]),
@@ -451,6 +455,9 @@
     ("uavsal_plan_last_launches", C.c_int, [C.c_void_p]),
     ("uavsal_plan_frame_repeat", C.c_int, [C.c_void_p, C.c_int, C.c_int, C.c_int, C.c_int, C.c_int]),
     ("uavsal_plan_frame_repeat_workgroups", C.c_int, [C.c_void_p, C.c_int]),
+    ("uavsal_plan_seam", C.c_int, [C.c_void_p, C.c_int, C.c_int, C.c_int]),
+    ("uavsal_plan_zero_state", C.c_int, [C.c_void_p, C.c_int, C.c_int, C.c_int, C.c_int, C.c_int, C.c_int]),
+    ("uavsal_plan_mode_report", C.c_int, [C.c_void_p, C.POINTER(C.c_int * 4)]),
     ("uavsal_plan_graph_build", C.c_int, [C.c_void_p, C.c_void_p]),
     ("uavsal_plan_graph_launch", C.c_int, [C.c_void_p, C.c_void_p]),
     ("uavsal_plan_time", C.c_int, [C.c_void_p, C.c_int, C.c_int, C.c_int, C.c_void_p, C.POINTER(C.c_float)]),
diff --git a/iip_uavsal_saliency_amd/csrc/plan.hip b/iip_uavsal_saliency_amd/csrc/plan.hip
--- a/iip_uavsal_saliency_amd/csrc/plan.hip
+++ b/iip_uavsal_saliency_amd/csrc/plan.hip
@@ -69,6 +69,10 @@
     int fr_pw = -1, fr_dw = -1, fr_mod = 0, fr_div = 0;
     bool fr_on = false;
     int fr_wg[2] = {0, 0};
+    std::vector<int> seam_next;
+    int zs_first = -1, zs_last = -1, zs_xin = -1, zs_gemm = -1, zs_xout = -1;
+    bool zs_on = false;
+    int mode_seams = 0, mode_elided = 0, mode_kernels = 0;
 };
 
 extern "C" uavsal_plan* uavsal_plan_create(void) { return new (std::nothrow) uavsal_plan(); }
@@ -256,6 +260,18 @@
         fr = cs == hipStreamCaptureStatusNone && !(a.group >= 0 && ((goff >> a.group) & 1u)) && !(b.group >= 0 && ((goff >> b.group) & 1u)) &&
              uavsal_conv_repeat_pair(&a.u.conv, &b.u.conv, p->fr_mod, p->fr_div) == 1;
     }
+    bool modes = repeat && (p->zs_on || !p->seam_next.empty());
+    if (modes) {
+        hipStreamCaptureStatus cs = hipStreamCaptureStatusNone;
+        if (hipStreamIsCapturing((hipStream_t)stream, &cs) != hipSuccess) { (void)hipGetLastError(); cs = hipStreamCaptureStatusActive; }
+        modes = cs == hipStreamCaptureStatusNone;
+    }
+    const uint32_t moff = masked ? p->groups_off : 0u;
+    auto masked_out = [&](int i) { return p->ops[i].group >= 0 && ((moff >> p->ops[i].group) & 1u); };
+    bool zs = modes && p->zs_on && p->zs_xin >= first && p->zs_xout < last && (p->zs_first < 0 || (p->zs_first >= first && p->zs_last < last)) &&
+              !masked_out(p->zs_xin) && !masked_out(p->zs_gemm) && !masked_out(p->zs_xout);
+    for (int i = p->zs_first; zs && i >= 0 && i <= p->zs_last; ++i) zs = !masked_out(i);
+    if (repeat && first == 0) p->mode_seams = p->mode_elided = p->mode_kernels = 0;
     const bool lanes = p->lanes_on && first == 0 && last == n;
     const uint32_t off = masked ? p->groups_off : 0u;
     hipStream_t main_s = (hipStream_t)stream;
@@ -279,12 +295,31 @@
         uavsal_stream_t s = (lanes && op.lane > 0) ? (uavsal_stream_t)p->side[op.lane] : stream;
         if (lanes && op.lane > 0 && !p->side[op.lane]) return UAVSAL_ESTATE;
         int e;
+        if (zs && ((p->zs_first >= 0 && i >= p->zs_first && i <= p->zs_last) || i == p->zs_xin || i == p->zs_gemm)) {
+            ++p->mode_elided;
+            ++*launched;
+            continue;
+        }
+        const bool seam = modes && i < (int)p->seam_next.size() && p->seam_next[i] == i + 1 && i + 1 < last && !masked_out(i + 1) &&
+                          p->ops[i + 1].lane == op.lane;
+        if (seam) {
+            const bool zh = zs && i == p->zs_xout;
+            e = zh ? uavsal_wino_seam_zero_h(&op.u.wino, &p->ops[i + 1].u.wino, s) : uavsal_wino_seam(&op.u.wino, &p->ops[i + 1].u.wino, s);
+            if (e) return e;
+            ++p->mode_seams; ++p->mode_kernels;
+            *launched += 2;
+            ++i;
+            continue;
+        }
         if (repeat && (i == p->fr_pw || i == p->fr_dw))
             e = uavsal_conv_gemm_mapped(&op.u.conv, s, fr ? p->fr_mod : 0, fr ? p->fr_div : 0, &p->fr_wg[i == p->fr_dw]);
+        else if (zs && i == p->zs_xout)
+            e = uavsal_wino_output_zero_h(&op.u.wino, s);
         else
             e = run_op(op, s);
         if (e) return e;
         ++*launched;
+        if (repeat) ++p->mode_kernels;
     }
     if (last == n) {
         hipStreamCaptureStatus cs = hipStreamCaptureStatusNone;
@@ -314,6 +349,45 @@
     return p->fr_on ? 1 : 0;
 }
 
+extern "C" int uavsal_plan_seam(uavsal_plan* p, int op_xout, int op_xin, int on) {
+    const int n = p ? (int)p->ops.size() : 0;
+    if (!p || op_xout < 0 || op_xin < 0 || op_xout >= n || op_xin >= n) return UAVSAL_EINVAL;
+    if (p->ops[op_xout].kind != OP_WINO_OUT || p->ops[op_xin].kind != OP_WINO_IN) return UAVSAL_EINVAL;
+    if ((int)p->seam_next.size() < n) p->seam_next.resize(n, -1);
+    p->seam_next[op_xout] = -1;
+    if (!on || p->exec || op_xin != op_xout + 1 || p->ops[op_xin].lane != p->ops[op_xout].lane ||
+        uavsal_wino_seam_check(&p->ops[op_xout].u.wino, &p->ops[op_xin].u.wino) != 0)
+        return 0;
+    p->seam_next[op_xout] = op_xin;
+    return 1;
+}
+
+extern "C" int uavsal_plan_zero_state(uavsal_plan* p, int op_state_in_first, int op_state_in_last, int op_xin0, int op_gemm0,
+                                      int op_xout0, int on) {
+    const int n = p ? (int)p->ops.size() : 0;
+    if (!p || op_xin0 < 0 || op_gemm0 != op_xin0 + 1 || op_xout0 != op_gemm0 + 1 || op_xout0 >= n) return UAVSAL_EINVAL;
+    if ((op_state_in_first < 0) != (op_state_in_last < 0) || op_state_in_last < op_state_in_first || op_state_in_last >= op_xin0)
+        return UAVSAL_EINVAL;
+    const Op& xi = p->ops[op_xin0];
+    const Op& g = p->ops[op_gemm0];
+    const Op& xo = p->ops[op_xout0];
+    if (xi.kind != OP_WINO_IN || g.kind != OP_CONV || xo.kind != OP_WINO_OUT) return UAVSAL_EINVAL;
+    for (int i = op_state_in_first; i >= 0 && i <= op_state_in_last; ++i)
+        if (p->ops[i].kind != OP_LAYOUT) return UAVSAL_EINVAL;
+    p->zs_first = op_state_in_first; p->zs_last = op_state_in_last;
+    p->zs_xin = op_xin0; p->zs_gemm = op_gemm0; p->zs_xout = op_xout0;
+    p->zs_on = on != 0 && !p->exec && xi.u.wino.R == 2 && xo.u.wino.R == 2 && xo.u.wino.epi == UAVSAL_EPI_TWA &&
+               xi.u.wino.n_seg == 0 && xi.u.wino.in == xo.u.wino.hprev && g.u.conv.a == xi.u.wino.out && g.u.conv.out == xo.u.wino.in &&
+               xi.lane == xo.lane && g.lane == xo.lane;
+    return p->zs_on ? 1 : 0;
+}
+
+extern "C" int uavsal_plan_mode_report(const uavsal_plan* p, int out[4]) {
+    if (!p || !out) return UAVSAL_EINVAL;
+    out[0] = p->mode_seams; out[1] = p->mode_elided; out[2] = p->mode_kernels; out[3] = 0;
+    return 0;
+}
+
 extern "C" int uavsal_plan_frame_repeat_workgroups(const uavsal_plan* p, int which) {
     return p && (which == 0 || which == 1) ? p->fr_wg[which] : UAVSAL_EINVAL;
 }
@@ -322,6 +396,8 @@
     if (!p) return UAVSAL_EINVAL;
     if (p->exec) return 0;
     p->fr_on = false;
+    p->zs_on = false;
+    p->seam_next.clear();
     hipStream_t s = (hipStream_t)stream;
     hipError_t e = hipStreamBeginCapture(s, hipStreamCaptureModeThreadLocal);
     if (e != hipSuccess) return (int)e;
diff --git a/iip_uavsal_saliency_amd/csrc/winograd.hip b/iip_uavsal_saliency_amd/csrc/winograd.hip
--- a/iip_uavsal_saliency_amd/csrc/winograd.hip
+++ b/iip_uavsal_saliency_amd/csrc/winograd.hip
@@ -136,8 +136,32 @@
 }
 
 template <int R>
+__device__ __forceinline__ void wino_tile_out(const float* mi, size_t plane, f32x4 (&y)[R][R]) {
+    constexpr int P = WinoT<R>::P;
+    f32x4 s[R][P];
+#pragma unroll
+    for (int j = 0; j < P; ++j) {
+        f32x4 col[P], sc_[R];
+#pragma unroll
+        for (int i = 0; i < P; ++i) col[i] = *reinterpret_cast<const f32x4*>(mi + (size_t)(P * i + j) * plane);
+        WinoT<R>::at(col, sc_);
+#pragma unroll
+        for (int a = 0; a < R; ++a) s[a][j] = sc_[a];
+    }
+#pragma unroll
+    for (int a = 0; a < R; ++a) WinoT<R>::at(s[a], y[a]);
+}
+
+__device__ __forceinline__ f32x4 twa_gate(f32x4 v, f32x4 pre, f32x4 xt, f32x4 hp) {
+    const f32x4 g = sigmoid4(v + pre);
+    f32x4 h;
+    h.x = fmaf(g.x, xt.x, __fmul_rn(1.f - g.x, hp.x)); h.y = fmaf(g.y, xt.y, __fmul_rn(1.f - g.y, hp.y));
+    h.z = fmaf(g.z, xt.z, __fmul_rn(1.f - g.z, hp.z)); h.w = fmaf(g.w, xt.w, __fmul_rn(1.f - g.w, hp.w));
+    return h;
+}
+
+template <int R, bool ZH>
 __global__ __launch_bounds__(256) void wino_output_kernel(const WinoK p) {
-    constexpr int P = WinoT<R>::P;
     const long long idx = (long long)blockIdx.x * 256 + threadIdx.x;
     if (idx >= p.total) return;
     const int c4 = (int)(idx % p.C4);
@@ -146,21 +170,15 @@
     const int n = (int)(tile / tpi);
     const int r = (int)(tile - (long long)n * tpi);
     const int tyi = r / p.tx, txi = r - tyi * p.tx;
-    const float* mi = p.in + (size_t)tile * p.ldi + c4 * 4;
-    const size_t plane = (size_t)p.Mp * p.ldi;
-    f32x4 s[R][P];
-#pragma unroll
-    for (int j = 0; j < P; ++j) {
-        f32x4 col[P], sc_[R];
-#pragma unroll
-        for (int i = 0; i < P; ++i) col[i] = *reinterpret_cast<const f32x4*>(mi + (size_t)(P * i + j) * plane);
-        WinoT<R>::at(col, sc_);
-#pragma unroll
-        for (int a = 0; a < R; ++a) s[a][j] = sc_[a];
-    }
     f32x4 y[R][R];
-#pragma unroll
-    for (int a = 0; a < R; ++a) WinoT<R>::at(s[a], y[a]);
+    if (ZH) {
+#pragma unroll
+        for (int a = 0; a < R; ++a)
+#pragma unroll
+            for (int b = 0; b < R; ++b) y[a][b] = (f32x4){0.f, 0.f, 0.f, 0.f};
+    } else {
+        wino_tile_out<R>(p.in + (size_t)tile * p.ldi + c4 * 4, (size_t)p.Mp * p.ldi, y);
+    }
     f32x4 sc = {1.f, 1.f, 1.f, 1.f}, bi = {0.f, 0.f, 0.f, 0.f};
     if (p.scale) {
         sc = *reinterpret_cast<const f32x4*>(p.scale + c4 * 4);
@@ -175,12 +193,12 @@
             if (yy >= p.H || xx >= p.W) continue;
             const size_t pix = (size_t)yy * p.W + xx;
             f32x4 v = y[a][b];
-            if (p.epi == UAVSAL_EPI_TWA) {
-                const f32x4 z = v + *reinterpret_cast<const f32x4*>(p.aux + ((size_t)n * p.aux_is + pix) * p.ldx + c4 * 4);
+            if (ZH || p.epi == UAVSAL_EPI_TWA) {
+                const f32x4 pre = *reinterpret_cast<const f32x4*>(p.aux + ((size_t)n * p.aux_is + pix) * p.ldx + c4 * 4);
                 const f32x4 xt = *reinterpret_cast<const f32x4*>(p.res + ((size_t)n * p.res_is + pix) * p.ldr + c4 * 4);
-                const f32x4 hp = *reinterpret_cast<const f32x4*>(p.hprev + ((size_t)n * p.h_is + pix) * p.ldh + c4 * 4);
-                const f32x4 g = sigmoid4(z);
-                v = g * xt + (1.f - g) * hp;
+                const f32x4 hp = ZH ? (f32x4){0.f, 0.f, 0.f, 0.f}
+                                    : *reinterpret_cast<const f32x4*>(p.hprev + ((size_t)n * p.h_is + pix) * p.ldh + c4 * 4);
+                v = twa_gate(v, pre, xt, hp);
             } else {
                 v.x = __builtin_amdgcn_fmed3f(fmaf(v.x, sc.x, bi.x), lo, hi); v.y = __builtin_amdgcn_fmed3f(fmaf(v.y, sc.y, bi.y), lo, hi);
                 v.z = __builtin_amdgcn_fmed3f(fmaf(v.z, sc.z, bi.z), lo, hi); v.w = __builtin_amdgcn_fmed3f(fmaf(v.w, sc.w, bi.w), lo, hi);
@@ -188,6 +206,91 @@
             }
             *reinterpret_cast<f32x4*>(p.out + ((size_t)n * p.out_is + pix) * p.ldo + c4 * 4) = v;
         }
+}
+
+struct SeamK {
+    WinoK o;
+    float* v;
+    int ldv;
+    int bx, by, slabs;
+};
+constexpr int SEAM_TY = 4, SEAM_TX = 4;
+constexpr int SEAM_Q = 16;
+constexpr int SEAM_PY = 2 * SEAM_TY + 2, SEAM_PX = 2 * SEAM_TX + 2;
+constexpr int SEAM_NT = ((SEAM_TY + 2) * (SEAM_TX + 2) * SEAM_Q + 63) / 64 * 64;
+static_assert(SEAM_NT <= 1024 && SEAM_PY * SEAM_PX * SEAM_Q * 16 <= 65536, "seam block");
+
+template <bool ZH>
+__global__ __launch_bounds__(SEAM_NT) void wino_seam_kernel(const SeamK k) {
+    __shared__ f32x4 hs[SEAM_PY * SEAM_PX * SEAM_Q];
+    const WinoK& p = k.o;
+    int b = blockIdx.x;
+    const int slab = b % k.slabs; b /= k.slabs;
+    const int bxi = b % k.bx; b /= k.bx;
+    const int byi = b % k.by;
+    const int n = b / k.by;
+    const int q0 = slab * SEAM_Q;
+    const int S = min(SEAM_Q, p.C4 - q0);
+    const size_t mplane = (size_t)p.Mp * p.ldi;
+    const f32x4 zero = {0.f, 0.f, 0.f, 0.f};
+    for (int it = threadIdx.x; it < (SEAM_TY + 2) * (SEAM_TX + 2) * S; it += SEAM_NT) {
+        const int q = it % S, lt = it / S;
+        const int lty = lt / (SEAM_TX + 2), ltx = lt - lty * (SEAM_TX + 2);
+        const int tyi = SEAM_TY * byi - 1 + lty, txi = SEAM_TX * bxi - 1 + ltx;
+        const bool real = tyi >= 0 && tyi < p.ty && txi >= 0 && txi < p.tx;
+        const int c4 = q0 + q;
+        f32x4 y[2][2] = {{zero, zero}, {zero, zero}};
+        if (real && !ZH) {
+            const size_t tile = ((size_t)n * p.ty + tyi) * p.tx + txi;
+            wino_tile_out<2>(p.in + tile * p.ldi + c4 * 4, mplane, y);
+        }
+        const bool own = lty >= 1 && lty <= SEAM_TY && ltx >= 1 && ltx <= SEAM_TX;
+#pragma unroll
+        for (int a = 0; a < 2; ++a)
+#pragma unroll
+            for (int c = 0; c < 2; ++c) {
+                const int ly = 2 * lty + a - 1, lx = 2 * ltx + c - 1;
+                if (ly < 0 || ly >= SEAM_PY || lx < 0 || lx >= SEAM_PX) continue;
+                const int yy = 2 * tyi + a, xx = 2 * txi + c;
+                f32x4 h = zero;
+                if (real && yy < p.H && xx < p.W) {
+                    const size_t pix = (size_t)yy * p.W + xx;
+                    const f32x4 pre = *reinterpret_cast<const f32x4*>(p.aux + ((size_t)n * p.aux_is + pix) * p.ldx + c4 * 4);
+                    const f32x4 xt = *reinterpret_cast<const f32x4*>(p.res + ((size_t)n * p.res_is + pix) * p.ldr + c4 * 4);
+                    const f32x4 hp = ZH ? zero : *reinterpret_cast<const f32x4*>(p.hprev + ((size_t)n * p.h_is + pix) * p.ldh + c4 * 4);
+                    h = twa_gate(y[a][c], pre, xt, hp);
+                    if (own) *reinterpret_cast<f32x4*>(p.out + ((size_t)n * p.out_is + pix) * p.ldo + c4 * 4) = h;
+                }
+                hs[(ly * SEAM_PX + lx) * SEAM_Q + q] = h;
+            }
+    }
+    __syncthreads();
+    for (int it = threadIdx.x; it < SEAM_TY * SEAM_TX * S; it += SEAM_NT) {
+        const int q = it % S, lt = it / S;
+        const int ity = lt / SEAM_TX, itx = lt - ity * SEAM_TX;
+        const int tyi = SEAM_TY * byi + ity, txi = SEAM_TX * bxi + itx;
+        if (tyi >= p.ty || txi >= p.tx) continue;
+        f32x4 t[4][4];
+#pragma unroll
+        for (int j = 0; j < 4; ++j) {
+            f32x4 col[4], tc[4];
+#pragma unroll
+            for (int i = 0; i < 4; ++i) col[i] = hs[((2 * ity + i) * SEAM_PX + 2 * itx + j) * SEAM_Q + q];
+            WinoT<2>::bt(col, tc);
+#pragma unroll
+            for (int i = 0; i < 4; ++i) t[i][j] = tc[i];
+        }
+        const size_t tile = ((size_t)n * p.ty + tyi) * p.tx + txi;
+        float* o = k.v + tile * k.ldv + (q0 + q) * 4;
+        const size_t plane = (size_t)p.Mp * k.ldv;
+#pragma unroll
+        for (int i = 0; i < 4; ++i) {
+            f32x4 v[4];
+            WinoT<2>::bt(t[i], v);
+#pragma unroll
+            for (int j = 0; j < 4; ++j) *reinterpret_cast<f32x4*>(o + (size_t)(4 * i + j) * plane) = v[j];
+        }
+    }
 }
 
 int fill(const uavsal_wino_desc* d, WinoK& k, bool input) {
@@ -268,7 +371,55 @@
     WinoK k;
     const int e = fill(d, k, false);
     if (e) return e;
-    if (d->R == 4) hipLaunchKernelGGL(wino_output_kernel<4>, dim3((unsigned)((k.total + 255) / 256)), dim3(256), 0, (hipStream_t)stream, k);
-    else hipLaunchKernelGGL(wino_output_kernel<2>, dim3((unsigned)((k.total + 255) / 256)), dim3(256), 0, (hipStream_t)stream, k);
+    if (d->R == 4) hipLaunchKernelGGL((wino_output_kernel<4, false>), dim3((unsigned)((k.total + 255) / 256)), dim3(256), 0, (hipStream_t)stream, k);
+    else hipLaunchKernelGGL((wino_output_kernel<2, false>), dim3((unsigned)((k.total + 255) / 256)), dim3(256), 0, (hipStream_t)stream, k);
     return uavsal_launch_status();
 }
+
+extern "C" int uavsal_wino_output_zero_h(const uavsal_wino_desc* d, uavsal_stream_t stream) {
+    WinoK k;
+    const int e = fill(d, k, false);
+    if (e) return e;
+    if (d->R != 2 || d->epi != UAVSAL_EPI_TWA) return UAVSAL_ESHAPE;
+    hipLaunchKernelGGL((wino_output_kernel<2, true>), dim3((unsigned)((k.total + 255) / 256)), dim3(256), 0, (hipStream_t)stream, k);
+    return uavsal_launch_status();
+}
+
+static int fill_seam(const uavsal_wino_desc* xout, const uavsal_wino_desc* xin, SeamK& s) {
+    WinoK ki;
+    int e = fill(xout, s.o, false);
+    if (!e) e = fill(xin, ki, true);
+    if (e) return e;
+    if (xout->R != 2 || xin->R != 2 || xout->epi != UAVSAL_EPI_TWA || xout->scale || xout->act != UAVSAL_ACT_NONE || ki.nseg)
+        return UAVSAL_ESHAPE;
+    if (xin->in != xout->out || ki.in_is != s.o.out_is || ki.ldi != s.o.ldo || ki.n_img != s.o.n_img || ki.H != s.o.H ||
+        ki.W != s.o.W || ki.C4 != s.o.C4 || ki.Mp != s.o.Mp)
+        return UAVSAL_ESHAPE;
+    s.v = ki.out; s.ldv = ki.ldo;
+    s.by = (s.o.ty + SEAM_TY - 1) / SEAM_TY; s.bx = (s.o.tx + SEAM_TX - 1) / SEAM_TX; s.slabs = (s.o.C4 + SEAM_Q - 1) / SEAM_Q;
+    if ((long long)s.o.n_img * s.by * s.bx * s.slabs > 0x7fffffffLL) return UAVSAL_ESHAPE;
+    return 0;
+}
+
+extern "C" int uavsal_wino_seam_check(const uavsal_wino_desc* xout, const uavsal_wino_desc* xin) {
+    SeamK s;
+    return fill_seam(xout, xin, s);
+}
+
+static int launch_seam(const uavsal_wino_desc* xout, const uavsal_wino_desc* xin, uavsal_stream_t stream, bool zero_h) {
+    SeamK s;
+    const int e = fill_seam(xout, xin, s);
+    if (e) return e;
+    const dim3 grid((unsigned)(s.o.n_img * s.by * s.bx * s.slabs));
+    if (zero_h) hipLaunchKernelGGL(wino_seam_kernel<true>, grid, dim3(SEAM_NT), 0, (hipStream_t)stream, s);
+    else hipLaunchKernelGGL(wino_seam_kernel<false>, grid, dim3(SEAM_NT), 0, (hipStream_t)stream, s);
+    return uavsal_launch_status();
+}
+
+extern "C" int uavsal_wino_seam(const uavsal_wino_desc* xout, const uavsal_wino_desc* xin, uavsal_stream_t stream) {
+    return launch_seam(xout, xin, stream, false);
+}
+
+extern "C" int uavsal_wino_seam_zero_h(const uavsal_wino_desc* xout, const uavsal_wino_desc* xin, uavsal_stream_t stream) {
+    return launch_seam(xout, xin, stream, true);
+}
diff --git a/iip_uavsal_saliency_amd/engine.py b/iip_uavsal_saliency_amd/engine.py
--- a/iip_uavsal_saliency_amd/engine.py
+++ b/iip_uavsal_saliency_amd/engine.py
@@ -230,9 +230,99 @@
             self._fr = (pw, dwpl) + ((N // self.ctx_T, 1) if self.ctx_mode == "tile" else (N, self.ctx_T))
         self._fr_idx = None
         self.repeat_armed = False
+        self._plan_recurrence_modes()
         self.use_lanes = bool(use_lanes)
         L.check(self.lib.uavsal_plan_enable_lanes(self.plan, 1 if self.use_lanes else 0), "plan_enable_lanes")
         self._graph_ready = False
+
+    @staticmethod
+    def _extent(v):
+        t = v.t
+        if isinstance(t, _ArenaRef):
+            lo = t.arena.buf.data_ptr() + 4 * t.off
+            return lo, lo + 4 * t.numel_
+        if isinstance(t, torch.Tensor):
+            return t.data_ptr(), t.data_ptr() + t.numel() * t.element_size()
+        return None
+
+    def seam_conflicts(self, prev, nxt):
+        v = self._extent(nxt["v"])
+        bad = []
+        for k in ("m", "out", "a", "x", "pre"):
+            e = self._extent(prev[k])
+            if v is None or (e is not None and e[0] < v[1] and v[0] < e[1]):
+                bad.append(k)
+        return bad
+
+    def _plan_recurrence_modes(self):
+        self._seams, self._zs = [], None
+        self._seams_on = None
+        self._zs_rec = None
+        self.zero_armed = False
+        steps = self.rec.twa_steps
+        if self.lstm or not self.inplace or self.arena_debug or not steps or any(s["r"] != 2 for s in steps):
+            return
+        for a, b in zip(steps, steps[1:]):
+            if b["xin"] == a["xout"] + 1 and not self.seam_conflicts(a, b):
+                self._seams.append((a["xout"], b["xin"]))
+        lay = [i for i, m in enumerate(self.ops_meta) if m.get("name") == "state.in"]
+        s0 = steps[0]
+        if s0["gemm"] == s0["xin"] + 1 and s0["xout"] == s0["gemm"] + 1:
+            self._zs = ((lay[0], lay[-1]) if lay else (-1, -1)) + (s0["xin"], s0["gemm"], s0["xout"])
+
+    def _state_is_zero(self, state) -> bool:
+        if state is None:
+            return True
+        try:
+            base = state._base if state._base is not None else state
+            sig = (state.data_ptr(), tuple(state.shape), tuple(state.stride()), state._version)
+        except RuntimeError:
+            return False
+        if state.dtype != torch.float32 or state.device != self.device:
+            return False
+        r = self._zs_rec
+        if r is not None and r["base"] is base and r["sig"] == sig:
+            if isinstance(r["zero"], tuple):
+                ev, word = r["zero"]
+                if not ev.query():
+                    return False
+                r["zero"] = bool(word[0])
+            return r["zero"]
+        src = state if state.is_contiguous() else state.contiguous()
+        ok = (src.view(torch.int32) == 0).all()
+        word = torch.zeros(1, dtype=torch.bool).pin_memory()
+        word.copy_(ok.reshape(1), non_blocking=True)
+        ev = torch.cuda.Event()
+        ev.record()
+        self._zs_rec = dict(base=base, sig=sig, zero=(ev, word))
+        return False
+
+    def invalidate_zero_state(self):
+        self._zs_rec = None
+
+    def _arm_modes(self, zero):
+        self.zero_armed = False
+        want = bool(getattr(self.model, "fuse_seams", True))
+        if self._seams and want != self._seams_on:
+            for xo, xi in self._seams:
+                r = self.lib.uavsal_plan_seam(self.plan, xo, xi, 1 if want else 0)
+                if r < 0:
+                    L.check(r, "plan_seam")
+            self._seams_on = want
+        if zero and self._zs is not None and bool(getattr(self.model, "skip_zero_state", True)):
+            r = self.lib.uavsal_plan_zero_state(self.plan, *self._zs, 1)
+            if r < 0:
+                L.check(r, "plan_zero_state")
+            self.zero_armed = r == 1
+
+    def _disarm_modes(self):
+        if self.zero_armed:
+            self.lib.uavsal_plan_zero_state(self.plan, *self._zs, 0)
+
+    def mode_report(self):
+        out = (C.c_int * 4)()
+        L.check(self.lib.uavsal_plan_mode_report(self.plan, C.byref(out)), "plan_mode_report")
+        return int(out[0]), int(out[1]), int(out[2])
 
     def __del__(self):
         try:
@@ -323,12 +413,15 @@
         pairs = [(state, self.h_view, self.state_in, "h0")]
         if self.c_view is not None:
             pairs.append((cstate, self.c_view, self.cstate_in, "c0"))
+        self._resident_zero = False
         for t, view, stage, name in pairs:
             if self._is_resident(t, view):
                 continue
             buf = self.named[name]
             if t is None:
                 buf.t.zero_()
+                if name == "h0":
+                    self._resident_zero = True
                 continue
             stage.copy_(t.reshape(stage.shape))
             d = L.LayoutDesc()
@@ -393,11 +486,16 @@
             else:
                 self.stage_inputs(x, cb0, cb1, state, cstate)
             self._arm_repeat(skip)
+            modes = self.inplace and bool(self._seams or self._zs)
+            if modes:
+                self._arm_modes(self._resident_zero if self.persistent else self._state_is_zero(state))
             with self.priors.launches():
                 try:
                     self.launch()
                 finally:
                     self._disarm_repeat()
+                    if modes:
+                        self._disarm_modes()
             if self.sync_errors:
                 self.check(wait=True)
             if not self._first_run_verified and self.split_mode:
@@ -461,7 +559,11 @@
                         mine.zero_()
                     elif prev is not None and prev is not self:
                         mine.copy_(prev.named[name].t)
-                L.check(self.lib.uavsal_plan_run(self.plan, split, -1, self._stream()), "plan_run(tail)")
+                self._arm_modes(bool(reset))
+                try:
+                    L.check(self.lib.uavsal_plan_run(self.plan, split, -1, self._stream()), "plan_run(tail)")
+                finally:
+                    self._disarm_modes()
         return out
 
     def check(self, wait=True):
diff --git a/iip_uavsal_saliency_amd/model.py b/iip_uavsal_saliency_amd/model.py
--- a/iip_uavsal_saliency_amd/model.py
+++ b/iip_uavsal_saliency_amd/model.py
@@ -154,6 +154,8 @@
         self.persistent_state = False
         self.dedupe_priors = True
         self.cache_priors = True
+        self.fuse_seams = True
+        self.skip_zero_state = True
         self.arena = True
         self.arena_debug = False
         self.max_engines = 4
@@ -251,6 +253,11 @@
             for eng in list(m._engines.values()):
                 eng.drop_prior_record()
 
+    def invalidate_state(self):
+        for m in [self] + list(self.__dict__.get("_stream_replicas") or []):
+            for eng in list(m._engines.values()):
+                eng.invalidate_zero_state()
+
     def _weights_version(self):
         return sum(t._version for t in self._wtensors)
 
diff --git a/iip_uavsal_saliency_amd/recorder.py b/iip_uavsal_saliency_amd/recorder.py
--- a/iip_uavsal_saliency_amd/recorder.py
+++ b/iip_uavsal_saliency_amd/recorder.py
@@ -62,6 +62,8 @@
         self.named: Dict[str, V] = {}
         self.prior_ops: List[int] = []
         self.binds: List[tuple] = []
+        self.twa_steps: List[dict] = []
+        self._twa_prev = None
         if not dry:
             self.plan = C.c_void_p(self.lib.uavsal_plan_create())
             if not self.plan:
@@ -348,6 +350,9 @@
         self._meta(kind="wino_in", name=name + ".xin", flops=0.0, bytes=4.0 * n * hw * cin + 4.0 * float(pp) * tiles * cin)
         self.op_args[-1].update(triple=name + ".xout")
         self.arena.touch(a, v)
+        if twa is not None and r == 2 and self._twa_prev is not None and self._twa_prev[0] == self.arena.lop - 1:
+            self.arena.touch(*self._twa_prev[1])
+        xin_op = len(self.ops_meta) - 1
         if not self.dry:
             wi = L.WinoDesc()
             wi.inp, wi.ldi, wi.in_img_stride = a.ptr, a.ld, st.get("a", hw)
@@ -373,6 +378,10 @@
             self._add(self.lib.uavsal_plan_add_conv, d, "plan_add_conv(%s)" % name)
         self._meta(kind="wino_out", name=name + ".xout", flops=0.0, bytes=4.0 * (float(pp) * tiles * cout + n * hw * cout))
         self.arena.touch(mm, out, *(twa or ()), *((a,) if twa is not None else ()))
+        if twa is not None:
+            self._twa_prev = (self.arena.lop, (mm, out, twa[0], twa[1], a))
+            self.twa_steps.append(dict(name=name, r=r, xin=xin_op, gemm=len(self.ops_meta) - 2, xout=len(self.ops_meta) - 1,
+                                       v=v, m=mm, out=out, a=a, x=twa[0], pre=twa[1]))
         if out.key is not None and self.dry:
             self.no_shadow.add(out.key)
         if not self.dry:
diff --git a/include/uavsal_hip.h b/include/uavsal_hip.h
--- a/include/uavsal_hip.h
+++ b/include/uavsal_hip.h
@@ -157,6 +157,10 @@
 
 int uavsal_wino_input(const uavsal_wino_desc* d, uavsal_stream_t stream);
 int uavsal_wino_output(const uavsal_wino_desc* d, uavsal_stream_t stream);
+int uavsal_wino_output_zero_h(const uavsal_wino_desc* d, uavsal_stream_t stream);
+int uavsal_wino_seam(const uavsal_wino_desc* xout, const uavsal_wino_desc* xin, uavsal_stream_t stream);
+int uavsal_wino_seam_zero_h(const uavsal_wino_desc* xout, const uavsal_wino_desc* xin, uavsal_stream_t stream);
+int uavsal_wino_seam_check(const uavsal_wino_desc* xout, const uavsal_wino_desc* xin);
 
 typedef struct uavsal_tsum_desc {
     const float* in;  int32_t ldi;
@@ -536,6 +540,9 @@
 int uavsal_plan_last_launches(const uavsal_plan* p);
 int uavsal_plan_frame_repeat(uavsal_plan* p, int op_pw, int op_dwpl, int src_mod, int src_div, int on);
 int uavsal_plan_frame_repeat_workgroups(const uavsal_plan* p, int which);
+int uavsal_plan_seam(uavsal_plan* p, int op_xout, int op_xin, int on);
+int uavsal_plan_zero_state(uavsal_plan* p, int op_state_in_first, int op_state_in_last, int op_xin0, int op_gemm0, int op_xout0, int on);
+int uavsal_plan_mode_report(const uavsal_plan* p, int out[4]);
 int uavsal_plan_graph_build(uavsal_plan* p, uavsal_stream_t stream);
 int uavsal_plan_graph_launch(uavsal_plan* p, uavsal_stream_t stream);
 
```

Result: faster. 2003 frames/s, median of 6 (+1.6%).
